# KirillKryukov/naf

Hardware: AMD Instinct MI355X
Metric: unnaf GB/s (uncompressed bases out) on 100 GB synthetic FASTA (higher is better)
Workload: dtype u8; 1 GPU; unnaf decode of a 100.0 GB synthetic-ACGT FASTA archive on one GPU (the size BASELINE.json's metric is quoted on; configs[1] at 10 GB rides along as cfg10_*), 100 records, 80-col lines; archive made in-run by the GPU ennaf; .naf 24739662224 B -> FASTA 99999995684 B, text + archive + decoded text resident in HBM; parallelism=one archive, one GPU, no data-path collective

## Files before the change

### naf_amd/csrc/ctx.h

```cpp
#pragma once
#include "common.h"
#include "../../include/naf_gpu.h"
#include <hip/hip_runtime.h>
#include <stdio.h>
#include <stdarg.h>
#include <string.h>
#include <vector>
#include <functional>
#include <string>

struct ArenaChunk { u8 *base; size_t cap, used; };

struct KTime { const char *name; hipEvent_t a, b; };

#define ZSPLIT_MAX 8
struct ZSplit { int parts; hipEvent_t ev[ZSPLIT_MAX]; u64 out_end[ZSPLIT_MAX]; int done; void *status; };
struct FlatStream { u64 q0, A; };
#define FLAT_DECODED (~0ull)
struct ZFlat { const u8 *src; const FlatStream *si; u64 nslots; const u8 *sym; void *status; bool ready;
               const u8 *tail; u64 tail_q; u32 tail_n;
               const u8 *cls; u32 n_decoded; u32 n_walk;
               struct naf_gpu_ctx *aux; hipEvent_t decoded_ev; void *later; };
struct CtxOpts { std::vector<std::pair<std::string, std::string>> kv; std::string trace; bool tracing = false; };
struct naf_gpu_ctx {
// ... 13 lines not shown
    std::vector<KTime> ktimes;
    std::vector<hipEvent_t> ev_pool;
    size_t ev_used = 0;
    std::vector<std::string> agg_names; std::vector<float> agg_ms; std::vector<int> agg_n;
    float stream_ms[5] = { 0, 0, 0, 0, 0 };
    naf_gpu_ctx *side = nullptr;
    naf_gpu_ctx *side2 = nullptr;
    naf_gpu_ctx *side3 = nullptr;
    naf_gpu_ctx *side4 = nullptr;
    void *sides_thread = nullptr; int sides_rc = 0;
    hipEvent_t fork_ev = nullptr;
    struct ZSplit *zsplit = nullptr;
    hipEvent_t split_ev[ZSPLIT_MAX + 2] = {};
    struct ZFlat *zflat = nullptr;
    void *io_pool = nullptr;
    void *shard_state = nullptr;
    struct HostWorker *worker = nullptr;
};

void ctx_worker_start(naf_gpu_ctx *x, std::function<void()> job);
void ctx_worker_join(naf_gpu_ctx *x);
int  ctx_sides_ready(naf_gpu_ctx *c);

int  ctx_fail(naf_gpu_ctx *c, int code, const char *fmt, ...);
const char *ctx_opt(const naf_gpu_ctx *c, const char *name);
static inline bool ctx_opt_is(const naf_gpu_ctx *c, const char *name, char v) { const char *e = ctx_opt(c, name); return e && e[0] == v; }
bool ctx_tracing(const naf_gpu_ctx *c);
void ctx_trace(naf_gpu_ctx *c, const char *fmt, ...);
#define HIP_TRY(c, call) do { hipError_t e_ = (call); if (e_ != hipSuccess) return ctx_fail((c), NAF_GPU_EHIP, "%s: %s (%s:%d)", #call, hipGetErrorString(e_), __FILE__, __LINE__); } while (0)
static inline void ctx_take_error(naf_gpu_ctx *c, const char (&text)[512]) { memcpy(c->err, text, sizeof c->err); }
static inline void ctx_take_error(naf_gpu_ctx *c, const naf_gpu_ctx *from) { ctx_take_error(c, from->err); }
static inline hipError_t ctx_side_join(naf_gpu_ctx *x) { ctx_worker_join(x); return hipStreamSynchronize(x->stream); }
#define SIDE_SYNC_TRY(c, e, x) do { if ((e) != hipSuccess) return ctx_fail((c), NAF_GPU_EHIP, "%s: %s (%s:%d)", "hipStreamSynchronize(" #x "->stream)", hipGetErrorString(e), __FILE__, __LINE__); } while (0)
struct CtxJoinGuard { naf_gpu_ctx *x; ~CtxJoinGuard() { if (x) ctx_worker_join(x); } };

void  arena_reset(naf_gpu_ctx *c);
void *arena_alloc(naf_gpu_ctx *c, size_t bytes);
void  arena_settle(naf_gpu_ctx *c);
template <typename T> T *arena_new(naf_gpu_ctx *c, size_t n) { return (T *)arena_alloc(c, n * sizeof(T)); }
static inline std::vector<size_t> arena_mark(const naf_gpu_ctx *c) { std::vector<size_t> m; for (auto &ch : c->chunks) m.push_back(ch.used); return m; }
static inline void arena_release(naf_gpu_ctx *c, const std::vector<size_t> &m) { for (size_t k = 0; k < c->chunks.size(); k++) c->chunks[k].used = k < m.size() ? m[k] : 0; }

int ctx_readback(naf_gpu_ctx *c, void *h_dst, const void *d_src, size_t bytes);
int ctx_readback2(naf_gpu_ctx *c, void *h1, const void *d1, size_t n1, void *h2, const void *d2, size_t n2);
int ctx_readbackv(naf_gpu_ctx *c, int n, void *const *h, const void *const *d, const size_t *bytes);

void ktime_begin(naf_gpu_ctx *c, const char *name);
void ktime_end(naf_gpu_ctx *c);

#define LAUNCH(c, name, kern, grid, block, shmem, ...) do { \
    ktime_begin((c), name); \
    hipLaunchKernelGGL(kern, dim3(grid), dim3(block), (shmem), (c)->stream, __VA_ARGS__); \
    ktime_end((c)); } while (0)

static inline u32 cdiv(u64 a, u64 b) { return (u32)((a + b - 1) / b); }

int scan_exclusive_u64(naf_gpu_ctx *c, u64 *d_vals, size_t n, u64 *d_total);
int scan_inclusive_max_i32(naf_gpu_ctx *c, i32 *d_vals, size_t n);
int scan_inclusive_max_i64(naf_gpu_ctx *c, i64 *d_vals, size_t n);
int scan_exclusive_u64_multi(naf_gpu_ctx *c, u64 *const *arrs, int k, size_t n, u64 *const *totals);
int scan_inclusive_max_i64_multi(naf_gpu_ctx *c, i64 *const *arrs, int k, size_t n);

int zstd_decode(naf_gpu_ctx *c, const u8 *d_src, size_t src_len, int has_magic, u8 *d_dst, size_t dst_cap, size_t *out_len, const u8 *head = nullptr);
int zstd_init_tables(naf_gpu_ctx *c);
void ennaf_shard_state_free(naf_gpu_ctx *c);
void io_pool_free(naf_gpu_ctx *c);
struct EmitP;
int zstd_decode_fused_fasta(naf_gpu_ctx *c, const u8 *d_src, size_t src_len, int has_magic, size_t *out_len, const EmitP *P, u8 *text);
struct ZRange { u64 want_lo, want_hi, got_lo, got_hi; bool ranged; u8 *own_buf; };
int zstd_decode_range(naf_gpu_ctx *c, const u8 *d_src, size_t src_len, int has_magic, u8 *d_dst, size_t dst_cap, size_t *out_len, ZRange *rg, const u8 *head = nullptr);
int zstd_split_status(naf_gpu_ctx *c, const ZSplit *sp);
int zstd_flat_later(naf_gpu_ctx *c, ZFlat *zf);
void zstd_flat_drop(ZFlat *zf);
int zstd_small_batch(naf_gpu_ctx *c, int n, const u8 *const *src, const size_t *len, u8 *const *dst, const size_t *cap, bool *ok);
bool zstd_small_fits(size_t len, size_t cap);
int zstd_small_launch(naf_gpu_ctx *c, int n, const u8 *const *src, const size_t *len, u8 *const *dst, const size_t *cap, u32 **d_res_out);
enum { ZENC_PART = 16, ZENC_PART_FIRST = 32, ZENC_PART_LAST = 64, ZENC_PREFER_RAW = 128, ZENC_PREFER_FLAT = 256, ZENC_SHORT_CODES = 512, ZENC_FRAME_TREE = 1024, ZENC_LONG_LAST = 2048 };
int zenc_level_window(int level);
int zenc_repeat_probe(naf_gpu_ctx *c, const u8 *d_src, size_t n, u32 *share_1024);
static inline u32 zenc_probe_every(u64 n) { u32 e = 64; while (((n >> 20) / e) > 128) e <<= 1; return e; }
struct ZencPlace { u8 *(*fn)(void *ud, size_t frame_len); void *ud; };
struct ZencJob;
#define ZENC_LOC_BND 20
struct ZencLoc { const u8 *loc; const i32 *blk_bnd; const u32 *blk_t0; u64 tiles; };
int zstd_encode_begin(naf_gpu_ctx *c, const u8 *d_src, size_t n, int level, int with_magic, int lz, int block_log_hint, int window_log, ZencJob **job, const u8 *direct = nullptr, u32 nd = 0, const ZencLoc *dloc = nullptr);
int zstd_encode_finish(naf_gpu_ctx *c, ZencJob *job, u8 *d_dst, size_t cap, size_t *out_len, const ZencPlace *place);
void zstd_encode_drop(ZencJob *job);
int zstd_encode_size(naf_gpu_ctx *c, ZencJob *job, size_t *frame_len);
const u64 *zstd_encode_total_ptr(const ZencJob *job);
void zstd_encode_set_total(ZencJob *job, u64 total);
int zstd_encode(naf_gpu_ctx *c, const u8 *d_src, size_t n, int level, u8 *d_dst, size_t cap, size_t *out_len, int with_magic, int lz = 0, int block_log_hint = 0, int window_log = 0, const ZencPlace *place = nullptr);
```

### naf_amd/csrc/enc.hip

```cpp
#include "ctx.h"
#include <time.h>
#include "wgscan.h"
#include "enc_swar.h"

#define ET_BYTES 16
#define ET_TILE (256 * ET_BYTES)

struct OpMaxI64 { template <typename T> __device__ static T id() { return (T)(-1); } template <typename T> __device__ static T f(T a, T b) { return (i64)a > (i64)b ? a : b; } };
struct OpMaxU32 { template <typename T> __device__ static T id() { return (T)0; } template <typename T> __device__ static T f(T a, T b) { return a > b ? a : b; } };
struct OpMaxU64 { template <typename T> __device__ static T id() { return (T)0; } template <typename T> __device__ static T f(T a, T b) { return a > b ? a : b; } };

#define REG_ACGT 0x80000000u
#define REG_E(reg) (((reg) >> 24) & 0x7Fu)
struct EncP {
    const u8 *text; u64 n, p0;
    u32 expected[8];
    u8 replacement;
    u8 id_gt_unexpected;
    u8 strict, pad;
    u32 qlo, qhi;
    u32 plo, phi;
    u32 slo, shi;
    u32 nuc32[8];
    u32 *any_case;
// ... 713 lines not shown
    u64 *longest;
    u64 *lead;
    u64 *strict_first;
    const u64 *t_seq, *t_ids, *t_cmt, *t_rec; const u32 *t_tail; const i64 *tile_eol;
    const u32 *irr_list;
    const u32 *t_reg;
    const u8 *direct; u32 nd;
    u32 loc_mode;
    const u32 *sparse_list; const u32 *n_sparse;
};


__device__ __forceinline__ void flush_tile(u8 *dst, const u8 *stage, u32 n)
{
    u32 head = (u32)((8 - ((uintptr_t)dst & 7)) & 7); if (head > n) head = n;
    if (threadIdx.x < head) dst[threadIdx.x] = stage[threadIdx.x];
    u32 words = (n - head) >> 3;
    const u64 *s64 = (const u64 *)stage;
    for (u32 w = threadIdx.x; w < words; w += blockDim.x) {
        u32 off = head + 8 * w, sh = (off & 7) * 8;
        u64 a = s64[off >> 3], b = s64[(off >> 3) + 1];
        *(u64 *)(dst + off) = sh ? (a >> sh) | (b << (64 - sh)) : a;
    }
    u32 done = head + 8 * words;
    if (threadIdx.x < n - done) dst[done + threadIdx.x] = stage[done + threadIdx.x];
}

__device__ __forceinline__ u32 nuc4x4(u32 x, const u32 *t)
{
    const u32 sel = x & 0x07070707u;
    const u32 r0 = swar_perm(t[1], t[0], sel), r1 = swar_perm(t[3], t[2], sel), r2 = swar_perm(t[5], t[4], sel), r3 = swar_perm(t[7], t[6], sel);
    const u32 m3 = ((x >> 3) & 0x01010101u) * 0xFFu, m4 = ((x >> 4) & 0x01010101u) * 0xFFu, m6 = ((x >> 6) & 0x01010101u) * 0xFFu;
    const u32 lo = (r0 & ~m3) | (r1 & m3), hi = (r2 & ~m3) | (r3 & m3);
    const u32 tab = (lo & ~m4) | (hi & m4);
    return (tab & m6) | (m4 & 0x0F0F0F0Fu & ~m6);
}
__device__ __forceinline__ u32 nuc4x4_quick(u32 x) { return swar_perm(0x0F0F0F0Fu, 0x02010408u, (x >> 1) & 0x07070707u); }
__device__ __forceinline__ u32 pack_codes8(u32 c0, u32 c1)
{
    const u32 t0 = c0 | (c0 >> 4), t1 = c1 | (c1 >> 4);
    return swar_perm(t1, t0, 0x06040200u);
}
__device__ __forceinline__ bool all_quick16(const u32 w[4], u32 qlo, u32 qhi)
{
    const u32 L = 0x7F7F7F7Fu; u32 bad = 0;
#pragma unroll
    for (int i = 0; i < 4; i++) { u32 x = w[i], r = swar_perm(qhi, qlo, (x >> 1) & 0x07070707u), d = r ^ (x & 0xDFDFDFDFu); bad |= ((d & L) + L) | d; }
    return (bad & 0x80808080u) == 0;
}
template <bool KNOWN_QUICK>
__device__ __forceinline__ void flush_pack(const EncP &P, u8 *packed, u32 *casebits, u64 tbase, u32 n, const u8 *stage )
{
    if (!n) return;
    const u32 o = (u32)(tbase & 15), span = o + n, ng = (span + 15) >> 4;
    const u64 G0 = tbase >> 4;
    for (u32 j = threadIdx.x; j < ng; j += blockDim.x) {
        const uint4 v = *(const uint4 *)(stage + 16 * j);
        const u32 w[4] = { v.x, v.y, v.z, v.w };
        u32 cd[4];
        if (KNOWN_QUICK || all_quick16(w, P.qlo, P.qhi)) {
#pragma unroll
            for (int i = 0; i < 4; i++) cd[i] = nuc4x4_quick(w[i]);
        } else {
#pragma unroll
            for (int i = 0; i < 4; i++) cd[i] = nuc4x4(w[i], P.nuc32);
        }
        u64 pk = (u64)pack_codes8(cd[0], cd[1]) | ((u64)pack_codes8(cd[2], cd[3]) << 32);
        const u32 H = 0x80808080u;
        u32 cb = swar_movemask16((v.x | ((v.x << 1) & (v.x << 2))) & H, (v.y | ((v.y << 1) & (v.y << 2))) & H,
                                 (v.z | ((v.z << 1) & (v.z << 2))) & H, (v.w | ((v.w << 1) & (v.w << 2))) & H);
        const u32 a = j == 0 ? o : 0u, b = span - 16 * j < 16 ? span - 16 * j : 16u;
        if (a == 0 && b == 16) {
            *(u64 *)(packed + 8 * (G0 + j)) = pk;
            if (casebits) ((u16 *)casebits)[G0 + j] = (u16)cb;
        } else {
            const u64 nm = (b == 16 ? ~0ull : ((1ull << (4 * b)) - 1)) & ~((1ull << (4 * a)) - 1);
            cb &= ((1u << b) - 1) & ~((1u << a) - 1);
            atomicOr((unsigned long long *)(packed + 8 * (G0 + j)), (unsigned long long)(pk & nm));
            if (casebits) atomicOr(casebits + ((G0 + j) >> 1), cb << (16 * (u32)((G0 + j) & 1)));
        }
    }
}
#define DIRECT_PROBE_BLOCKS_LOG 5
__global__ __launch_bounds__(256) void k_direct_blocks(const u8 *text, const u64 *t_seq, const u32 *t_reg, u64 tiles, u32 nd, u32 prefer_flat, int probed, u8 *direct, const u32 *blk_t0 = nullptr, i32 *blk_bnd = nullptr)
{
    __shared__ u32 bins[4][64];
    const u32 wv = threadIdx.x >> 6, lane = threadIdx.x & 63;
    const u32 b = blockIdx.x * 4 + wv;
    bins[wv][lane] = 0;
    __syncthreads();
    bool ok = b < nd;
    if (ok && probed && (((b >> DIRECT_PROBE_BLOCKS_LOG) & (u32)(probed - 1)) == 0)) ok = false;
    u64 t0 = 0, t1 = 0;
    if (ok) {
        const u64 B0 = (u64)b << 16, B1 = B0 + 65536;
        u64 lo = 0, hi = tiles;
        if (blk_t0) { lo = blk_t0[b]; hi = lo + 1; }
        while (hi - lo > 1) {
            const u64 step = (hi - lo + 63) / 64;
            const u64 p = lo + (u64)lane * step;
            const bool le = p < hi && t_seq[p] <= B0;
            const u32 cnt = (u32)__popcll(__ballot(le));
            const u64 nlo = lo + (u64)(cnt - 1) * step, nhi = nlo + step < hi ? nlo + step : hi;
            lo = nlo; hi = nhi;
        }
        t0 = lo;
        const u64 t = t0 + lane;
        const u64 ts = t <= tiles ? t_seq[t] : ~0ull;
        const bool in = t < tiles && ts < B1;
        if (blk_bnd && lane < ZENC_LOC_BND) { const i64 rel = (i64)ts - (i64)B0; blk_bnd[(u64)b * ZENC_LOC_BND + lane] = t <= tiles && rel < (1 << 30) ? (i32)rel : (i32)(1 << 30); }
        const u64 bal = __ballot(in);
        const bool good = !in || ((t_reg[t] & REG_ACGT) != 0);
        ok = __ballot(!good) == 0 && bal != ~0ull;
        t1 = t0 + (u64)__popcll(bal) - 1;
    }
    if (ok) {
        const u64 x0 = t0 * ET_TILE, span = (t1 + 1 - t0) * ET_TILE;
        const u8 *at = text + x0 + (((u64)lane * span) >> 6 & ~63ull);
        uint4 v[4]; __builtin_memcpy(v, at, 64);
        const u32 w[16] = { v[0].x, v[0].y, v[0].z, v[0].w, v[1].x, v[1].y, v[1].z, v[1].w, v[2].x, v[2].y, v[2].z, v[2].w, v[3].x, v[3].y, v[3].z, v[3].w };
        u32 *mybins = &bins[wv][(lane & 3) * 16];
#pragma unroll
        for (int i = 0; i < 16; i++) {
#pragma unroll
            for (int h = 0; h < 2; h++) {
                const u32 pr = (w[i] >> (16 * h)) & 0xFFFFu, c0 = pr & 0xFF, c1 = pr >> 8;
                if ((c0 & 0x40) && (c1 & 0x40)) atomicAdd(&mybins[((c0 >> 1) & 3) | (((c1 >> 1) & 3) << 2)], 1u);
            }
        }
    }
    __syncthreads();
    if (ok) {
        const u32 c = lane < 16 ? bins[wv][lane] + bins[wv][16 + lane] + bins[wv][32 + lane] + bins[wv][48 + lane] : 0u;
        u32 ns = c;
#pragma unroll
        for (u32 d = 1; d < 16; d <<= 1) ns += __shfl_xor((int)ns, d, 64);
        float h = c ? (float)c * __log2f((float)ns / (float)c) : 0.0f;
#pragma unroll
        for (u32 d = 1; d < 16; d <<= 1) h += __shfl_xor(h, d, 64);
        ns = (u32)__shfl((int)ns, 0, 64); h = __shfl(h, 0, 64);
        ok = ns >= 1024 && h * (float)prefer_flat > 4.0f * (float)ns * (float)(prefer_flat - 1);
    }
    if (b < nd && lane == 0) direct[b] = ok ? 1 : 0;
}
__global__ __launch_bounds__(256) void k_direct_verdict(const u64 *t_seq, const u32 *t_reg, const u8 *t_hist, u64 tiles, u32 nd, u32 prefer_flat, int probed, const u32 *blk_t0, u8 *direct, i32 *blk_bnd)
{
    const u32 b = blockIdx.x * 256 + threadIdx.x;
    if (b >= nd) return;
    const u64 B0 = (u64)b << 16, B1 = B0 + 65536, t0 = blk_t0[b];
    bool ok = !(probed && (((b >> DIRECT_PROBE_BLOCKS_LOG) & (u32)(probed - 1)) == 0));
    u64 ts[ZENC_LOC_BND];
#pragma unroll
    for (u32 i = 0; i < ZENC_LOC_BND; i++) ts[i] = t0 + i <= tiles ? t_seq[t0 + i] : ~0ull;
#pragma unroll
    for (u32 i = 0; i < ZENC_LOC_BND; i++) { const i64 rel = (i64)ts[i] - (i64)B0; blk_bnd[(u64)b * ZENC_LOC_BND + i] = ts[i] != ~0ull && rel < (1 << 30) ? (i32)rel : (i32)(1 << 30); }
    u32 acc[8] = { 0, 0, 0, 0, 0, 0, 0, 0 };
    bool end = false;
#pragma unroll
    for (u32 i = 0; i < ZENC_LOC_BND - 1; i++) {
        if (!end && ok) {
            if (t0 + i >= tiles || ts[i] >= B1) end = true;
            else if (!(t_reg[t0 + i] & REG_ACGT)) ok = false;
            else {
                const uint4 h = *(const uint4 *)(t_hist + (t0 + i) * 16);
                acc[0] += h.x & 0x00FF00FFu; acc[1] += (h.x >> 8) & 0x00FF00FFu; acc[2] += h.y & 0x00FF00FFu; acc[3] += (h.y >> 8) & 0x00FF00FFu;
                acc[4] += h.z & 0x00FF00FFu; acc[5] += (h.z >> 8) & 0x00FF00FFu; acc[6] += h.w & 0x00FF00FFu; acc[7] += (h.w >> 8) & 0x00FF00FFu;
            }
        }
    }
    ok = ok && end;
    if (ok) {
        u32 ns = 0;
#pragma unroll
        for (int k = 0; k < 8; k++) ns += (acc[k] & 0xFFFFu) + (acc[k] >> 16);
        float h = 0.0f;
#pragma unroll
        for (int k = 0; k < 8; k++) {
            const u32 c0 = acc[k] & 0xFFFFu, c1 = acc[k] >> 16;
            if (c0) h += (float)c0 * __log2f((float)ns / (float)c0);
            if (c1) h += (float)c1 * __log2f((float)ns / (float)c1);
        }
        ok = ns >= 1024 && h * (float)prefer_flat > 4.0f * (float)ns * (float)(prefer_flat - 1);
    }
    direct[b] = ok ? 1 : 0;
}
__global__ __launch_bounds__(256) void k_case_gather(const u8 *direct, u32 nd, const u32 *blk_t0, const i32 *blk_bnd, const u8 *locc, const u8 *t_lower, u64 *casebits)
{
    __shared__ i32 s_bnd[ZENC_LOC_BND]; __shared__ u8 s_low[ZENC_LOC_BND];
    const u32 b = blockIdx.x;
    if (b >= nd || !direct[b]) return;
    const u64 t0 = blk_t0[b];
    if (threadIdx.x < ZENC_LOC_BND) { s_bnd[threadIdx.x] = blk_bnd[(u64)b * ZENC_LOC_BND + threadIdx.x]; s_low[threadIdx.x] = t_lower[t0 + threadIdx.x]; }
    __syncthreads();
    u32 a[4], c[4], e[4], sh[4], av[4], kk[4]; u64 nx[4];
#pragma unroll
    for (u32 r = 0; r < 4; r++) {
        const u32 W = r * 256u + threadIdx.x;
        const i32 r0 = (i32)(64u * W);
        u32 k = (u32)(r0 - s_bnd[0]) >> 12;
        if (s_bnd[k + 1] <= r0) k++;
        if (s_bnd[k + 1] <= r0) k++;
        const u32 i = (u32)(r0 - s_bnd[k]);
        av[r] = (u32)(s_bnd[k + 1] - r0); kk[r] = k; sh[r] = i & 31u;
        const u32 *p = (const u32 *)(locc + (t0 + k) * (LOC_TILE / 2)) + (i >> 5);
        a[r] = p[0]; c[r] = p[1]; e[r] = p[2];
        nx[r] = av[r] < 64u ? ld64(locc + (t0 + k + 1) * (LOC_TILE / 2)) : 0ull;
    }
#pragma unroll
    for (u32 r = 0; r < 4; r++) {
        u64 w = s_low[kk[r]] ? (u64)__builtin_amdgcn_alignbit(c[r], a[r], sh[r]) | ((u64)__builtin_amdgcn_alignbit(e[r], c[r], sh[r]) << 32) : 0ull;
        if (av[r] < 64u) {
            w &= (1ull << av[r]) - 1;
            if (s_low[kk[r] + 1]) w |= nx[r] << av[r];
        }
        casebits[((u64)b << 10) + r * 256u + threadIdx.x] = w;
    }
}
__global__ void k_irregular_list(const u32 *t_reg, const u64 *pre, u64 tiles, u32 *list, const u64 *t_seq = nullptr, u32 *blk_t0 = nullptr)
{
    const u64 t = (u64)blockIdx.x * blockDim.x + threadIdx.x;
    if (t >= tiles) return;
    if (!t_reg[t]) list[pre[t]] = (u32)t;
    if (blk_t0) {
        const u64 lo = t_seq[t], hi = t_seq[t + 1];
        for (u64 b = (lo + 65535) >> 16; (b << 16) < hi; b++) blk_t0[b] = (u32)t;
    }
}
__global__ void k_pack_edges_zero(const u64 *t_seq, u64 tiles, u64 T, u8 *packed, u32 *casebits, const u8 *direct, u32 nd, u32 loc_mode = 0)
{
    const u64 t = (u64)blockIdx.x * blockDim.x + threadIdx.x;
    if (t >= tiles) return;
    const u64 b0 = t_seq[t], b1 = t + 1 < tiles ? t_seq[t + 1] : T;
    if (b1 <= b0) return;
    const u64 g0 = b0 >> 4, g1 = (b1 - 1) >> 4;
    const bool d0 = direct && (g0 >> 12) < nd && direct[g0 >> 12], d1 = direct && (g1 >> 12) < nd && direct[g1 >> 12];
    if (loc_mode) {
        if (!d0) { *(u64 *)(packed + 8 * g0) = 0; if (casebits) ((u16 *)casebits)[g0] = 0; }
        if (!d1) { *(u64 *)(packed + 8 * g1) = 0; if (casebits) ((u16 *)casebits)[g1] = 0; }
        return;
    }
    if (d0) *((u32 *)(packed + ((g0 >> 12) << 15) + (((g0 >> 10) & 3) << 12)) + (1023u - (u32)(g0 & 1023u))) = 0; else *(u64 *)(packed + 8 * g0) = 0;
    if (d1) *((u32 *)(packed + ((g1 >> 12) << 15) + (((g1 >> 10) & 3) << 12)) + (1023u - (u32)(g1 & 1023u))) = 0; else *(u64 *)(packed + 8 * g1) = 0;
    if (casebits) { ((u16 *)casebits)[g0] = 0; ((u16 *)casebits)[g1] = 0; }
}

__device__ __forceinline__ u64 low_bytes(u32 n) { return n >= 8 ? ~0ull : ((1ull << (8 * n)) - 1); }
__device__ __forceinline__ void lds_store_n(u8 *p, u64 lo, u64 hi, u32 n)
{
    if (n >= 16) { __builtin_memcpy(p, &lo, 8); __builtin_memcpy(p + 8, &hi, 8); return; }
    if (n & 8) { __builtin_memcpy(p, &lo, 8); p += 8; lo = hi; }
    if (n & 4) { u32 v = (u32)lo; __builtin_memcpy(p, &v, 4); p += 4; lo >>= 32; }
    if (n & 2) { u16 v = (u16)lo; __builtin_memcpy(p, &v, 2); p += 2; lo >>= 16; }
    if (n & 1) *p = (u8)lo;
}

__device__ __forceinline__ u32 piece_run_compact(const Piece &pc, u32 a, u32 b, u32 sp, u64 &lo, u64 &hi)
{
    piece_from(pc, a, lo, hi);
    u32 d = (sp >> a) & ((1u << (b - a)) - 1);
    const u32 n = (b - a) - (u32)__popc(d);
    while (d) {
        u32 k = 31 - __clz((int)d); d &= ~(1u << k);
        u64 slo = (lo >> 8) | (hi << 56), shi = hi >> 8;
        if (k < 8) { u64 m = low_bytes(k); lo = (lo & m) | (slo & ~m); hi = shi; }
        else { u64 m = low_bytes(k - 8); hi = (hi & m) | (shi & ~m); }
    }
    return n;
// ... 1721 lines not shown
    if (format == NAF_FMT_FASTA) {
        EncP P; memset(&P, 0, sizeof P);
        P.text = d_text; P.n = n; P.p0 = p0;
        set_expected(P, seq_type, true);
        u64 tiles = n / ET_TILE + 1;
        i64 *t_eol = arena_new<i64>(c, tiles + 1), *t_sp = arena_new<i64>(c, tiles + 1);
        u64 *t_seq = arena_new<u64>(c, tiles + 2), *t_ids = arena_new<u64>(c, tiles + 2), *t_cmt = arena_new<u64>(c, tiles + 2), *t_rec = arena_new<u64>(c, tiles + 2);
        u32 *t_tail = arena_new<u32>(c, tiles + 1), *t_reg = arena_new<u32>(c, tiles + 1), *irr_list = arena_new<u32>(c, tiles + 1);
        u64 *t_irr = arena_new<u64>(c, tiles + 2);
        u64 *tot = arena_new<u64>(c, 8);
        if (!t_eol || !t_sp || !t_seq || !t_ids || !t_cmt || !t_rec || !t_tail || !t_reg || !irr_list || !t_irr || !tot) return NAF_GPU_ENOMEM;
        HIP_TRY(c, hipMemsetAsync(tot + 6, 0, 8, c->stream));
        P.any_case = (u32 *)(tot + 6);
        const char *e_ed = ctx_opt(c, "DIRECT"), *e_epf = ctx_opt(c, "PREFER_FLAT"), *e_ebl = ctx_opt(c, "BLOCK_LOG"), *e_epr = ctx_opt(c, "PROBE"), *e_elz = ctx_opt(c, "LZ"), *e_op = ctx_opt(c, "ONEPASS");
        const u32 e_prefer_flat = e_epf && e_epf[0] ? (u32)atoi(e_epf) : 16u;
        const bool direct_opts = allow_direct && S.fourbit && o->level <= 1 && !o->long_log && !(e_ed && e_ed[0] == '0') && e_prefer_flat >= 2 && !(e_ebl && atoi(e_ebl) != 15) && !(e_epr && e_epr[0] == '1')
                                 && !(e_elz && !strcmp(e_elz, "all")) && n >= 16 * ET_TILE;
        const bool fused = direct_opts && enc_wave_wg(c) && !(e_op && e_op[0] == '0') && (n >> 17) >= ((e_ed && e_ed[0] == '2') || (e_op && e_op[0] == '2') ? 2u : 256u);
        u8 *loc = nullptr, *t_hist = nullptr, *locc = nullptr, *t_lower = nullptr; u32 *t_needf0 = nullptr; u64 *t_need0 = nullptr;
        if (fused) {
            loc = (u8 *)arena_alloc(c, (tiles + 1) * LOC_TILE + 64); t_hist = (u8 *)arena_alloc(c, (tiles + 1) * 16);
            locc = (u8 *)arena_alloc(c, (tiles + 1) * (LOC_TILE / 2) + 64); t_lower = (u8 *)arena_alloc(c, tiles + ZENC_LOC_BND + 2);
            if (!locc || !t_lower) return NAF_GPU_ENOMEM;
            HIP_TRY(c, hipMemsetAsync(t_lower, 0, tiles + ZENC_LOC_BND + 2, c->stream));
            t_needf0 = arena_new<u32>(c, tiles + 1); t_need0 = arena_new<u64>(c, tiles + 2);
            if (!loc || !t_hist || !t_needf0 || !t_need0) return NAF_GPU_ENOMEM;
            LAUNCH(c, "ennaf_split_once", (k_enc_fused<true, 1>), (u32)tiles, 64, 0, P, t_eol, t_sp, t_seq, t_ids, t_cmt, t_rec, t_tail, t_reg, t_irr, t_needf0, t_need0, tiles, loc, t_hist, locc, t_lower);
        } else
        LAUNCH(c, "ennaf_last", k_enc_last_fa, cdiv(tiles, 4 * LAST_TPW), 256, 0, P, t_eol, t_sp, tiles);
        { i64 *const a2[2] = { t_eol, t_sp }; if ((rc = scan_inclusive_max_i64_multi(c, a2, 2, tiles))) return rc; }
        if (S.fourbit && n >= 16 * ET_TILE) {
            u32 *t_needf = fused ? t_needf0 : arena_new<u32>(c, tiles + 1), *need_list = arena_new<u32>(c, tiles + 1); u64 *t_need = fused ? t_need0 : arena_new<u64>(c, tiles + 2);
            if (!t_needf || !need_list || !t_need) return NAF_GPU_ENOMEM;
            if (fused) LAUNCH(c, "ennaf_pure_check", k_pure_check, cdiv(tiles, 256), 256, 0, P, (const i64 *)t_eol, tiles, t_needf, t_need, t_reg, t_irr, (const u32 *)t_tail);
            else if (enc_wave_wg(c)) LAUNCH(c, "ennaf_count_pure", (k_enc_count_pure<1, 1>), (u32)tiles, 64, 0, P, (const i64 *)t_eol, t_seq, t_ids, t_cmt, t_rec, t_tail, t_reg, t_irr, t_needf, t_need, tiles);
            else LAUNCH(c, "ennaf_count_pure", (k_enc_count_pure<4, 1>), cdiv(tiles, 4), 256, 0, P, (const i64 *)t_eol, t_seq, t_ids, t_cmt, t_rec, t_tail, t_reg, t_irr, t_needf, t_need, tiles);
            if ((rc = scan_exclusive_u64(c, t_need, tiles, tot + 5))) return rc;
            LAUNCH(c, "ennaf_need_list", k_need_list, cdiv(tiles, 256), 256, 0, (const u32 *)t_needf, (const u64 *)t_need, tiles, need_list, (const u32 *)nullptr);
            u64 n_need = 0;
            if ((rc = ctx_readback(c, &n_need, tot + 5, 8))) return rc;
            if (ctx_tracing(c)) {
                std::vector<u32> hr(tiles); hipMemcpy(hr.data(), t_reg, tiles * 4, hipMemcpyDeviceToHost);
                u64 nz = 0; for (u64 i = 0; i < tiles; i++) nz += hr[i] != 0;
                ctx_trace(c, "[reg] tiles %llu need %llu regular %llu; reg[1..4] = %08x %08x %08x %08x\n", (unsigned long long)tiles, (unsigned long long)n_need, (unsigned long long)nz, hr[1], hr[2], hr[3], hr[4]);
            }
            if (n_need) LAUNCH(c, "ennaf_count", k_enc_count, n_need, 256, 0, P, (const i64 *)t_eol, (const i64 *)t_sp, t_seq, t_ids, t_cmt, t_rec, t_tail, t_reg, t_irr, (const u32 *)need_list);
        } else
        LAUNCH(c, "ennaf_count", k_enc_count, tiles, 256, 0, P, (const i64 *)t_eol, (const i64 *)t_sp, t_seq, t_ids, t_cmt, t_rec, t_tail, t_reg, t_irr, (const u32 *)nullptr);
        { u64 *const a5[5] = { t_seq, t_ids, t_cmt, t_rec, t_irr }, *const t5[5] = { tot + 0, tot + 1, tot + 2, tot + 3, tot + 4 }; if ((rc = scan_exclusive_u64_multi(c, a5, 5, tiles, t5))) return rc; }
        HIP_TRY(c, hipMemcpyAsync(t_seq + tiles, tot + 0, 8, hipMemcpyDeviceToDevice, c->stream));
        u32 *blk_t0 = fused ? arena_new<u32>(c, (size_t)(n >> 16) + 2) : nullptr;
        if (fused && !blk_t0) return NAF_GPU_ENOMEM;
        LAUNCH(c, "ennaf_irregular_list", k_irregular_list, cdiv(tiles, 256), 256, 0, (const u32 *)t_reg, (const u64 *)t_irr, tiles, irr_list, (const u64 *)t_seq, blk_t0);
        u64 h[7];
        if ((rc = ctx_readback(c, h, tot, 56))) return rc;
        T = h[0]; n_ids = h[1]; n_cmt = h[2]; N = h[3];
        S.no_case = (u32)h[6] == 0 && !(ctx_opt(c, "CASE_CENSUS") && ctx_opt(c, "CASE_CENSUS")[0] == '0');
        P.any_case = nullptr;
        const u64 n_irregular = h[4];
        if ((rc = alloc_bases(c, S, !(allow_direct && S.no_case)))) return rc;
        s_ids = (u8 *)arena_alloc(c, n_ids + 16); s_cmt = (u8 *)arena_alloc(c, n_cmt + 16);
        rec_begin = arena_new<u64>(c, N + 1); rec_end = arena_new<u64>(c, N + 1);
        const size_t NU = 3 * 257 + 3;
        u64 *d_unexp = arena_new<u64>(c, NU);
        if (!s_ids || !s_cmt || !rec_begin || !rec_end || !d_unexp) return NAF_GPU_ENOMEM;
        HIP_TRY(c, hipMemsetAsync(d_unexp, 0, NU * 8, c->stream));
        HIP_TRY(c, hipMemsetAsync(d_unexp + 3 * 257 + 1, 0xFF, 8, c->stream));
        HIP_TRY(c, hipMemsetAsync(rec_begin, 0, (N + 1) * 8, c->stream));
        EncOut O; O.seq = bases; O.packed = S.packed; O.casebits = (u32 *)S.casebits; O.ids = s_ids; O.cmt = s_cmt; O.rec_begin = rec_begin; O.rec_end = rec_end;
        O.unexpected = d_unexp; O.longest = d_unexp + 3 * 257; O.strict_first = o->strict ? d_unexp + 3 * 257 + 1 : nullptr; O.lead = d_unexp + 3 * 257 + 2;
        O.t_seq = t_seq; O.t_ids = t_ids; O.t_cmt = t_cmt; O.t_rec = t_rec; O.t_tail = t_tail; O.tile_eol = t_eol; O.t_reg = t_reg; O.irr_list = S.fourbit ? irr_list : nullptr;
        O.direct = nullptr; O.nd = 0; O.loc_mode = 0; O.sparse_list = nullptr; O.n_sparse = nullptr;
        if (S.fourbit) {
            const u64 n_seqb = (T + 1) / 2;
            const char *ed = e_ed, *epr = e_epr;
            const u32 prefer_flat = e_prefer_flat;
            const u64 nd64 = n_seqb >> 15;
            O.loc_mode = 0; O.sparse_list = nullptr; O.n_sparse = nullptr;
            if (direct_opts && nd64 >= ((ed && ed[0] == '2') || (fused && e_op && e_op[0] == '2') ? 2u : 256u) && nd64 < 0x7FFFFFFFull && !((T & 1) && (n_seqb & 32767) == 0)) {
                S.nd = (u32)nd64; S.direct = (u8 *)arena_alloc(c, S.nd); if (!S.direct) return NAF_GPU_ENOMEM;
                const bool use_loc = fused && !(e_op && e_op[0] == '3' && !S.no_case);
                i32 *blk_bnd = use_loc ? arena_new<i32>(c, (size_t)S.nd * ZENC_LOC_BND + 1) : nullptr;
                if (use_loc && !blk_bnd) return NAF_GPU_ENOMEM;
                if (use_loc) LAUNCH(c, "ennaf_direct_blocks", k_direct_verdict, cdiv(S.nd, 256), 256, 0, (const u64 *)t_seq, (const u32 *)t_reg, (const u8 *)t_hist, tiles, S.nd, prefer_flat, (epr && epr[0] == '0') ? 0 : (int)zenc_probe_every(n_seqb), (const u32 *)blk_t0, S.direct, blk_bnd);
                else LAUNCH(c, "ennaf_direct_blocks", k_direct_blocks, cdiv(S.nd, 4), 256, 0, d_text, (const u64 *)t_seq, (const u32 *)t_reg, tiles, S.nd, prefer_flat, (epr && epr[0] == '0') ? 0 : (int)zenc_probe_every(n_seqb), S.direct, (const u32 *)blk_t0, blk_bnd);
                O.direct = S.direct; O.nd = S.nd;
                if (use_loc) {
                    u32 *sparse_list = arena_new<u32>(c, tiles + 1), *n_sparse = arena_new<u32>(c, 2);
                    if (!sparse_list || !n_sparse) return NAF_GPU_ENOMEM;
                    HIP_TRY(c, hipMemsetAsync(n_sparse, 0, 8, c->stream));
                    O.loc_mode = 1; O.sparse_list = sparse_list; O.n_sparse = n_sparse;
                    LAUNCH(c, "ennaf_sparse_list", k_sparse_list, cdiv(tiles, 256), 256, 0, P, (const i64 *)t_eol, O, tiles, sparse_list, n_sparse);
                    S.dloc.loc = loc; S.dloc.blk_bnd = blk_bnd; S.dloc.blk_t0 = blk_t0; S.dloc.tiles = tiles;
                    if (S.casebits) LAUNCH(c, "ennaf_case_gather", k_case_gather, S.nd, 256, 0, (const u8 *)S.direct, S.nd, (const u32 *)blk_t0, (const i32 *)blk_bnd, (const u8 *)locc, (const u8 *)t_lower, S.casebits);
                }
                if (ctx_tracing(c)) {
                    std::vector<u8> hd(S.nd); hipStreamSynchronize(c->stream); hipMemcpy(hd.data(), S.direct, S.nd, hipMemcpyDeviceToHost);
                    u64 k = 0; for (u8 v : hd) k += v;
                    ctx_trace(c, "[direct] %llu of %u blocks\n", (unsigned long long)k, S.nd);
                }
            }
            S.sc4.P = P; S.sc4.O = O; S.sc4.t_eol = t_eol; S.sc4.t_sp = t_sp; S.sc4.t_seq = t_seq; S.sc4.tiles = tiles; S.sc4.T = T; S.sc4.n = n; S.sc4.n_irregular = n_irregular;
            if ((rc = ennaf_scatter4(c, S.sc4, S.packed, S.casebits))) return rc;
        } else LAUNCH(c, "ennaf_scatter", k_enc_scatter<false>, tiles, 256, 0, P, (const i64 *)t_eol, (const i64 *)t_sp, O);
        std::vector<u64> hu(NU);
        if ((rc = ctx_readback(c, hu.data(), d_unexp, NU * 8))) return rc;
        const u64 sk = hu[3 * 257 + 1];
        if (o->strict && sk != ~0ull) {
            const u64 pos = sk >> 11;
            unsigned long long *d_cnt = arena_new<unsigned long long>(c, 1); if (!d_cnt) return NAF_GPU_ENOMEM;
            HIP_TRY(c, hipMemsetAsync(d_cnt, 0, 8, c->stream));
            LAUNCH(c, "ennaf_count_starts", k_count_starts, (u32)((pos - p0) / 65536 + 1 < 1024 ? (pos - p0) / 65536 + 1 : 1024), 256, 0, d_text, p0, pos, 0, d_cnt);
            u64 cnt = 0; if ((rc = ctx_readback(c, &cnt, d_cnt, 8))) return rc;
            S.err_kind = SE_STRICT; S.err_char = (u32)(sk & 0x1FF); S.err_rec = cnt; S.err_a = (sk >> 9) & 3;
            return 0;
        }
        for (int k = 0; k < 3; k++) for (int i = 0; i < 257; i++) S.unexpected[k][i] = hu[k * 257 + i];
        longest = hu[3 * 257];
        S.lead = N ? hu[3 * 257 + 2] : T;
    }
    return 0;
}

struct EnnafCarry {
    u64 tail_extra;
    u32 skip_first;
    u32 tail_hi;
    int prev_masked;
    int skip_run0;
    u64 run_ext;
};
struct EnnafStreams { const u8 *ptr[6]; u64 len[6], orig[6]; int lz[6], block_log[6], window_log[6]; bool present[6];
                      u32 tail[6]; int flags[6];
                      const u8 *direct; u32 nd, tail_packed; const ZencLoc *dloc; };

static int ennaf_streams(naf_gpu_ctx *c, EnnafSplit &S, const EnnafCarry &K, EnnafStreams &X, int part = 3)
{
    if (part & 1) memset(&X, 0, sizeof X);
    int rc; const u64 T = S.T, N = S.N;
    u32 *s_len = nullptr; u8 *s_seq = nullptr, *s_mask = nullptr;
    u64 n_lenb = 0, n_seqb = 0, n_mask = 0; int mask_block_log = 15; u32 seq_tail = 0;
    if (S.format != 0) {
        if (N && (part & 2)) {
            u64 *lu = arena_new<u64>(c, N + 2); if (!lu) return NAF_GPU_ENOMEM;
            const u64 total = T + K.tail_extra;
            LAUNCH(c, "ennaf_len_count", k_len_unit_count, cdiv(N, 256), 256, 0, (const u64 *)S.rec_begin, (const u64 *)S.rec_end, N, total, lu, S.all_ends);
            if ((rc = scan_exclusive_u64(c, lu, N, lu + N + 1))) return rc;
            u64 nu = 0; if ((rc = ctx_readback(c, &nu, lu + N + 1, 8))) return rc;
            s_len = arena_new<u32>(c, nu + 1); if (!s_len) return NAF_GPU_ENOMEM;
            LAUNCH(c, "ennaf_len_write", k_len_unit_write, cdiv(N, 256), 256, 0, (const u64 *)S.rec_begin, (const u64 *)S.rec_end, N, total, (const u64 *)lu, s_len, S.all_ends);
            n_lenb = nu * 4;
        }
        const u64 mt = (T + MBB_TILE - 1) / MBB_TILE;
        u64 *tc = S.tc;
        if (!(part & 1)) { }
        else if (S.fourbit) {
            const u64 Tp = T > K.skip_first ? T - K.skip_first : 0;
            n_seqb = (Tp + 1) / 2;
            if (K.skip_first && n_seqb) {
                s_seq = (u8 *)arena_alloc(c, n_seqb + 16); if (!s_seq) return NAF_GPU_ENOMEM;
                LAUNCH(c, "ennaf_nibble_shift", k_nibble_shift, cdiv(cdiv(n_seqb, 8), 256), 256, 0, (const u8 *)S.packed, (T + 1) / 2, s_seq, n_seqb);
            } else s_seq = S.packed;
            if ((Tp & 1) && K.tail_hi) LAUNCH(c, "ennaf_tail_nibble", k_set_high_nibble, 1, 64, 0, s_seq + n_seqb - 1, K.tail_hi);
            if ((Tp & 1) && !K.tail_hi && n_seqb >= 2 && !S.store_qual) seq_tail = 1;
        } else {
            if (S.no_mask && T) LAUNCH(c, "ennaf_toupper", k_toupper, cdiv(T, 256), 256, 0, S.bases, T);
            s_seq = S.bases; n_seqb = T;
        }
        if (S.store_mask && T && (part & 2)) {
            u64 nb = 0; i64 *tile_last = S.census ? S.census_last : nullptr;
            const bool one_run = !S.census && S.no_case && !K.skip_run0 && !K.prev_masked;
            if (!one_run) {
            if (!S.census) {
                tc = arena_new<u64>(c, mt + 2); tile_last = arena_new<i64>(c, mt + 1); if (!tc || !tile_last) return NAF_GPU_ENOMEM;
                LAUNCH(c, "ennaf_mask_count", k_maskb_count, mt, 256, 0, (const u64 *)S.casebits, T, tc, 0, tile_last);
                if ((rc = scan_inclusive_max_i64(c, tile_last, mt))) return rc;
            }
            const int b0 = S.census ? ((S.first_base >= 96) != (K.prev_masked != 0)) : 0;
            if (b0) LAUNCH(c, "ennaf_mask_b0", k_add_u64, 1, 64, 0, tc, (u64)1);
            if ((rc = scan_exclusive_u64(c, tc, mt, tc + mt + 1))) return rc;
            if ((rc = ctx_readback(c, &nb, tc + mt + 1, 8))) return rc;
            }
            u64 nu = 0;
            if (nb == 0 && !K.skip_run0) {
                const u64 len = T + K.run_ext;
                nu = len / 255 + 1;
                s_mask = (u8 *)arena_alloc(c, nu + 16); if (!s_mask) return NAF_GPU_ENOMEM;
                HIP_TRY(c, hipMemsetAsync(s_mask, 0xFF, nu, c->stream));
                SmallBytes lb; memset(&lb, 0, sizeof lb); lb.b[0] = (u8)(len % 255); lb.n = 1;
                LAUNCH(c, "ennaf_mask_units", k_put_bytes, 1, 64, 0, s_mask + (nu - 1), lb);
            } else {
            u64 *any_long = arena_new<u64>(c, 1), *bnd = nullptr;
            if (!any_long) return NAF_GPU_ENOMEM;
            u64 longs = 1;
            const char *ms = ctx_opt(c, "MASK_SHORT");
            if (tile_last && nb >= (1u << 16) && nb * 64 >= T && !(ms && (ms[0] == '0' || ms[0] == '1'))) {
                nu = nb + 1 - (K.skip_run0 ? 1 : 0);
                s_mask = (u8 *)arena_alloc(c, nu + 16); if (!s_mask) return NAF_GPU_ENOMEM;
                HIP_TRY(c, hipMemsetAsync(any_long, 0, 8, c->stream));
                LAUNCH(c, "ennaf_mask_units", k_maskb_units_direct, mt, 256, 0, (const u64 *)S.casebits, T, (const u64 *)tc, (const i64 *)tile_last, nb, s_mask, K.run_ext, K.skip_run0, K.prev_masked, any_long);
                if ((rc = ctx_readback(c, &longs, any_long, 8))) return rc;
            }
            if (longs) {
            bnd = arena_new<u64>(c, nb + 1); if (!bnd) return NAF_GPU_ENOMEM;
            if (nb) LAUNCH(c, "ennaf_mask_bscatter", k_maskb_scatter, mt, 256, 0, (const u64 *)S.casebits, T, (const u64 *)tc, nb, bnd, K.prev_masked);
            { 
              if (!(ms && ms[0] == '0') && (nb + 1) * 255 > T + K.run_ext) {
                  nu = nb + 1 - (K.skip_run0 ? 1 : 0);
                  s_mask = (u8 *)arena_alloc(c, nu + 16); if (!s_mask) return NAF_GPU_ENOMEM;
                  HIP_TRY(c, hipMemsetAsync(any_long, 0, 8, c->stream));
                  LAUNCH(c, "ennaf_mask_units", k_mask_units_short, cdiv(nb + 1, 256), 256, 0, (const u64 *)bnd, nb, T, s_mask, K.run_ext, K.skip_run0, any_long);
                  if ((rc = ctx_readback(c, &longs, any_long, 8))) return rc;
              } }
            }
            if (longs) {
                u64 *ru = arena_new<u64>(c, nb + 3); if (!ru) return NAF_GPU_ENOMEM;
                LAUNCH(c, "ennaf_mask_runs", k_mask_run_units, cdiv(nb + 1, 256), 256, 0, (const u64 *)bnd, nb, T, ru, K.run_ext, K.skip_run0);
                if ((rc = scan_exclusive_u64(c, ru, nb + 1, ru + nb + 2))) return rc;
                if ((rc = ctx_readback(c, &nu, ru + nb + 2, 8))) return rc;
                s_mask = (u8 *)arena_alloc(c, nu + 16); if (!s_mask) return NAF_GPU_ENOMEM;
                if (nu) HIP_TRY(c, hipMemsetAsync(s_mask, 0xFF, nu, c->stream));
                LAUNCH(c, "ennaf_mask_units", k_mask_units_write, cdiv(nb + 1, 256), 256, 0, (const u64 *)bnd, nb, T, (const u64 *)ru, s_mask, K.run_ext, K.skip_run0);
            }
            }
            mask_block_log = 13;
            { const char *mb = ctx_opt(c, "MASK_BLOCK_LOG"); if (mb && atoi(mb) >= 10 && atoi(mb) <= 17) mask_block_log = atoi(mb); else if (nu >= (64ull << 20)) mask_block_log = 15; }
            n_mask = nu;
        }
    }
    if (part & 1) {
        X.ptr[0] = S.s_ids; X.len[0] = X.orig[0] = S.n_ids; X.lz[0] = 1; X.present[0] = true;
        X.ptr[1] = S.s_cmt; X.len[1] = X.orig[1] = S.n_cmt; X.lz[1] = 1; X.present[1] = true;
        { const char *sb_ = ctx_opt(c, "NAMES_BLOCK_LOG"); const int v = sb_ ? atoi(sb_) : 0; if (v >= 10 && v <= 15) X.block_log[1] = v; else if (S.n_cmt >= (16u << 20)) X.block_log[1] = 15; }
        X.tail_packed = seq_tail; X.direct = nullptr; X.nd = 0;
        X.dloc = nullptr;
        if (S.direct && (part & 1)) { X.direct = S.direct; X.nd = S.nd; seq_tail = (u32)(n_seqb & 32767); X.dloc = S.dloc.loc ? &S.dloc : nullptr; }
        X.ptr[4] = s_seq; X.len[4] = n_seqb; X.orig[4] = T; X.present[4] = true; X.tail[4] = seq_tail;
        if (S.store_qual) X.flags[4] |= ZENC_LONG_LAST;
        X.ptr[5] = S.s_qual; X.len[5] = X.orig[5] = S.n_qual; X.present[5] = S.store_qual;
    }
    if (part & 2) {
        X.ptr[2] = (const u8 *)s_len; X.len[2] = X.orig[2] = n_lenb; X.lz[2] = 1; X.present[2] = true;
        { const char *sb_ = ctx_opt(c, "SIDE_BLOCK_LOG"); const int v = sb_ ? atoi(sb_) : 0; if (v >= 10 && v <= 15) X.block_log[2] = v; else if (n_lenb >= (16u << 20)) X.block_log[2] = 15; }
        X.ptr[3] = s_mask; X.len[3] = X.orig[3] = n_mask; X.block_log[3] = mask_block_log; X.present[3] = S.store_mask; X.flags[3] = ZENC_PREFER_RAW;
    }
    return 0;
}

static void ennaf_probe_verdict(EnnafStreams &X, u32 share) { if (share >= 32) { X.window_log[4] = 19; X.lz[4] = 1; } }
static int ennaf_windows(naf_gpu_ctx *c, EnnafStreams &X, const naf_gpu_ennaf_opts *o, bool *defer = nullptr)
{
    const int wl = zenc_level_window(o->level);
    for (int i = 0; i < 6; i++) X.window_log[i] = wl;
    if (o->level <= 1) X.flags[4] |= ZENC_PREFER_FLAT;
    if (o->level <= 1) { X.flags[4] |= ZENC_SHORT_CODES; X.flags[5] |= ZENC_SHORT_CODES; }
    if (o->level <= 1) { X.flags[4] |= ZENC_FRAME_TREE; X.flags[5] |= ZENC_FRAME_TREE; }
    if (o->long_log) { X.window_log[4] = o->long_log < 10 ? 10 : o->long_log > 31 ? 31 : o->long_log; X.lz[4] = 1; }
    else if (!wl && X.present[4] && X.len[4]) {
        const char *pe = ctx_opt(c, "PROBE");
        u32 share = 0;
        if (pe && pe[0] == '1') share = 1024;
        else if (!(pe && pe[0] == '0') && defer) { *defer = true; return 0; }
        else if (!(pe && pe[0] == '0')) {
            int rc = zenc_repeat_probe(c, X.ptr[4], X.len[4], &share); if (rc) return rc;
        }
        ennaf_probe_verdict(X, share);
    }
    return 0;
}

static size_t naf_header_bytes(const naf_gpu_ennaf_opts *o, bool store_mask, bool store_qual, u64 longest, u64 N, u8 *hd )
{
    size_t hl = 0;
    hd[hl++] = 0x01; hd[hl++] = 0xF9; hd[hl++] = 0xEC;
    if (o->seq_type == NAF_SEQ_DNA) hd[hl++] = 1; else { hd[hl++] = 2; hd[hl++] = (u8)o->seq_type; }
    hd[hl++] = (u8)(((o->title ? 1 : 0) << 6) | (1 << 5) | (1 << 4) | (1 << 3) | ((store_mask ? 1 : 0) << 2) | (1 << 1) | (store_qual ? 1 : 0));
    hd[hl++] = ' ';
    hl += vle(o->line_length >= 0 ? (u64)o->line_length : longest, hd + hl);
    hl += vle(N, hd + hl);
    if (o->title) hl += vle(strlen(o->title), hd + hl);
    return hl;
}

struct PlaceTail { const ZencPlace *outer; size_t tail_len; u8 *at; };
static u8 *place_before_tail(void *ud, size_t len) { PlaceTail *t = (PlaceTail *)ud; return t->at = t->outer->fn(t->outer->ud, len + t->tail_len); }
struct StreamJob { ZencJob *main; const u8 *d_stream; u64 len; int level, flags; u32 tail; bool sized; u8 *tail_tmp; size_t tail_len; int tail_flags; };
static int encode_stream_begin(naf_gpu_ctx *c, const u8 *d_stream, u64 len, int level, int flags, int lz, int block_log, int window_log, u32 tail, StreamJob *J, const u8 *direct = nullptr, u32 nd = 0, const ZencLoc *dloc = nullptr)
{
    J->main = nullptr; J->d_stream = d_stream; J->len = len; J->level = level; J->flags = flags; J->tail = (tail && len > tail) ? tail : 0;
    J->sized = false; J->tail_tmp = nullptr; J->tail_len = 0; J->tail_flags = 0;
    int f1 = flags;
    if (J->tail) f1 = ZENC_PART | ((!(flags & ZENC_PART) || (flags & ZENC_PART_FIRST)) ? ZENC_PART_FIRST : 0) | (flags & (ZENC_PREFER_RAW | ZENC_PREFER_FLAT | ZENC_SHORT_CODES | ZENC_FRAME_TREE));
    J->tail_flags = flags & ZENC_LONG_LAST;
    if (direct && (lz || len - J->tail != (u64)nd << 15)) return ctx_fail(c, NAF_GPU_EARG, "direct blocks need a stream of whole blocks and no match finder");
    int rc = zstd_encode_begin(c, d_stream, len - J->tail, level, f1, lz, block_log, window_log, &J->main, direct, nd, dloc);
    if (rc) { zstd_encode_drop(J->main); J->main = nullptr; }
    return rc;
}
static int encode_stream_size(naf_gpu_ctx *c, StreamJob *J, size_t *clen)
{
    if (J->tail && !J->sized) {
        const int f2 = ZENC_PART | ((!(J->flags & ZENC_PART) || (J->flags & ZENC_PART_LAST)) ? ZENC_PART_LAST : 0) | J->tail_flags;
        const size_t tb = naf_gpu_zstd_compress_bound(J->tail);
        u8 *tmp = (u8 *)arena_alloc(c, tb); if (!tmp) return NAF_GPU_ENOMEM;
        size_t b = 0;
        int rc = zstd_encode(c, J->d_stream + (J->len - J->tail), J->tail, J->level, tmp, tb, &b, f2, 0, 0, 0); if (rc) return rc;
        J->tail_tmp = tmp; J->tail_len = b;
    }
    size_t a = 0;
    int rc = zstd_encode_size(c, J->main, &a); if (rc) return rc;
    J->sized = true;
    *clen = a + J->tail_len;
    return 0;
}
static int encode_stream_finish(naf_gpu_ctx *c, StreamJob *J, size_t *clen, const ZencPlace *place)
{
    ZencJob *mj = J->main; J->main = nullptr;
    if (!J->tail) return zstd_encode_finish(c, mj, nullptr, 0, clen, place);
    const int f2 = ZENC_PART | ((!(J->flags & ZENC_PART) || (J->flags & ZENC_PART_LAST)) ? ZENC_PART_LAST : 0) | J->tail_flags;
// ... 14 lines not shown
}
static int encode_stream(naf_gpu_ctx *c, const u8 *d_stream, u64 len, int level, u8 *dst, size_t cap, size_t *clen, int flags, int lz, int block_log, int window_log, u32 tail, const ZencPlace *place = nullptr)
{
    if (place) {
        StreamJob J; int rc = encode_stream_begin(c, d_stream, len, level, flags, lz, block_log, window_log, tail, &J); if (rc) return rc;
        return encode_stream_finish(c, &J, clen, place);
    }
    if (!tail || len <= tail) return zstd_encode(c, d_stream, len, level, dst, cap, clen, flags, lz, block_log, window_log);
    const bool part = (flags & ZENC_PART) != 0;
    const int f1 = ZENC_PART | ((!part || (flags & ZENC_PART_FIRST)) ? ZENC_PART_FIRST : 0) | (flags & (ZENC_PREFER_RAW | ZENC_PREFER_FLAT | ZENC_SHORT_CODES | ZENC_FRAME_TREE));
    const int f2 = ZENC_PART | ((!part || (flags & ZENC_PART_LAST)) ? ZENC_PART_LAST : 0) | (flags & ZENC_LONG_LAST) | (tail >= 2048 ? (flags & (ZENC_PREFER_FLAT | ZENC_SHORT_CODES)) : 0);
    size_t a = 0, b = 0;
    int rc = zstd_encode(c, d_stream, len - tail, level, dst, cap, &a, f1, lz, block_log, window_log); if (rc) return rc;
    rc = zstd_encode(c, d_stream + (len - tail), tail, level, dst + a, cap - a, &b, f2, 0, 0, 0); if (rc) return rc;
    *clen = a + b;
    return 0;
}

__global__ void k_collect4(const u64 *a, const u64 *b, const u64 *c4, const u64 *d, u64 *out) { if (threadIdx.x < 4) { const u64 *p = threadIdx.x == 0 ? a : threadIdx.x == 1 ? b : threadIdx.x == 2 ? c4 : d; out[threadIdx.x] = p ? *p : 0; } }
struct SecOut { u64 orig, comp; };

struct SecPlace { naf_gpu_ctx *c; u8 *d_naf; size_t cap, pos; u64 orig; size_t hl; int rc; };
static u8 *place_section(void *ud, size_t clen)
{
    SecPlace *p = (SecPlace *)ud; naf_gpu_ctx *c = p->c;
    SmallBytes h; memset(&h, 0, sizeof h);
    size_t hl = vle(p->orig, h.b); hl += vle(clen, h.b + hl); h.n = (u32)hl;
    if (p->pos + hl + clen > p->cap) { p->rc = ctx_fail(c, NAF_GPU_ECAP, "ennaf output capacity %zu too small", p->cap); return nullptr; }
    hipLaunchKernelGGL(k_put_bytes, dim3(1), dim3(64), 0, c->stream, p->d_naf + p->pos, h);
    if (hipGetLastError() != hipSuccess) { p->rc = ctx_fail(c, NAF_GPU_EHIP, "section header launch failed"); return nullptr; }
    p->hl = hl;
    return p->d_naf + p->pos + hl;
}

static int put_section(naf_gpu_ctx *c, naf_gpu_ctx *report, const u8 *d_stream, u64 stream_len, u64 orig, int level, u8 *d_naf, size_t cap, size_t &pos, SecOut &so, int lz, int block_log, int window_log, u32 tail, StreamJob *early, int flags = 0, const u8 *direct = nullptr, u32 nd = 0, const ZencLoc *dloc = nullptr)
{
    SecPlace sp = { c, d_naf, cap, pos, orig, 0, 0 }; ZencPlace P = { place_section, &sp };
    size_t clen = 0;
    StreamJob J;
    int rc = 0;
    if (!early) { rc = encode_stream_begin(c, d_stream, stream_len, level, flags, lz, block_log, window_log, tail, &J, direct, nd, dloc); early = &J; }
    if (!rc) rc = encode_stream_finish(c, early, &clen, &P);
    if (rc) { if (report != c) ctx_fail(report, sp.rc ? sp.rc : rc, "%s", c->err); return sp.rc ? sp.rc : rc; }
    pos += sp.hl + clen;
    so.orig = orig; so.comp = clen;
    return 0;
}

static int ennaf_whole(naf_gpu_ctx *c, const void *d_text_, size_t n, const naf_gpu_ennaf_opts *o,
                       void *d_naf_, size_t cap, size_t *naf_len, naf_gpu_ennaf_report *rep);
extern "C" int naf_gpu_ennaf(naf_gpu_ctx *c, const void *d_text_, size_t n, const naf_gpu_ennaf_opts *o,
                             void *d_naf_, size_t cap, size_t *naf_len, naf_gpu_ennaf_report *rep)
{
    if (!c || !o || !d_naf_ || !naf_len || (!d_text_ && n)) return NAF_GPU_EARG;
    int rc = ennaf_whole(c, d_text_, n, o, d_naf_, cap, naf_len, rep);
    arena_settle(c);
    return rc;
}
static int ennaf_whole(naf_gpu_ctx *c, const void *d_text_, size_t n, const naf_gpu_ennaf_opts *o,
                       void *d_naf_, size_t cap, size_t *naf_len, naf_gpu_ennaf_report *rep)
{
    arena_reset(c);
    { int rs = ctx_sides_ready(c); if (rs) return rs; }
    const u8 *d_text = (const u8 *)d_text_; u8 *d_naf = (u8 *)d_naf_;
    naf_gpu_ennaf_report R; memset(&R, 0, sizeof R);
    if (o->seq_type < 0 || o->seq_type > 3) return ctx_fail(c, NAF_GPU_EARG, "bad seq_type");
    int format = 0, rc; u64 p0 = 0;
    if ((rc = ennaf_sniff(c, d_text, n, o->format, &format, &p0))) return rc;
    R.format = format;
    EnnafSplit S;
    if ((rc = ennaf_split(c, d_text, n, o, format, p0, true, S, true))) return rc;
    if (S.err_kind) return split_error_text(c, o->seq_type, S.err_kind, S.err_char, S.err_rec, S.err_a, S.err_b, 0);
    EnnafCarry K; memset(&K, 0, sizeof K);
    naf_gpu_ctx *sc = c->side;
    const char *eo = ctx_opt(c, "ENC_OVERLAP");
    const bool force_overlap = eo && !strcmp(eo, "2");
    const bool overlap = sc && !(eo && !strcmp(eo, "0")) && (force_overlap || S.T >= (32u << 20) || S.n_qual >= (16u << 20));
    EnnafStreams X;
    if ((rc = ennaf_streams(c, S, K, X, overlap ? 1 : 3))) return rc;
    bool probe_later = false;
    if ((rc = ennaf_windows(c, X, o, overlap ? &probe_later : nullptr))) return rc;
    auto undirect = [&]() -> int {
        if (!X.direct) return 0;
        X.direct = nullptr; X.nd = 0; X.tail[4] = X.tail_packed; S.direct = nullptr; S.nd = 0; X.dloc = nullptr; S.dloc.loc = nullptr;
        S.sc4.O.direct = nullptr; S.sc4.O.nd = 0; S.sc4.O.loc_mode = 0;
        return ennaf_scatter4(c, S.sc4, S.packed, S.casebits);
    };
    if (X.lz[4] && (rc = undirect())) return rc;
    u8 hd[64]; size_t hl = naf_header_bytes(o, S.store_mask, S.store_qual, S.longest, S.N, hd);
    size_t tl = o->title ? strlen(o->title) : 0;
    size_t pos = 0;
    if (hl + tl > cap) return ctx_fail(c, NAF_GPU_ECAP, "ennaf output capacity %zu too small", cap);
    { SmallBytes hb; memset(&hb, 0, sizeof hb); memcpy(hb.b, hd, hl); hb.n = (u32)hl; LAUNCH(c, "ennaf_header", k_put_bytes, 1, 64, 0, d_naf, hb); pos += hl; }
    if (tl) { HIP_TRY(c, hipMemcpyAsync(d_naf + pos, o->title, tl, hipMemcpyHostToDevice, c->stream)); pos += tl; HIP_TRY(c, hipStreamSynchronize(c->stream)); }
    StreamJob big[6]; bool early[6] = { false, false, false, false, false, false };
    naf_gpu_ctx *sb = nullptr; int rcB = 0;
    naf_gpu_ctx *pc = nullptr; int rcP = 0; u32 probe_share = 0; bool probe_out = false;
    auto bail = [&](int r, naf_gpu_ctx *from) -> int {
        if (sb) ctx_worker_join(sb);
        if (probe_out) { ctx_worker_join(pc); probe_out = false; hipStreamSynchronize(pc->stream); }
        for (int k = 0; k < 6; k++) if (early[k]) { zstd_encode_drop(big[k].main); early[k] = false; }
        hipStreamSynchronize(sc->stream); if (sb) hipStreamSynchronize(sb->stream);
        return from && from != c ? ctx_fail(c, r, "%s", from->err) : r;
    };
    if (overlap) {
        arena_reset(sc);
        HIP_TRY(c, hipEventRecord(c->fork_ev, c->stream));
        HIP_TRY(c, hipStreamWaitEvent(sc->stream, c->fork_ev, 0));
        sb = (S.N >= 65536 || force_overlap || (S.store_mask && S.T >= (256u << 20))) ? c->side2 : nullptr;
        if (sb) {
            arena_reset(sb);
            HIP_TRY(c, hipStreamWaitEvent(sb->stream, c->fork_ev, 0));
            ctx_worker_start(sb, [&] {
                rcB = ennaf_streams(sb, S, K, X, 2);
                for (int i = 2; i < 4 && !rcB; i++)
                    if (X.present[i]) { rcB = encode_stream_begin(sb, X.ptr[i], X.len[i], o->level, X.flags[i], X.lz[i], X.block_log[i], X.window_log[i], X.tail[i], &big[i]); early[i] = !rcB; }
            });
        } else if ((rc = ennaf_streams(sc, S, K, X, 2))) return bail(rc, sc);
        if (probe_later && c->side3) {
            pc = c->side3;
            arena_reset(pc);
            if (hipStreamWaitEvent(pc->stream, c->fork_ev, 0) != hipSuccess) return bail(ctx_fail(c, NAF_GPU_EHIP, "ennaf: the look's stream"), c);
            probe_out = true;
            ctx_worker_start(pc, [&] { rcP = zenc_repeat_probe(pc, X.ptr[4], X.len[4], &probe_share); });
        }
        for (int i = 4; i < 6; i++)
            if (X.present[i]) {
                if ((rc = encode_stream_begin(c, X.ptr[i], X.len[i], o->level, X.flags[i], X.lz[i], X.block_log[i], X.window_log[i], X.tail[i], &big[i], i == 4 ? X.direct : nullptr, i == 4 ? X.nd : 0u, i == 4 ? X.dloc : nullptr))) return bail(rc, c);
                early[i] = true;
            }
        for (int i = 0; i < 2; i++)
            if (X.present[i]) {
                if ((rc = encode_stream_begin(sc, X.ptr[i], X.len[i], o->level, X.flags[i], X.lz[i], X.block_log[i], X.window_log[i], X.tail[i], &big[i]))) return bail(rc, sc);
                early[i] = true;
            }
        if (probe_later) {
            if (probe_out) { ctx_worker_join(pc); probe_out = false; if (rcP) return bail(rcP, pc); }
            else if ((rc = zenc_repeat_probe(sc, X.ptr[4], X.len[4], &probe_share))) return bail(rc, sc);
            ennaf_probe_verdict(X, probe_share);
            if (X.lz[4]) {
                zstd_encode_drop(big[4].main); early[4] = false;
                if ((rc = undirect())) return bail(rc, c);
                if ((rc = encode_stream_begin(c, X.ptr[4], X.len[4], o->level, X.flags[4], X.lz[4], X.block_log[4], X.window_log[4], X.tail[4], &big[4]))) return bail(rc, c);
                early[4] = true;
            }
        }
    }
    for (int i = 0; i < 257; i++) { R.unexpected_id[i] = S.unexpected[0][i]; R.unexpected_comment[i] = S.unexpected[1][i]; R.unexpected_seq[i] = S.unexpected[2][i]; R.unexpected_qual[i] = S.unexpected[3][i]; }
    R.n_sequences = S.N; R.n_bases = S.T; R.longest_line = S.longest;

    SecOut so[6]; memset(so, 0, sizeof so);
    bool joined = !overlap, joinedB = sb == nullptr;
    auto join = [&]() -> int {
        if (joined) return 0;
        joined = true;
        if (hipEventRecord(c->split_ev[0], sc->stream) != hipSuccess || hipStreamWaitEvent(c->stream, c->split_ev[0], 0) != hipSuccess) return ctx_fail(c, NAF_GPU_EHIP, "ennaf: joining the side stream failed");
        if (sb && (hipEventRecord(c->split_ev[1], sb->stream) != hipSuccess || hipStreamWaitEvent(c->stream, c->split_ev[1], 0) != hipSuccess)) return ctx_fail(c, NAF_GPU_EHIP, "ennaf: joining the side stream failed");
        return 0;
    };
    auto joinB = [&]() -> int {
        if (joinedB) return 0;
        joinedB = true;
        ctx_worker_join(sb);
        return rcB ? ctx_fail(c, rcB, "%s", sb->err) : 0;
    };
    const char *sf = ctx_opt(c, "SIZES_FIRST");
    if (overlap && !(sf && sf[0] == '0')) {
// ... 378 lines not shown
```

### naf_amd/csrc/zstd_enc.hip

```cpp
#include "ctx.h"
#include <vector>
#include "zstd_enc_core.h"

#define ZENC_TREE_SLOT 192
#include "wgscan.h"
#include "enc_swar.h"
struct OpMaxU64 { template <typename T> __device__ static T id() { return (T)0; } template <typename T> __device__ static T f(T a, T b) { return a > b ? a : b; } };
#define ZENC_HCOPIES 4
#define ZENC_CACHE_ENTRIES 256
struct ZTreeEntry { u64 key; u32 tb, pad; u8 wt[256]; u8 tree[ZENC_TREE_SLOT]; };
struct ZTreeCache { ZTreeEntry e[ZENC_CACHE_ENTRIES]; };
static_assert(ZENC_CACHE_ENTRIES == 256, "one entry per thread of the plan kernel");
struct ZPlanWS {
    u32 tot[256]; u32 w[512]; u16 order[256]; u16 parent[512]; u8 depth[512];
    u8 len[256], wt[256], tree[ZENC_TREE_SLOT], tmp[160];
    FseWS fse; u32 log, tb;
};

struct ZFlat16 { u32 tb; u8 tree[ZENC_TREE_SLOT]; };
static const ZFlat16 &zenc_flat16()
{
    static const ZFlat16 T = [] {
        ZFlat16 t; memset(&t, 0, sizeof t);
        u8 wt[256]; memset(wt, 0, sizeof wt);
        for (u32 s = 0; s < 256; s++) if (__builtin_popcount(s & 15u) == 1 && __builtin_popcount(s >> 4) == 1) wt[s] = 1;
        static FseWS ws; u8 tmp[160];
        t.tb = huf_write_tree_w(t.tree, wt, 0x88u, tmp, ws, true);
        return t;
    }();
    return T;
}
__host__ __device__ static inline u64 zenc_block_lo(u64 n, u32 nblk, u32 b) { u64 q = n / nblk, r = n % nblk; return (u64)b * q + (b < r ? b : r); }

#define ZENC_FLATSCAN_WAVES 4
__global__ __launch_bounds__(64 * ZENC_FLATSCAN_WAVES) void k_zenc_flat_scan(const u8 *src, u64 n, u32 nblk, ZEncPlan *plan, u16 *codes, u8 *trees, u64 *csize, u8 *done, u32 min_gain, u32 prefer_flat, ZFlat16 f16, const u8 *planned, const u8 *direct)
{
    __shared__ u32 bins[ZENC_FLATSCAN_WAVES][64];
    const u32 wv = threadIdx.x >> 6, lane = threadIdx.x & 63;
    for (u32 bq = blockIdx.x; bq * ZENC_FLATSCAN_WAVES < nblk; bq += gridDim.x) {
    const u32 b = bq * ZENC_FLATSCAN_WAVES + wv;
    if (planned && bq * ZENC_FLATSCAN_WAVES + ZENC_FLATSCAN_WAVES <= nblk && *(const u32 *)(planned + bq * ZENC_FLATSCAN_WAVES) == 0x01010101u) continue;
    bins[wv][lane] = 0;
    __syncthreads();
    bool ok = b < nblk;
    u32 bn = 0; const u8 *s = src;
    if (ok) {
        const u64 lo = zenc_block_lo(n, nblk, b), hi = zenc_block_lo(n, nblk, b + 1);
        bn = (u32)(hi - lo); s = src + lo;
        ok = bn >= 2048;
    }
    const bool dir = ok && direct && direct[b];
    if (ok && !dir) {
        u64 bad = 0;
        const bool sampler = (lane & 3) == 0;
        u32 *mybins = &bins[wv][((lane >> 2) & 3) * 16];
        const u64 M5 = 0x5555555555555555ull, M3 = 0x3333333333333333ull, ONE = 0x1111111111111111ull;
#pragma unroll 8
        for (u32 i = lane * 16; i + 16 <= bn; i += 1024) {
            const u64 w0 = ld64(s + i), w1 = ld64(s + i + 8);
            u64 c0 = w0 - ((w0 >> 1) & M5), c1 = w1 - ((w1 >> 1) & M5);
            c0 = (c0 & M3) + ((c0 >> 2) & M3); c1 = (c1 & M3) + ((c1 >> 2) & M3);
            bad |= (c0 ^ ONE) | (c1 ^ ONE);
            if (sampler) {
                const u64 lg = ((w0 >> 1) & 0x7777777777777777ull) - ((w0 >> 3) & 0x1111111111111111ull);
                const u64 rk = ((lg >> 2) & 0x0C0C0C0C0C0C0C0Cull) | (lg & 0x0303030303030303ull);
#pragma unroll
                for (u32 k = 0; k < 8; k++) atomicAdd(&mybins[(u32)(rk >> (8 * k)) & 15u], 1u);
            }
        }
        if (lane == 0) for (u32 k = bn & ~15u; k < bn; k++) { const u32 v = s[k]; if (__popc(v & 15u) != 1 || __popc(v >> 4) != 1) bad = 1; }
        ok = __ballot(bad != 0) == 0;
    }
    __syncthreads();
    bool fast = dir;
    if (ok && !dir) {
        const u32 c = lane < 16 ? bins[wv][lane] + bins[wv][16 + lane] + bins[wv][32 + lane] + bins[wv][48 + lane] : 0u;
        u32 ns = c;
#pragma unroll
        for (u32 d = 1; d < 16; d <<= 1) ns += __shfl_xor((int)ns, d, 64);
        float h = c ? (float)c * __log2f((float)ns / (float)c) : 0.0f;
#pragma unroll
        for (u32 d = 1; d < 16; d <<= 1) h += __shfl_xor(h, d, 64);
        ns = (u32)__shfl((int)ns, 0, 64); h = __shfl(h, 0, 64);
        fast = ns > 0 && h * (float)prefer_flat > 4.0f * (float)ns * (float)(prefer_flat - 1);
    }
    if (fast) {
        const u32 perq = (bn + 3) / 4;
        ZEncPlan p; p.n = bn; p.kind = ZK_RAW; p.csize = 3 + bn; p.log = 0; p.tree_bytes = 0; p.lhdr = 0; p.pad = 0; p.frame = 0; p.pad2 = 0;
        for (u32 k = 0; k < 4; k++) p.ssz[k] = ((k < 3 ? perq : bn - 3 * perq) * 4 + 8) >> 3;
        zenc_plan_finish(p, bn, 4, f16.tb, min_gain);
        fast = p.kind == ZK_HUF;
        if (fast) {
            p.pad = dir ? 2 : 1;
            if (lane == 0) { plan[b] = p; if (csize) csize[b] = p.csize; }
            if (!dir)
            for (u32 sym = lane; sym < 256; sym += 64) {
                const bool is16 = __popc(sym & 15u) == 1 && __popc(sym >> 4) == 1;
                const u32 hn = sym >> 4, ln = sym & 15u, rank = 4 * ((hn >> 1) - (hn >> 3)) + ((ln >> 1) - (ln >> 3));
                codes[(u64)b * 256 + sym] = is16 ? (u16)(rank | (4u << 12)) : (u16)0;
            }
            for (u32 k = lane; k < p.tree_bytes; k += 64) trees[(u64)b * ZENC_TREE_SLOT + k] = f16.tree[k];
        }
    }
    if (b < nblk && lane == 0) done[b] = fast ? 1 : 0;
    }
}

__global__ void k_zenc_direct_plans(const u8 *direct, u32 nblk, ZEncPlan pd, ZFlat16 f16, ZEncPlan *plan, u8 *trees, u64 *csize, u8 *done)
{
    const u32 b = blockIdx.x * blockDim.x + threadIdx.x;
    if (b >= nblk || !direct[b]) return;
    plan[b] = pd; if (csize) csize[b] = pd.csize; done[b] = 1;
    for (u32 k = 0; k < pd.tree_bytes; k++) trees[(u64)b * ZENC_TREE_SLOT + k] = f16.tree[k];
}

__global__ __launch_bounds__(256) void k_zenc_plan(const u8 *src, u64 n, u32 nblk, ZEncPlan *plan, u16 *codes, u8 *trees, u64 *csize, const u32 *blk_len, u64 slot, ZTreeCache *cache, u32 sample_stride, u32 try_fse, u32 min_gain, u32 maxbits, u32 prefer_flat, const u8 *done, u8 *wt_defer,
                                                    u32 *fhist = nullptr, const ZEncPlan *fplan = nullptr, const u16 *fcodes = nullptr, const u32 *fratio = nullptr, u32 long_last = 0)
{
    __shared__ u32 hist[ZENC_HCOPIES * 1024];
    u32 b = sample_stride ? blockIdx.x * sample_stride : blockIdx.x;
    if (done && done[b]) return;
    u64 lo = zenc_block_lo(n, nblk, b), hi = zenc_block_lo(n, nblk, b + 1);
    if (blk_len) { lo = (u64)b * slot; hi = lo + blk_len[b]; }
    u32 bn = (u32)(hi - lo);
    for (u32 i = threadIdx.x; i < ZENC_HCOPIES * 1024; i += 256) hist[i] = 0;
    __syncthreads();
    u32 per = (bn + 3) / 4; if (!per) per = 1;
    const u8 *s = src + lo;
    const u32 cpy = threadIdx.x & (ZENC_HCOPIES - 1), rot = 8 * cpy;
    u32 *my = hist + cpy * 1024;
    const u64 rot8 = 0x0101010101010101ull * rot;
#ifdef ZPLAN_NOHIST
    if (threadIdx.x < 16) for (u32 q = 0; q < 4; q++) hist[q * 256 + threadIdx.x * 17] = bn / 64;
    if (0)
#endif
    for (u32 i0 = threadIdx.x * 8; i0 < bn; i0 += 8 * 2048) {
        u64 wv[8];
#pragma unroll
        for (u32 j = 0; j < 8; j++) { const u32 i = i0 + j * 2048; wv[j] = i + 8 <= bn ? ld64(s + i) : 0; }
#pragma unroll
        for (u32 j = 0; j < 8; j++) {
            const u32 i = i0 + j * 2048;
            if (i >= bn) break;
            if (i + 8 <= bn) {
                const u64 w = wv[j];
                const u32 q0 = (i >= per) + (i >= 2 * per) + (i >= 3 * per), q7 = (i + 7 >= per) + (i + 7 >= 2 * per) + (i + 7 >= 3 * per);
                if (q0 == q7) {
                    const u64 H = 0x8080808080808080ull;
                    const u64 wr = ((w & ~H) + rot8) ^ (w & H);
                    u32 *hq = my + q0 * 256;
                    const u32 lo = (u32)wr, hi = (u32)(wr >> 32);
#pragma unroll
                    for (u32 k = 0; k < 4; k++) { atomicAdd(&hq[(lo >> (8 * k)) & 0xFF], 1u); atomicAdd(&hq[(hi >> (8 * k)) & 0xFF], 1u); }
                } else {
#pragma unroll
                    for (u32 k = 0; k < 8; k++) { u32 pos = i + k, q = (pos >= per) + (pos >= 2 * per) + (pos >= 3 * per); atomicAdd(&my[q * 256 + (((u32)(w >> (8 * k)) + rot) & 0xFF)], 1u); }
                }
            } else {
                for (u32 k = 0; i + k < bn; k++) { u32 pos = i + k, q = (pos >= per) + (pos >= 2 * per) + (pos >= 3 * per); atomicAdd(&my[q * 256 + ((s[pos] + rot) & 0xFF)], 1u); }
            }
        }
    }
    __syncthreads();
    u32 red4[4];
    for (u32 q = 0; q < 4; q++) { u32 v = 0; for (u32 k = 0; k < ZENC_HCOPIES; k++) v += hist[k * 1024 + q * 256 + ((threadIdx.x + 8 * k) & 0xFF)]; red4[q] = v; }
    __syncthreads();
    for (u32 q = 0; q < 4; q++) hist[q * 256 + threadIdx.x] = red4[q];
    __syncthreads();
    static_assert(sizeof(ZPlanWS) <= (ZENC_HCOPIES - 1) * 4096, "plan workspace must fit the dead histogram copies");
    ZPlanWS &ws = *(ZPlanWS *)(hist + 1024);
    __shared__ u64 red[4];
    const u32 sym = threadIdx.x;
    u32 mine = hist[sym] + hist[256 + sym] + hist[512 + sym] + hist[768 + sym];
    ws.tot[sym] = mine; ws.len[sym] = 0;
    u32 distinct = (u32)__syncthreads_count(mine != 0);
    __shared__ u16 plist[256]; __shared__ u32 wave_n[4];
    u64 bal = __ballot(mine != 0);
    u32 myidx = (u32)__popcll(bal & ((1ull << (threadIdx.x & 63)) - 1));
    if ((threadIdx.x & 63) == 0) wave_n[threadIdx.x >> 6] = (u32)__popcll(bal);
    __syncthreads();
    for (u32 w = 0; w < (threadIdx.x >> 6); w++) myidx += wave_n[w];
    if (mine) plist[myidx] = (u16)sym;
    __syncthreads();
    ZEncPlan p; p.n = bn; p.kind = ZK_RAW; p.csize = 3 + bn; p.log = 0; p.tree_bytes = 0; p.lhdr = 0; p.pad = 0; p.frame = 0; p.pad2 = 0;
    p.ssz[0] = p.ssz[1] = p.ssz[2] = p.ssz[3] = 0;
    if (fhist && sample_stride && mine) atomicAdd(&fhist[sym], mine);
    if (fcodes && !sample_stride && fplan->kind == ZK_HUF && bn >= 64 && distinct >= 2) {
        __shared__ u64 fred[4];
        const u32 fl = (u32)fcodes[sym] >> 12;
        if (__syncthreads_and(mine == 0 || fl != 0)) {
            const float ent = mine ? (float)mine * __log2f((float)bn / (float)mine) : 0.f;
            u64 both; wg_scan_inclusive<u64, OpAdd>(((u64)(mine * fl) << 32) | (u64)(u32)(ent + 0.5f), &both, fred);
            const u64 fbits = both >> 32, ebits = both & 0xFFFFFFFFull;
            if (fbits * 1024 * 100 <= ebits * fratio[0] * 103 + 6400ull * 1024) {
                for (u32 k = 0; k < 4; k++) { u64 bits; wg_scan_inclusive<u64, OpAdd>((u64)hist[256 * k + sym] * fl, &bits, fred); p.ssz[k] = (u32)((bits + 1 + 7) / 8); }
                zenc_plan_finish(p, bn, fplan->log, 0, min_gain);
                if (p.kind == ZK_HUF && p.csize + fplan->tree_bytes <= 3 + bn) {
                    p.frame = 1; codes[(u64)b * 256 + sym] = fcodes[sym];
                    if (threadIdx.x == 0) { plan[b] = p; if (csize) csize[b] = p.csize; }
                    return;
                }
                if (p.kind != ZK_HUF) {
                    if (threadIdx.x == 0) { plan[b] = p; if (csize) csize[b] = p.csize; }
// ... 100 lines not shown
        __syncthreads();
        u32 log = ws.log;
        if (prefer_flat && log && !flat_log && (distinct & (distinct - 1)) == 0) {
            const u32 k = (u32)(31 - __clz((int)distinct));
            u64 hb; wg_scan_inclusive<u64, OpAdd>((u64)mine * ws.len[sym], &hb, red);
            const u64 fb = (u64)bn * k;
            if (fb >= hb && (fb - hb) * prefer_flat < fb) {
                ws.len[sym] = mine ? (u8)k : (u8)0;
                if (threadIdx.x == 0) ws.log = k;
                flat_log = k;
            }
            __syncthreads();
            log = ws.log;
        }
        if (log) {
            u32 l = ws.len[sym];
            ws.wt[sym] = l ? (u8)(log + 1 - l) : 0;
            u64 lastw; wg_scan_inclusive<u64, OpMaxU64>(l ? (u64)sym : 0, &lastw, red);
            u64 hk; wg_scan_inclusive<u64, OpAdd>(l ? (u64)(sym * 16 + (log + 1 - l) + 1) * 0x9E3779B97F4A7C15ull ^ ((u64)sym << 40) : 0, &hk, red);
            hk |= 1;
            bool hit = false;
            if (cache && !sample_stride) {
                __shared__ u32 s_slot;
                if (threadIdx.x == 0) s_slot = ~0u;
                __syncthreads();
                if (cache->e[sym].key == hk) atomicMin(&s_slot, sym);
                __syncthreads();
                u32 slot_i = s_slot;
                if (slot_i != ~0u) {
                    const ZTreeEntry *ce = &cache->e[slot_i];
                    hit = __syncthreads_and(ce->wt[sym] == ws.wt[sym]) != 0;
                    if (hit) { if (sym < ZENC_TREE_SLOT) ws.tree[sym] = ce->tree[sym]; if (sym == 0) ws.tb = ce->tb; }
                }
            }
            const bool direct_w = !try_fse && (u32)lastw >= 1 && (u32)lastw <= 128;
            defer = wt_defer && !sample_stride && !hit && !direct_w && (u32)lastw >= 1;
            if (!hit && direct_w) {
                const u32 nw = (u32)lastw;
                if (sym == 0) { ws.tree[0] = (u8)(127 + nw); ws.tb = 1 + (nw + 1) / 2; }
                if (2 * sym < nw) ws.tree[1 + sym] = (u8)((ws.wt[2 * sym] << 4) | (2 * sym + 1 < nw ? ws.wt[2 * sym + 1] : 0));
            }
            else if (!hit && defer) wt_defer[(u64)b * 256 + sym] = ws.wt[sym];
            else if (!hit && threadIdx.x == 0) ws.tb = huf_write_tree_w(ws.tree, ws.wt, (u32)lastw, ws.tmp, ws.fse, try_fse != 0);
            if (cache && sample_stride) {
                __syncthreads();
                ZTreeEntry *ce = &cache->e[blockIdx.x];
                ce->wt[sym] = ws.wt[sym]; if (sym < ZENC_TREE_SLOT) ce->tree[sym] = ws.tree[sym];
                if (sym == 0) { ce->tb = ws.tb; ce->key = ws.tb ? hk : 0; }
            }
            u64 bits;
            if (flat_log) {
                const u32 perq = (bn + 3) / 4;
                for (u32 k = 0; k < 4; k++) p.ssz[k] = ((k < 3 ? perq : bn - 3 * perq) * flat_log + 8) >> 3;
            } else
            for (u32 k = 0; k < 4; k++) { wg_scan_inclusive<u64, OpAdd>((u64)hist[256 * k + sym] * l, &bits, red); p.ssz[k] = (u32)((bits + 1 + 7) / 8); }
            __syncthreads();
            u32 tb = ws.tb;
            if (defer) {
                huf = true; p.log = (u8)log; p.tree_bytes = (u16)lastw; p.lhdr = (u8)(try_fse != 0);
                p.pad = (u8)(0x80u | ((log == 4 && distinct == 16) ? 1u : 0u));
            } else
            if (tb) { zenc_plan_finish(p, bn, log, tb, min_gain); huf = p.kind == ZK_HUF; if (huf && log == 4 && distinct == 16) p.pad = 1; }
        }
    }
    if (threadIdx.x == 0) { plan[b] = p; if (csize) csize[b] = p.csize; }
    if (huf && p.log && ws.len[plist[0]] == p.log && distinct == (1u << p.log)) {
        const u32 l = ws.len[sym];
        codes[(u64)b * 256 + sym] = l ? (u16)(myidx | (l << 12)) : (u16)0;
        if (!defer && sym < p.tree_bytes) trees[(u64)b * ZENC_TREE_SLOT + sym] = ws.tree[sym];
    } else
    if (huf) {
        __shared__ u32 wcnt[16], wstart[16];
        if (sym < 16) wcnt[sym] = 0;
        __syncthreads();
        u32 l = ws.len[sym], wgt = l ? p.log + 1 - l : 0, rank = 0;
        if (l) { atomicAdd(&wcnt[wgt], 1u); for (u32 j = 0; j < myidx; j++) rank += ws.len[plist[j]] == l; }
        __syncthreads();
        if (sym == 0) { u32 pos = 0; for (u32 w = 1; w <= p.log; w++) { wstart[w] = pos; pos += wcnt[w] << (w - 1); } }
        __syncthreads();
        codes[(u64)b * 256 + sym] = l ? (u16)(((wstart[wgt] >> (wgt - 1)) + rank) | (l << 12)) : (u16)0;
        if (!defer && sym < p.tree_bytes) trees[(u64)b * ZENC_TREE_SLOT + sym] = ws.tree[sym];
    }
}

#define ZENC_FRAME_BLOCK 32768u
__global__ __launch_bounds__(256) void k_zenc_frame_block(const u32 *fhist, u8 *blockbuf, u32 *blen)
{
    __shared__ u64 red[4];
    const u32 sym = threadIdx.x, h = fhist[sym];
    u64 tot; wg_scan_inclusive<u64, OpAdd>((u64)h, &tot, red);
    u32 cnt = 0;
    if (h && tot) { cnt = (u32)(((u64)h * (ZENC_FRAME_BLOCK - 256)) / tot); if (!cnt) cnt = 1; }
    u64 all; const u64 inc = wg_scan_inclusive<u64, OpAdd>((u64)cnt, &all, red);
    u8 *o = blockbuf + (inc - cnt);
    for (u32 k = 0; k < cnt; k++) o[k] = (u8)sym;
    if (sym == 0) *blen = (u32)all;
}
__global__ __launch_bounds__(256) void k_zenc_frame_ratio(u32 *fhist, const u16 *fcodes)
{
    __shared__ u64 red[4];
    const u32 h = fhist[threadIdx.x], l = (u32)fcodes[threadIdx.x] >> 12;
    u64 tot = wg_reduce1<u64, OpAdd>((u64)h, red);
    __syncthreads();
    const float ent = (h && tot) ? (float)h * __log2f((float)tot / (float)h) : 0.f;
    const u64 both = wg_reduce1<u64, OpAdd>(((u64)h * l) << 0 | 0ull, red);
    __syncthreads();
    const u64 e = wg_reduce1<u64, OpAdd>((u64)(ent + 0.5f), red);
    if (threadIdx.x == 0) { u64 r = e ? both * 1024 / e : 1024; fhist[257] = (u32)(r < 1024 ? 1024 : r > 1229 ? 1229 : r); }
}
#define ZQ_MISSING 0x80u
__device__ __forceinline__ u32 zq_hash4(u32 x) { return (x ^ (x >> 4)) & 0x0F0F0F0Fu; }
__global__ __launch_bounds__(256) void k_zenc_frame_stats(const u32 *fhist, const u16 *fcodes, float *fstat)
{
    __shared__ u64 red[4];
    const u32 sym = threadIdx.x, h = fhist[sym], l = (u32)fcodes[sym] >> 12, x[3] = { l, l * l, (sym ^ (sym >> 4)) & 15u };
    const u64 N = wg_reduce1<u64, OpAdd>((u64)h, red);
    __syncthreads();
    for (u32 k = 0; k < 3; k++) {
        const u64 a = wg_reduce1<u64, OpAdd>((u64)h * x[k], red);
        __syncthreads();
        const u64 b2 = wg_reduce1<u64, OpAdd>((u64)h * x[k] * x[k], red);
        __syncthreads();
        if (sym == 0) {
            const double mu = N ? (double)a / (double)N : 0.0, var = N ? (double)b2 / (double)N - mu * mu : 0.0;
            fstat[2 * k] = (float)mu; fstat[2 * k + 1] = var > 0.0 ? (float)sqrt(var) : 0.f;
        }
    }
}
__global__ __launch_bounds__(256) void k_zenc_frame_quick(const u8 *src, u64 n, u32 nblk, ZEncPlan *plan, u16 *codes, u64 *csize, u8 *done,
                                                           const ZEncPlan *fplan, const u16 *fcodes, const float *fstat, u32 min_gain, u32 stride, u32 *tally, const u32 *gate)
{
    __shared__ __attribute__((aligned(16))) u8 tab[256 * 64];
    __shared__ u32 s_q[4][4], s_accept;
    const u32 b = stride ? blockIdx.x * stride : blockIdx.x, tid = threadIdx.x, lane = tid & 63, q = tid >> 6;
    if (!stride && gate && gate[0] * 2 < gate[1]) return;
    if (b >= nblk || done[b] || fplan->kind != ZK_HUF) return;
    const u64 lo = zenc_block_lo(n, nblk, b), hi = zenc_block_lo(n, nblk, b + 1);
    const u32 bn = (u32)(hi - lo);
    if (bn < 64) return;
    const u16 fc = fcodes[tid];
    {
        const u32 l = (u32)fc >> 12, v = (l ? l : ZQ_MISSING) * 0x01010101u;
        uint4 r; r.x = r.y = r.z = r.w = v;
        uint4 *row = (uint4 *)(tab + 64 * tid);
        row[0] = r; row[1] = r; row[2] = r; row[3] = r;
    }
    __syncthreads();
    const u32 per = (bn + 3) / 4;
    const u32 qlo = q * per < bn ? q * per : bn, qhi = q == 3 ? bn : (qlo + per < bn ? qlo + per : bn);
    const u8 *s = src + lo, *my = tab + lane;
    u32 s1 = 0, s2 = 0, orr = 0, sh = 0;
    for (u32 i0 = qlo + lane * 8; i0 < qhi; i0 += 8 * 512) {
        u64 wv[8];
#pragma unroll
        for (u32 j = 0; j < 8; j++) { const u32 i = i0 + j * 512; wv[j] = i + 8 <= qhi ? ld64(s + i) : 0; }
#pragma unroll
        for (u32 j = 0; j < 8; j++) {
            const u32 i = i0 + j * 512;
            if (i >= qhi) break;
            if (i + 8 <= qhi) {
                const u32 x0 = (u32)wv[j], x1 = (u32)(wv[j] >> 32);
#pragma unroll
                for (u32 k = 0; k < 4; k++) {
                    const u32 t0 = my[((x0 >> (8 * k)) & 0xFF) << 6], t1 = my[((x1 >> (8 * k)) & 0xFF) << 6];
                    s1 += t0 + t1; s2 += t0 * t0; s2 += t1 * t1; orr |= t0 | t1;
                }
                sh = swar_dot4(zq_hash4(x0), 0x01010101u, sh); sh = swar_dot4(zq_hash4(x1), 0x01010101u, sh);
            } else for (u32 k = 0; i + k < qhi; k++) {
                const u32 c = s[i + k], t = my[c << 6];
                s1 += t; s2 += t * t; orr |= t; sh += (c ^ (c >> 4)) & 15u;
            }
        }
    }
#pragma unroll
    for (int d = 32; d; d >>= 1) { s1 += (u32)__shfl_xor((int)s1, d, 64); s2 += (u32)__shfl_xor((int)s2, d, 64); sh += (u32)__shfl_xor((int)sh, d, 64); orr |= (u32)__shfl_xor((int)orr, d, 64); }
    if (lane == 0) { s_q[q][0] = s1; s_q[q][1] = s2; s_q[q][2] = sh; s_q[q][3] = orr; }
    __syncthreads();
    ZEncPlan p;
    if (tid == 0) {
        u32 accept = 0;
        const u32 S[3] = { s_q[0][0] + s_q[1][0] + s_q[2][0] + s_q[3][0], s_q[0][1] + s_q[1][1] + s_q[2][1] + s_q[3][1], s_q[0][2] + s_q[1][2] + s_q[2][2] + s_q[3][2] };
        bool like = !((s_q[0][3] | s_q[1][3] | s_q[2][3] | s_q[3][3]) & ZQ_MISSING);
        const float fb = (float)bn, rt = sqrtf(fb);
        for (u32 k = 0; k < 3 && like; k++) {
            const float want = fb * fstat[2 * k], d = fabsf((float)S[k] - want);
            if (d > 6.f * rt * fstat[2 * k + 1] + 0.005f * want) like = false;
        }
        if (like) {
            p.n = bn; p.kind = ZK_RAW; p.csize = 3 + bn; p.log = 0; p.tree_bytes = 0; p.lhdr = 0; p.pad = 0; p.frame = 0; p.pad2 = 0;
            for (u32 k = 0; k < 4; k++) p.ssz[k] = (s_q[k][0] + 1 + 7) / 8;
            zenc_plan_finish(p, bn, fplan->log, 0, min_gain);
            if (p.kind == ZK_HUF && p.csize + fplan->tree_bytes <= 3 + bn) { p.frame = 1; accept = 1; }
            else if (p.kind != ZK_HUF) accept = 2;
        }
        if (stride) { atomicAdd(&tally[1], 1u); if (accept) atomicAdd(&tally[0], 1u); accept = 0; }
        if (accept) { plan[b] = p; if (csize) csize[b] = p.csize; done[b] = 1; }
        s_accept = accept;
    }
    __syncthreads();
    if (s_accept == 1) codes[(u64)b * 256 + tid] = fc;
}

__global__ void k_zenc_frame_class(const ZEncPlan *plan, u32 nblk, i32 *v)
{
    const u32 b = blockIdx.x * blockDim.x + threadIdx.x;
    if (b < nblk) v[b] = plan[b].kind == ZK_HUF ? (i32)(2 * b + (plan[b].frame ? 0u : 1u)) : -1;
}
__global__ void k_zenc_frame_fix(ZEncPlan *plan, u32 nblk, const i32 *v, const ZEncPlan *fplan, const u8 *ftree, u8 *trees, u64 *csize)
{
    const u32 b = blockIdx.x * blockDim.x + threadIdx.x;
    if (b >= nblk || plan[b].kind != ZK_HUF || !plan[b].frame) return;
    const i32 prev = b ? v[b - 1] : -1;
    if (prev >= 0 && !(prev & 1)) return;
    ZEncPlan p = plan[b];
    const u32 tb = fplan->tree_bytes;
    zenc_plan_force(p, tb);
    for (u32 k = 0; k < tb; k++) trees[(u64)b * ZENC_TREE_SLOT + k] = ftree[k];
    plan[b] = p; if (csize) csize[b] = p.csize;
}

struct ZTreeLane { FseWS fse; u8 tmp[160]; u8 w[256]; u32 odd; };
static_assert((sizeof(ZTreeLane) / 4) % 2 == 1, "odd word stride: the lanes' workspaces start in different LDS banks");
__global__ __launch_bounds__(64) void k_zenc_tree(u32 nblk, ZEncPlan *plan, u8 *trees, u64 *csize, const u8 *wt_defer, u32 min_gain)
{
    __builtin_amdgcn_s_setprio(3);
    extern __shared__ __attribute__((aligned(16))) u8 tree_lds[];
    const u32 b = blockIdx.x * 64 + threadIdx.x;
    const bool pending = b < nblk && (plan[b].pad & 0x80u);
    if (!__ballot(pending)) return;
    if (!pending) return;
    ZTreeLane &L = ((ZTreeLane *)tree_lds)[threadIdx.x];
    ZEncPlan p = plan[b];
    const u32 lastw = p.tree_bytes, log = p.log, try_fse = p.lhdr, flat16 = p.pad & 1u;
    for (u32 k = 0; k < 256; k += 4) *(u32 *)(L.w + k) = *(const u32 *)(wt_defer + (u64)b * 256 + k);
    u8 *tree = trees + (u64)b * ZENC_TREE_SLOT;
    const u32 tb = huf_write_tree_w(tree, L.w, lastw, L.tmp, L.fse, try_fse != 0);
    p.kind = ZK_RAW; p.csize = 3 + p.n; p.log = 0; p.tree_bytes = 0; p.lhdr = 0; p.pad = 0; p.frame = 0; p.pad2 = 0;
    if (tb) { zenc_plan_finish(p, p.n, log, tb, min_gain); if (p.kind == ZK_HUF && flat16) p.pad = 1; }
    plan[b] = p;
    if (csize) csize[b] = p.csize;
}

#define LZ_MINMATCH 5
__device__ __forceinline__ u32 rdlane(u32 v, u32 l) { return (u32)__builtin_amdgcn_readlane((int)v, (int)l); }
#define LZ_HASH_LOG 12
#define LZ_BLOCK_MAX 32768
#define LZ_LANE_EXT 32
struct LzBufs {
    u8 *lits; u64 slot;
    u16 *ll, *ml, *of; u64 seq_slot;
    u32 *ofv;
    u32 *nseq, *nlit;
    u8 *seqbuf; u32 *seq_bytes;
};
__global__ __launch_bounds__(64) void k_lz_parse(const u8 *src, u64 n, u32 nblk, LzBufs B, u32 buf_bytes, u32 hash_log, const u8 *fallback = nullptr)
{
    if (fallback && !fallback[blockIdx.x]) return;

    __builtin_amdgcn_s_setprio(3);
    extern __shared__ __attribute__((aligned(16))) u8 lz_lds[];
    u8 *buf = lz_lds;
    u16 *tab = (u16 *)(lz_lds + buf_bytes);
    const u32 b = blockIdx.x, lane = threadIdx.x;
    const u64 lo = zenc_block_lo(n, nblk, b);
    const u32 bn = (u32)(zenc_block_lo(n, nblk, b + 1) - lo);
    for (u32 i = lane * 16; i < bn; i += 64 * 16) {
        if (i + 16 <= bn) { uint4 v; __builtin_memcpy(&v, src + lo + i, 16); *(uint4 *)(buf + i) = v; }
        else for (u32 k = i; k < bn; k++) buf[k] = src[lo + k];
    }
    for (u32 i = lane; i < (1u << hash_log); i += 64) tab[i] = 0;
    for (u32 i = bn + lane; i < bn + 320 && i < buf_bytes; i += 64) buf[i] = 0;
    __syncthreads();
    u8 *lits = B.lits + (u64)b * B.slot;
    u16 *sll = B.ll + (u64)b * B.seq_slot, *sml = B.ml + (u64)b * B.seq_slot, *sof = B.of + (u64)b * B.seq_slot;
    u32 cur = 0, anchor = 0, ns = 0, nl = 0;
    while (cur + LZ_MINMATCH <= bn) {
        u32 p = cur + lane; bool valid = p + LZ_MINMATCH <= bn;
        u32 v = 0, h = 0, c = 0, m = 0;
        if (valid) {
            __builtin_memcpy(&v, buf + p, 4);
            h = (v * 2654435761u) >> (32 - hash_log);
            c = tab[h];
            if (c) {
                u32 q = c - 1, cv; __builtin_memcpy(&cv, buf + q, 4);
                if (cv == v) {
                    m = 4;
                    for (;;) {
                        u64 x, y; __builtin_memcpy(&x, buf + q + m, 8); __builtin_memcpy(&y, buf + p + m, 8);
                        const u64 d = x ^ y;
                        if (d) { m += (u32)(__ffsll((long long)d) - 1) >> 3; break; }
                        m += 8;
                        if (p + m >= bn || m >= LZ_LANE_EXT) break;
                    }
                    if (p + m > bn) m = bn - p;
                }
            }
        }
        u64 win = __ballot(m >= LZ_MINMATCH);
        if (valid) tab[h] = (u16)(p + 1);
        u32 next = cur < anchor ? anchor : cur;
        while (next < cur + 64) {
            u64 w2 = win & ~((1ull << (next - cur)) - 1);
            if (!w2) break;
            u32 f = (u32)__ffsll((long long)w2) - 1;
            u32 pf = cur + f, mf = rdlane(m, f), cf = rdlane(c, f) - 1;
            while (mf >= LZ_LANE_EXT && pf + mf < bn) {
                u32 x, y; __builtin_memcpy(&x, buf + cf + mf + 4 * lane, 4); __builtin_memcpy(&y, buf + pf + mf + 4 * lane, 4);
                u32 d = x ^ y;
                u64 ne = __ballot(d != 0);
                if (!ne) { mf += 256; continue; }
                u32 l0 = (u32)__ffsll((long long)ne) - 1;
                u32 d0 = rdlane(d, l0);
                mf += 4 * l0 + (((u32)__ffs((int)d0) - 1) >> 3);
                break;
            }
            if (pf + mf > bn) mf = bn - pf;
            u32 ll = pf - anchor;
            for (u32 k = lane; k < ll; k += 64) lits[nl + k] = buf[anchor + k];
            if (lane == 0) { sll[ns] = (u16)ll; sml[ns] = (u16)mf; sof[ns] = (u16)(pf - cf); }
            nl += ll; ns++;
            anchor = next = pf + mf;
        }
        cur += 64;
// ... 337 lines not shown
    mode[b] = lz ? 1 : 0; csize[b] = lz ? s1 : s0;
}

#define ZENC_BLOCKS_PER_WG 16
#define ZENC_OROW 80
template <int GROUP>
__device__ __forceinline__ void huf_encode_stream_staged(u8 *out, const u8 *src, u32 n, const u16 *codes, u8 *orow)
{
    u64 acc = 0; u32 nb = 0;
    u32 lo = (u32)((uintptr_t)out & 63), fill = lo;
    u8 *seg = out - lo;
    auto flush_group = [&]() {
        __builtin_memcpy(orow + fill, &acc, 8);
        fill += nb >> 3; acc >>= (nb & ~7u); nb &= 7;
        if (fill >= 64) {
            if (lo == 0) { const uint4 *r = (const uint4 *)orow; uint4 *g = (uint4 *)seg; g[0] = r[0]; g[1] = r[1]; g[2] = r[2]; g[3] = r[3]; }
            else { for (u32 k = lo; k < 64; k++) seg[k] = orow[k]; lo = 0; }
            u64 t0, t1; __builtin_memcpy(&t0, orow + 64, 8); __builtin_memcpy(&t1, orow + 72, 8);
            __builtin_memcpy(orow, &t0, 8); __builtin_memcpy(orow + 8, &t1, 8);
            seg += 64; fill -= 64;
        }
    };
    auto put_e = [&](u32 e) { acc |= (u64)(e & 0xFFF) << nb; nb += e >> 12; };
    u32 i = n;
    while (i >= 64) {
        i -= 64;
        uint4 q[4]; __builtin_memcpy(q, src + i, 64);
#pragma unroll
        for (int wdx = 7; wdx >= 0; wdx--) {
            const uint4 &qq = q[wdx >> 1];
            u64 w = (wdx & 1) ? ((u64)qq.z | ((u64)qq.w << 32)) : ((u64)qq.x | ((u64)qq.y << 32));
            u32 e[8];
#pragma unroll
            for (int k = 0; k < 8; k++) e[k] = codes[(u32)(w >> (8 * k)) & 0xFF];
            if (GROUP == 8) {
#pragma unroll
                for (int k = 7; k >= 0; k--) put_e(e[k]);
                flush_group();
            } else {
                put_e(e[7]); put_e(e[6]); put_e(e[5]); put_e(e[4]); flush_group();
                put_e(e[3]); put_e(e[2]); put_e(e[1]); put_e(e[0]); flush_group();
            }
        }
    }
    while (i > 0) {
        u32 g = i < 4 ? i : 4;
        for (u32 k = 0; k < g; k++) put_e(codes[src[--i]]);
        flush_group();
    }
    acc |= 1ull << nb; nb++;
    __builtin_memcpy(orow + fill, &acc, 8); fill += (nb + 7) >> 3;
    for (u32 k = lo; k < fill; k++) seg[k] = orow[k];
}

__device__ __forceinline__ void zenc_flat4_stream(u8 *out, const u8 *s, u32 n, const u16 *codes, u32 lane)
{
    const u32 B = (4 * n + 8) >> 3;
    for (u32 t0 = lane * 16; t0 < B; t0 += 64 * 16) {
        const u32 q0 = 2 * t0;
        if (q0 + 32 <= n) {
            uint4 v0, v1; __builtin_memcpy(&v0, s + (n - 32 - q0), 16); __builtin_memcpy(&v1, s + (n - 16 - q0), 16);
            const u32 wd[8] = { v0.x, v0.y, v0.z, v0.w, v1.x, v1.y, v1.z, v1.w };
            u64 lo = 0, hi = 0;
#pragma unroll
            for (int i = 0; i < 16; i++) {
                const u32 a = (wd[(31 - i) >> 2] >> (8 * ((31 - i) & 3))) & 0xFFu, b2 = (wd[(15 - i) >> 2] >> (8 * ((15 - i) & 3))) & 0xFFu;
                lo |= (u64)(codes[a] & 0xFu) << (4 * i);
                hi |= (u64)(codes[b2] & 0xFu) << (4 * i);
            }
            const uint4 o4 = make_uint4((u32)lo, (u32)(lo >> 32), (u32)hi, (u32)(hi >> 32));
            __builtin_memcpy(out + t0, &o4, 16);
        } else {
            const u32 t1 = t0 + 16 < B ? t0 + 16 : B;
            for (u32 t = t0; t < t1; t++) {
                const u32 qa = 2 * t, qb = qa + 1;
                const u32 na = qa < n ? (codes[s[n - 1 - qa]] & 0xFu) : (qa == n ? 1u : 0u), nbv = qb < n ? (codes[s[n - 1 - qb]] & 0xFu) : (qb == n ? 1u : 0u);
                out[t] = (u8)(na | (nbv << 4));
            }
        }
    }
}

struct ZWriteLz { const u8 *mode; const ZEncPlan *plan1; const u16 *codes1; const u8 *trees1; LzBufs B; u32 not_last; u32 wave_general; u32 frame_split; };
struct ZencJob { const u8 *src; size_t n; u32 nblk, frame_wlog; ZEncPlan *plan; u16 *codes; u8 *trees; u64 *offs; u64 hdr; int with_magic, empty; ZWriteLz L; bool direct; u32 block_bytes; ZencLoc dloc; u64 known_total; int have_total; };
template <bool FRAME>
__global__ __launch_bounds__(64) void k_zenc_write(const u8 *src, u64 n, u32 nblk, const ZEncPlan *plan, const u16 *codes_g, const u8 *trees,
                                                    const u64 *offs, u8 *dst, u64 frame_hdr, ZWriteLz L)
{
    __shared__ __attribute__((aligned(16))) u16 codes[FRAME ? 1 : ZENC_BLOCKS_PER_WG][256];
    __shared__ __attribute__((aligned(16))) u8 orows[64 * ZENC_OROW];
    int lane = threadIdx.x;
    u32 b0 = blockIdx.x * ZENC_BLOCKS_PER_WG;
    auto framed = [&](u32 bb) { return plan[bb].kind == ZK_HUF && plan[bb].frame != 0 && !plan[bb].pad; };
    if (FRAME) {
        const u32 bb = b0 + (u32)lane;
        const u64 fr = __ballot(lane < ZENC_BLOCKS_PER_WG && bb < nblk && framed(bb));
        if (!fr) return;
        const uint4 *g = (const uint4 *)(codes_g + (u64)(b0 + (u32)__ffsll((long long)fr) - 1) * 256);
        if (lane < 32) ((uint4 *)codes[0])[lane] = g[lane];
    } else {
    {
        const u32 bb = b0 + (u32)lane;
        const bool other = lane < ZENC_BLOCKS_PER_WG && bb < nblk && !(plan[bb].kind == ZK_HUF && (plan[bb].pad == 2 || L.wave_general) && !(L.mode && L.mode[bb])) && !(L.frame_split && framed(bb));
        if (__ballot(other) == 0) return;
    }
    for (u32 jj = 0; jj < ZENC_BLOCKS_PER_WG; jj++) {
        u32 bb = b0 + jj;
        if (bb >= nblk) break;
        const bool lzb = L.mode && L.mode[bb];
        if ((lzb ? L.plan1[bb].kind : plan[bb].kind) != ZK_HUF || (!lzb && plan[bb].pad == 2)) continue;
        if (L.frame_split && framed(bb)) continue;
        const uint4 *g = (const uint4 *)((lzb ? L.codes1 : codes_g) + (u64)bb * 256);
        if (lane < 32) ((uint4 *)codes[FRAME ? 0 : jj])[lane] = g[lane];
    }
    }
    __syncthreads();
    if (!FRAME) for (u32 jj = 0; jj < ZENC_BLOCKS_PER_WG; jj++) {
        const u32 bb = b0 + jj;
        if (bb >= nblk) break;
        if (L.mode && L.mode[bb]) continue;
        const ZEncPlan p = plan[bb];
        if (p.kind != ZK_HUF || !p.pad || L.wave_general) continue;
        if (p.pad == 2) continue;
        u8 *out = dst + frame_hdr + offs[bb];
        const u64 lo = zenc_block_lo(n, nblk, bb);
        if (lane == 0) { zenc_write_block_prefix(out, p, trees + (u64)bb * ZENC_TREE_SLOT, bb + 1 == nblk && !L.not_last, src[lo]); out[p.csize - 1] = 0; }
        const u32 per = (p.n + 3) / 4;
        u32 o = 3 + p.lhdr + p.tree_bytes + 6;
        for (u32 q = 0; q < 4; q++) { zenc_flat4_stream(out + o, src + lo + (u64)q * per, q < 3 ? per : p.n - 3 * per, codes[FRAME ? 0 : jj], (u32)lane); o += p.ssz[q]; }
    }
    u32 j = lane >> 2, k = lane & 3, b = b0 + j;
    if (b < nblk && (FRAME ? framed(b) : !(L.frame_split && framed(b)))) {
        const bool lzb = L.mode && L.mode[b];
        const u16 *ct = codes[FRAME ? 0 : j];
        u8 *out = dst + frame_hdr + offs[b];
        if (!lzb && plan[b].kind == ZK_HUF && (plan[b].pad || L.wave_general)) { }
        else if (!lzb) {
            const ZEncPlan p = plan[b];
            u64 lo = zenc_block_lo(n, nblk, b);
            if (k == 0) zenc_write_block_prefix(out, p, trees + (u64)b * ZENC_TREE_SLOT, b + 1 == nblk && !L.not_last, p.n ? src[lo] : 0);
            if (p.kind == ZK_HUF) {
                u32 per = (p.n + 3) / 4;
                u32 cnt = k < 3 ? per : p.n - 3 * per;
                const u32 o = 3 + p.lhdr + p.tree_bytes + 6 + (k > 0 ? p.ssz[0] : 0u) + (k > 1 ? p.ssz[1] : 0u) + (k > 2 ? p.ssz[2] : 0u);
                if (p.log <= 7) huf_encode_stream_staged<8>(out + o, src + lo + (u64)k * per, cnt, ct, orows + lane * ZENC_OROW);
                else huf_encode_stream_staged<4>(out + o, src + lo + (u64)k * per, cnt, ct, orows + lane * ZENC_OROW);
                if (k == 3) out[p.csize - 1] = 0;
            }
        } else {
            const ZEncPlan p = L.plan1[b];
            const u8 *lits = L.B.lits + (u64)b * L.B.slot;
            const u32 lsec = lz_lit_section_bytes(p), sbytes = L.B.seq_bytes[b];
            if (k == 0) zenc_write_block_header(out, 2, lsec + sbytes, b + 1 == nblk && !L.not_last);
            if (p.kind == ZK_HUF) {
                if (k == 0) zenc_write_huf_lit_prefix(out + 3, p, L.trees1 + (u64)b * ZENC_TREE_SLOT);
                u32 per = (p.n + 3) / 4;
                u32 cnt = k < 3 ? per : p.n - 3 * per;
                const u32 o = 3 + p.lhdr + p.tree_bytes + 6 + (k > 0 ? p.ssz[0] : 0u) + (k > 1 ? p.ssz[1] : 0u) + (k > 2 ? p.ssz[2] : 0u);
                if (p.log <= 7) huf_encode_stream_staged<8>(out + o, lits + (u64)k * per, cnt, ct, orows + lane * ZENC_OROW);
                else huf_encode_stream_staged<4>(out + o, lits + (u64)k * per, cnt, ct, orows + lane * ZENC_OROW);
            } else if (k == 0) {
                u32 h = zenc_lit_header_raw(out + 3, p.kind == ZK_RLE ? 1u : 0u, p.n);
                if (p.kind == ZK_RLE) out[3 + h] = lits[0];
                else for (u32 i = 0; i < p.n; i++) out[3 + h + i] = lits[i];
            }
            const u8 *sq = L.B.seqbuf + (u64)b * L.B.slot;
            for (u32 i = k; i < sbytes; i += 4) out[3 + lsec + i] = sq[i];
        }
    }
    if (!FRAME) for (u32 jj = 0; jj < ZENC_BLOCKS_PER_WG; jj++) {
        u32 bb = b0 + jj;
        if (bb >= nblk) break;
        if ((L.mode && L.mode[bb]) || plan[bb].kind != ZK_RAW) continue;
        u64 lo = zenc_block_lo(n, nblk, bb);
        u32 bn = plan[bb].n;
        const u8 *s = src + lo; u8 *o = dst + frame_hdr + offs[bb] + 3;
        for (u32 i = lane * 8; i + 8 <= bn; i += 64 * 8) st64(o + i, ld64(s + i));
        for (u32 i = (bn & ~7u) + lane; i < bn; i += 64) o[i] = s[i];
    }
}

#define ZWW_OBUF 12288u
#define ZWW_BLOCKS 64u
__global__ __launch_bounds__(256) void k_zenc_write_wave(const u8 *src, u64 n, u32 nblk, const ZEncPlan *plan, const u16 *codes_g, const u8 *trees,
                                                         const u64 *offs, u8 *dst, u64 frame_hdr, u32 not_last)
{
    extern __shared__ __attribute__((aligned(16))) u8 zww[];
    __shared__ u64 s_general;
    if (threadIdx.x < 64) {
        const u64 bb = (u64)blockIdx.x + (u64)threadIdx.x * gridDim.x;
        const u64 m = __ballot(bb < nblk && plan[bb].kind == ZK_HUF && plan[bb].pad != 2);
        if (threadIdx.x == 0) s_general = m;
    }
    __syncthreads();
    for (u64 todo = s_general; todo; todo &= todo - 1) {
    const u32 b = blockIdx.x + (u32)(__ffsll((long long)todo) - 1) * gridDim.x;
    const ZEncPlan p = plan[b];
    __syncthreads();
    u16 *codes = (u16 *)zww;
    if (threadIdx.x < 32) ((uint4 *)codes)[threadIdx.x] = ((const uint4 *)(codes_g + (u64)b * 256))[threadIdx.x];
    const u32 k = threadIdx.x >> 6, lane = threadIdx.x & 63;
    u32 *ob = (u32 *)(zww + 512 + k * ZWW_OBUF);
    const u32 per = (p.n + 3) / 4, cnt = k < 3 ? per : p.n - 3 * per, sbytes = k == 0 ? p.ssz[0] : k == 1 ? p.ssz[1] : k == 2 ? p.ssz[2] : p.ssz[3];
    for (u32 i = lane; i < (sbytes + 11) / 4; i += 64) ob[i] = 0;
    __syncthreads();
    const u64 lo_b = zenc_block_lo(n, nblk, b);
    const u8 *s = src + lo_b + (u64)k * per;
    u8 *out = dst + frame_hdr + offs[b];
    const u32 o = 3 + p.lhdr + p.tree_bytes + 6 + (k > 0 ? p.ssz[0] : 0u) + (k > 1 ? p.ssz[1] : 0u) + (k > 2 ? p.ssz[2] : 0u);
    if (p.pad == 1) {
        zenc_flat4_stream(out + o, s, cnt, codes, lane);
        if (threadIdx.x == 0) zenc_write_block_prefix(out, p, trees + (u64)b * ZENC_TREE_SLOT, b + 1 == nblk && !not_last, 0);
        if (threadIdx.x == 255) out[p.csize - 1] = 0;
        continue;
    }
    const u32 chunk = (cnt + 63) / 64, lo = lane * chunk < cnt ? lane * chunk : cnt, hi = lo + chunk < cnt ? lo + chunk : cnt;
    u32 bits = 0;
    {
        u32 i = lo;
        for (; i + 8 <= hi; i += 8) { const u64 v = ld64(s + i);
#pragma unroll
            for (u32 q = 0; q < 8; q++) bits += codes[(u32)(v >> (8 * q)) & 0xFFu] >> 12; }
        for (; i < hi; i++) bits += codes[s[i]] >> 12;
    }
    const u32 incl = wave_scan_inclusive<u32, OpAdd>(bits);
    const u32 total = (u32)__builtin_amdgcn_readlane((int)incl, 63);
    u32 pos = total - incl;
    u64 acc = 0; u32 nb = pos & 31, w = pos >> 5;
    {
        u32 i = hi;
        for (; i >= lo + 8; i -= 8) { const u64 v = ld64(s + i - 8);
#pragma unroll
            for (int q = 7; q >= 0; q--) {
                const u32 e = codes[(u32)(v >> (8 * q)) & 0xFFu];
                acc |= (u64)(e & 0xFFFu) << nb; nb += e >> 12;
                if (nb >= 32) { atomicOr(&ob[w], (u32)acc); w++; acc >>= 32; nb -= 32; }
            } }
        for (; i-- > lo;) {
            const u32 e = codes[s[i]];
            acc |= (u64)(e & 0xFFFu) << nb; nb += e >> 12;
            if (nb >= 32) { atomicOr(&ob[w], (u32)acc); w++; acc >>= 32; nb -= 32; }
        }
    }
    if (nb) atomicOr(&ob[w], (u32)acc);
    if (lane == 0) atomicOr(&ob[total >> 5], 1u << (total & 31));
    __syncthreads();
    const u8 *img = (const u8 *)ob;
    for (u32 i = lane * 8; i + 8 <= sbytes; i += 64 * 8) st64(out + o + i, ld64(img + i));
    for (u32 i = (sbytes & ~7u) + lane; i < sbytes; i += 64) out[o + i] = img[i];
    if (threadIdx.x == 0) zenc_write_block_prefix(out, p, trees + (u64)b * ZENC_TREE_SLOT, b + 1 == nblk && !not_last, 0);
    if (threadIdx.x == 255) out[p.csize - 1] = 0;
    }
}

__global__ __launch_bounds__(256) void k_zenc_write_direct(const u8 *src, u32 nblk, const ZEncPlan *plan, const u8 *trees, const u64 *offs, u8 *dst, u64 frame_hdr, u32 not_last)
{
    const u32 b = blockIdx.x, q = threadIdx.x >> 6, lane = threadIdx.x & 63;
    const ZEncPlan p = plan[b];
    if (p.kind != ZK_HUF || p.pad != 2) return;
    const u32 o = 3 + p.lhdr + p.tree_bytes + 6 + (q > 0 ? p.ssz[0] : 0u) + (q > 1 ? p.ssz[1] : 0u) + (q > 2 ? p.ssz[2] : 0u);
    const uint4 *in = (const uint4 *)(src + ((u64)b << 15) + 4096u * q);
    u8 *out = dst + frame_hdr + offs[b], *so = out + o;
    if (threadIdx.x == 255) { zenc_write_block_prefix(out, p, trees + (u64)b * ZENC_TREE_SLOT, b + 1 == nblk && !not_last, 0); out[p.csize - 1] = 0; }
    uint4 v[4];
#pragma unroll
    for (u32 r = 0; r < 4; r++) v[r] = in[r * 64 + lane];
#pragma unroll
    for (u32 r = 0; r < 4; r++) __builtin_memcpy(so + 16u * (r * 64 + lane), &v[r], 16);
    if (lane == 0) so[4096] = 1;
}

__device__ __forceinline__ u32 nibble_rev32(u32 x) { const u32 r = __builtin_bswap32(x); return ((r & 0x0F0F0F0Fu) << 4) | ((r >> 4) & 0x0F0F0F0Fu); }
__global__ __launch_bounds__(256) void k_zenc_write_direct_loc(ZencLoc D, u32 nblk, const ZEncPlan *plan, const u8 *trees, const u64 *offs, u8 *dst, u64 frame_hdr, u32 not_last)
{
    __shared__ i32 s_bnd[4][ZENC_LOC_BND];
    const u32 b = blockIdx.x, q = threadIdx.x >> 6, lane = threadIdx.x & 63;
    const u64 t0 = D.blk_t0[b];
    const i32 mine = lane < ZENC_LOC_BND ? D.blk_bnd[(u64)b * ZENC_LOC_BND + lane] : 0;
    const ZEncPlan p = plan[b];
    if (p.kind != ZK_HUF || p.pad != 2) return;
    if (lane < ZENC_LOC_BND) s_bnd[q][lane] = mine;
    __builtin_amdgcn_fence(__ATOMIC_RELEASE, "wavefront"); __builtin_amdgcn_wave_barrier(); __builtin_amdgcn_fence(__ATOMIC_ACQUIRE, "wavefront");
    const i32 *bnd = s_bnd[q];
    const i32 b0rel = bnd[0];
    uint4 A[4]; u32 E[4], sh[4], avail[4]; u64 N0[4], N1[4];
#pragma unroll
    for (u32 r = 0; r < 4; r++) {
        const u32 cidx = r * 64 + lane, Q = 255u - cidx;
        const i32 r0 = (i32)(16384u * q + 64u * Q);
        u32 k = (u32)(r0 - b0rel) >> 12;
        if (bnd[k + 1] <= r0) k++;
        if (bnd[k + 1] <= r0) k++;
        const u32 i = (u32)(r0 - bnd[k]);
        const u32 *pw = (const u32 *)(D.loc + (t0 + k) * 1024) + (i >> 4);
        __builtin_memcpy(&A[r], pw, 16); E[r] = pw[4];
        sh[r] = 2u * (i & 15u);
        const u32 av = (u32)(bnd[k + 1] - r0);
        avail[r] = av < 64u ? av : 64u;
        N0[r] = N1[r] = 0;
        if (av < 64u) { const u8 *nx = D.loc + (t0 + k + 1) * 1024; N0[r] = ld64(nx); N1[r] = ld64(nx + 8); }
    }
    const u32 o = 3 + p.lhdr + p.tree_bytes + 6 + (q > 0 ? p.ssz[0] : 0u) + (q > 1 ? p.ssz[1] : 0u) + (q > 2 ? p.ssz[2] : 0u);
    u8 *out = dst + frame_hdr + offs[b], *so = out + o;
    if (threadIdx.x == 255) { zenc_write_block_prefix(out, p, trees + (u64)b * ZENC_TREE_SLOT, b + 1 == nblk && !not_last, 0); out[p.csize - 1] = 0; }
    uint4 v[4];
#pragma unroll
    for (u32 r = 0; r < 4; r++) {
        const u32 w0 = __builtin_amdgcn_alignbit(A[r].y, A[r].x, sh[r]), w1 = __builtin_amdgcn_alignbit(A[r].z, A[r].y, sh[r]),
                  w2 = __builtin_amdgcn_alignbit(A[r].w, A[r].z, sh[r]), w3 = __builtin_amdgcn_alignbit(E[r], A[r].w, sh[r]);
        u64 a = (u64)w0 | ((u64)w1 << 32), c = (u64)w2 | ((u64)w3 << 32);
        if (avail[r] < 64u) {
            const u64 n0 = N0[r], n1 = N1[r];
            const u32 s = 2u * avail[r];
            if (s < 64) { const u64 m = (1ull << s) - 1; a = (a & m) | (n0 << s); c = (n1 << s) | (n0 >> (64 - s)); }
            else if (s == 64) { c = n0; }
            else { const u64 m = (1ull << (s - 64)) - 1; c = (c & m) | (n0 << (s - 64)); }
        }
        v[r] = make_uint4(nibble_rev32((u32)(c >> 32)), nibble_rev32((u32)c), nibble_rev32((u32)(a >> 32)), nibble_rev32((u32)a));
    }
#pragma unroll
    for (u32 r = 0; r < 4; r++) __builtin_memcpy(so + 16u * (r * 64 + lane), &v[r], 16);
    if (lane == 0) so[4096] = 1;
}

__global__ void k_zenc_frame_header(u8 *dst, int with_magic, u32 wlog)
{
    if (threadIdx.x || blockIdx.x) return;
    u32 p = 0;
    if (with_magic) { dst[p++] = 0x28; dst[p++] = 0xB5; dst[p++] = 0x2F; dst[p++] = 0xFD; }
    dst[p++] = 0x00;
    dst[p++] = (u8)((wlog - 10) << 3);
}

#define PROBE_REGION_LOG 20
#define PROBE_TLOG 16
__global__ __launch_bounds__(256) void k_ldm_probe(const u8 *src, u64 n, u32 *tab, u32 *counts , int pass, u32 every)
{
    const u64 region = (u64)(blockIdx.x >> 9) * every, rbase = region << PROBE_REGION_LOG;
    const u64 p0 = rbase + ((u64)(blockIdx.x & 511) * 256 + threadIdx.x) * 8;
    u32 anchors = 0, hits = 0;
    if (p0 + 24 <= n) {
        const u64 w0 = ld64(src + p0), w1 = ld64(src + p0 + 8), w2 = ld64(src + p0 + 16);
        u32 *t = tab + ((u64)(blockIdx.x >> 9) << PROBE_TLOG);
#pragma unroll
        for (u32 k = 0; k < 8; k++) {
            const u64 a = k ? (w0 >> (8 * k)) | (w1 << (64 - 8 * k)) : w0, b = k ? (w1 >> (8 * k)) | (w2 << (64 - 8 * k)) : w1;
            u32 idx;
            if (!ldm_key(a, b, PROBE_TLOG, idx) || (ldm_mix(a) >> 58) != 0) continue;
            const u32 rel = (u32)(p0 + k - rbase);
            if (pass == 0) atomicMin(&t[idx], rel);
            else {
                anchors++;
                const u32 q = t[idx];
                if (q < rel && rel - q < (1u << 19) && ld64(src + rbase + q) == a && ld64(src + rbase + q + 8) == b) hits++;
            }
        }
    }
    if (pass) {
        __shared__ u32 s_c[4];
        const u32 tot = wg_reduce1<u32, OpAdd>(anchors | (hits << 16), s_c);
        if (threadIdx.x == 0) counts[blockIdx.x] = tot;
    }
}
int zenc_repeat_probe(naf_gpu_ctx *c, const u8 *d_src, size_t n, u32 *share_1024)
{
    *share_1024 = 0;
    if (n < 65536) return 0;
    if (n < (4u << PROBE_REGION_LOG)) { *share_1024 = 1024; return 0; }
    const u32 every = zenc_probe_every(n);
    const u64 regions = ((n >> PROBE_REGION_LOG) + every - 1) / every;
    const u32 nwg = (u32)(regions * 512);
    u32 *tab = arena_new<u32>(c, regions << PROBE_TLOG), *cnt = arena_new<u32>(c, nwg);
    if (!tab || !cnt) return NAF_GPU_ENOMEM;
    HIP_TRY(c, hipMemsetAsync(tab, 0xFF, (regions << PROBE_TLOG) * 4, c->stream));
    LAUNCH(c, "zenc_probe_insert", k_ldm_probe, nwg, 256, 0, d_src, (u64)n, tab, cnt, 0, every);
    LAUNCH(c, "zenc_probe_count", k_ldm_probe, nwg, 256, 0, d_src, (u64)n, tab, cnt, 1, every);
    std::vector<u32> hc(nwg);
    int rc = ctx_readback(c, hc.data(), cnt, (size_t)nwg * 4); if (rc) return rc;
    u64 h[2] = { 0, 0 };
    for (u32 v : hc) { h[0] += v & 0xFFFF; h[1] += v >> 16; }
    if (h[0]) *share_1024 = (u32)(h[1] * 1024 / h[0]);
    return 0;
}

int zenc_level_window(int level)
{
    static const unsigned char w[23] = { 0, 0, 20, 21, 21, 21, 21, 21, 21, 21, 22, 22, 22, 22, 22, 22, 22, 23, 23, 23, 25, 26, 27 };
    if (level < 2) return 0;
    return w[level > 22 ? 22 : level];
}

extern "C" size_t naf_gpu_zstd_compress_bound(size_t n)
{
    return n + 3 * (n / 1024 + 2) + 64;
}

int zstd_encode_begin(naf_gpu_ctx *c, const u8 *d_src, size_t n, int level, int with_magic, int lz, int block_log_hint, int window_log, ZencJob **job, const u8 *direct, u32 nd, const ZencLoc *dloc)
{
    ZencJob *J = new ZencJob; *job = J;
    memset(J, 0, sizeof *J);
    J->src = d_src; J->n = n;
    const bool part = (with_magic & ZENC_PART) != 0, part_first = (with_magic & ZENC_PART_FIRST) != 0, part_last = (with_magic & ZENC_PART_LAST) != 0;
    const u32 min_gain = (with_magic & ZENC_PREFER_RAW) ? 32u : 0u;
    const bool frame_tree_ok = level <= 1 && (with_magic & ZENC_FRAME_TREE) != 0;
    u32 maxbits = (with_magic & ZENC_PREFER_RAW) ? 9u : (with_magic & ZENC_SHORT_CODES) ? 7u : (u32)ZENC_HUF_MAXBITS;
    u32 prefer_flat = (with_magic & ZENC_PREFER_FLAT) ? 16u : 0u;
    if (prefer_flat) { const char *pf = ctx_opt(c, "PREFER_FLAT"); if (pf && pf[0]) prefer_flat = (u32)atoi(pf); }
    const u32 long_last = ((with_magic & ZENC_LONG_LAST) && (!part || part_last)) ? 1u : 0u;
    with_magic &= ~(ZENC_PREFER_RAW | ZENC_PREFER_FLAT | ZENC_SHORT_CODES | ZENC_FRAME_TREE | ZENC_LONG_LAST);
    if (part) with_magic = 0;
    if (part && n == 0 && !part_last) {
        J->empty = 1; J->hdr = part_first ? 2 : 0; J->frame_wlog = (u32)(window_log >= 10 ? window_log : 19);
        return 0;
    }
    u32 block_log = 15;
    if (block_log_hint >= 10 && block_log_hint <= 17) block_log = (u32)block_log_hint;
    const char *e = ctx_opt(c, "BLOCK_LOG");
    if (e) { int v = atoi(e); if (v >= 10 && v <= 17) block_log = (u32)v; }
    const char *el = ctx_opt(c, "LZ");
    bool use_lz = lz || level >= 2;
    if (el && !strcmp(el, "0")) use_lz = false;
    if (el && !strcmp(el, "all")) use_lz = true;
    if (use_lz && !e) block_log = (lz && block_log_hint >= 10 && block_log_hint <= 15) ? (u32)block_log_hint : 13u;
    if (use_lz && block_log > 15) block_log = 15;
    const bool lzx = use_lz && window_log >= 10 && n >= 64;
    if (window_log > 31) window_log = 31;
    if (lzx) {
        block_log = 16;
        if (block_log > (u32)window_log) block_log = (u32)window_log;
    }
    const u32 frame_wlog = (use_lz && window_log >= 10) ? (u32)window_log : 19u;
    u64 bs = 1ull << block_log;
    u64 nblk64 = n ? (n + bs - 1) / bs : 1;
    if (nblk64 > 0x7FFFFFFFull) return ctx_fail(c, NAF_GPU_EARG, "stream too large");
    u32 nblk = (u32)nblk64;
    u64 hdr = with_magic ? 6 : (part && !part_first) ? 0 : 2;
    ZEncPlan *plan = arena_new<ZEncPlan>(c, nblk);
    u16 *codes = arena_new<u16>(c, (size_t)nblk * 256); u8 *trees = (u8 *)arena_alloc(c, (size_t)nblk * ZENC_TREE_SLOT);
    u64 *offs = arena_new<u64>(c, (size_t)nblk + 2);
    const u32 try_fse = level >= 2;
    const u32 sample_stride = nblk >= 16 * ZENC_CACHE_ENTRIES ? nblk / ZENC_CACHE_ENTRIES : 0;
    ZTreeCache *cache = sample_stride ? arena_new<ZTreeCache>(c, 1) : nullptr;
    if (!plan || !codes || !trees || !offs || (sample_stride && !cache)) return NAF_GPU_ENOMEM;
    if (cache) HIP_TRY(c, hipMemsetAsync(cache, 0, sizeof(ZTreeCache), c->stream));
    u8 *done = nullptr;
    if (direct && (use_lz || block_log != 15 || nblk != nd || n != (size_t)nd << 15 || prefer_flat < 2 || !zenc_flat16().tb))
        return ctx_fail(c, NAF_GPU_EARG, "direct blocks: the stream must be %u blocks of 32 KiB coded without the match finder", nd);
    if (prefer_flat >= 2 && n >= 2048 && zenc_flat16().tb) {
        done = (u8 *)arena_alloc(c, nblk); if (!done) return NAF_GPU_ENOMEM;
        bool dplans = false;
        if (direct) {
            ZEncPlan pd; memset(&pd, 0, sizeof pd);
            const u32 bn = 32768, perq = bn / 4;
            pd.n = bn; pd.kind = ZK_RAW; pd.csize = 3 + bn;
            for (u32 k = 0; k < 4; k++) pd.ssz[k] = (perq * 4 + 8) >> 3;
            zenc_plan_finish(pd, bn, 4, zenc_flat16().tb, min_gain);
            if (pd.kind == ZK_HUF) {
                pd.pad = 2; dplans = true;
                LAUNCH(c, "zenc_direct_plans", k_zenc_direct_plans, cdiv(nblk, 256), 256, 0, direct, nblk, pd, zenc_flat16(), plan, trees, offs, done);
            }
        }
        LAUNCH(c, "zenc_flat_scan", k_zenc_flat_scan, (dplans && cdiv(nblk, ZENC_FLATSCAN_WAVES) > 16384u) ? 16384u : cdiv(nblk, ZENC_FLATSCAN_WAVES), 64 * ZENC_FLATSCAN_WAVES, 0, d_src, (u64)n, nblk, plan, codes, trees, offs, done, min_gain, prefer_flat, zenc_flat16(), dplans ? direct : (const u8 *)nullptr, direct);
    }
    const char *eft = ctx_opt(c, "FRAME_TREE");
    const bool frame_tree = frame_tree_ok && cache && !use_lz && !direct && !(eft && eft[0] == '0');
    u32 *fhist = nullptr; ZEncPlan *fplan = nullptr; u16 *fcodes = nullptr; u8 *ftree = nullptr;
    if (frame_tree) {
        fhist = arena_new<u32>(c, 256 + 2); fplan = arena_new<ZEncPlan>(c, 1); fcodes = arena_new<u16>(c, 256); ftree = (u8 *)arena_alloc(c, ZENC_TREE_SLOT);
        if (!fhist || !fplan || !fcodes || !ftree) return NAF_GPU_ENOMEM;
        HIP_TRY(c, hipMemsetAsync(fhist, 0, 258 * 4, c->stream));
        HIP_TRY(c, hipMemsetAsync(fplan, 0, sizeof(ZEncPlan), c->stream));
        HIP_TRY(c, hipMemsetAsync(fcodes, 0, 512, c->stream));
    }
    if (cache) LAUNCH(c, "zenc_plan_sample", k_zenc_plan, ZENC_CACHE_ENTRIES, 256, 0, d_src, (u64)n, nblk, plan, codes, trees, offs, (const u32 *)nullptr, (u64)0, cache, sample_stride, try_fse, min_gain, maxbits, prefer_flat, (const u8 *)done, (u8 *)nullptr, fhist, (const ZEncPlan *)nullptr, (const u16 *)nullptr);
    if (frame_tree) {
        u8 *fblock = (u8 *)arena_alloc(c, ZENC_FRAME_BLOCK + 64); if (!fblock) return NAF_GPU_ENOMEM;
        LAUNCH(c, "zenc_frame_block", k_zenc_frame_block, 1, 256, 0, (const u32 *)fhist, fblock, fhist + 256);
        u8 *fwt = (u8 *)arena_alloc(c, 256); if (!fwt) return NAF_GPU_ENOMEM;
        LAUNCH(c, "zenc_plan_frame", k_zenc_plan, 1, 256, 0, (const u8 *)fblock, (u64)0, 1u, fplan, fcodes, ftree, (u64 *)nullptr, (const u32 *)(fhist + 256), (u64)0, (ZTreeCache *)nullptr, 0u, try_fse, 0u, maxbits, 0u, (const u8 *)nullptr, fwt, (u32 *)nullptr, (const ZEncPlan *)nullptr, (const u16 *)nullptr);
        LAUNCH(c, "zenc_tree", k_zenc_tree, 1, 64, 64 * sizeof(ZTreeLane), 1u, fplan, ftree, (u64 *)nullptr, (const u8 *)fwt, 0u);
        LAUNCH(c, "zenc_frame_ratio", k_zenc_frame_ratio, 1, 256, 0, fhist, (const u16 *)fcodes);
        const char *fq = ctx_opt(c, "FRAME_QUICK");
        if (!(fq && fq[0] == '0')) {
            float *fstat = arena_new<float>(c, 8); if (!fstat) return NAF_GPU_ENOMEM;
            if (!done) { done = (u8 *)arena_alloc(c, nblk); if (!done) return NAF_GPU_ENOMEM; HIP_TRY(c, hipMemsetAsync(done, 0, nblk, c->stream)); }
            LAUNCH(c, "zenc_frame_stats", k_zenc_frame_stats, 1, 256, 0, (const u32 *)fhist, (const u16 *)fcodes, fstat);
            u32 *tally = arena_new<u32>(c, 2); if (!tally) return NAF_GPU_ENOMEM;
            HIP_TRY(c, hipMemsetAsync(tally, 0, 8, c->stream));
            const u32 qs = nblk / 512 ? nblk / 512 : 1u;
            LAUNCH(c, "zenc_frame_quick", k_zenc_frame_quick, cdiv(nblk, qs), 256, 0, d_src, (u64)n, nblk, plan, codes, offs, done, (const ZEncPlan *)fplan, (const u16 *)fcodes, (const float *)fstat, min_gain, qs, tally, (const u32 *)nullptr);
            LAUNCH(c, "zenc_frame_quick", k_zenc_frame_quick, nblk, 256, 0, d_src, (u64)n, nblk, plan, codes, offs, done, (const ZEncPlan *)fplan, (const u16 *)fcodes, (const float *)fstat, min_gain, 0u, (u32 *)nullptr, (const u32 *)tally);
        }
    }
    LzBufs B; memset(&B, 0, sizeof B);
    u8 *lz_fallback = nullptr;
    const u32 lz_buf = (u32)((bs + 1 + 320 + 15) & ~15ull);
    if (use_lz && n >= 64) {
        B.slot = bs; B.seq_slot = bs / 4 + 2; B.of = nullptr; B.ofv = nullptr;
        B.lits = (u8 *)arena_alloc(c, (size_t)nblk * B.slot + 64); B.seqbuf = (u8 *)arena_alloc(c, (size_t)nblk * B.slot + 64);
        B.ll = arena_new<u16>(c, (size_t)nblk * B.seq_slot + 8); B.ml = arena_new<u16>(c, (size_t)nblk * B.seq_slot + 8);
        if (lzx) B.ofv = arena_new<u32>(c, (size_t)nblk * B.seq_slot + 8); else B.of = arena_new<u16>(c, (size_t)nblk * B.seq_slot + 8);
        B.nseq = arena_new<u32>(c, nblk); B.nlit = arena_new<u32>(c, nblk); B.seq_bytes = arena_new<u32>(c, nblk);
        if (!B.lits || !B.seqbuf || !B.ll || !B.ml || (!B.of && !B.ofv) || !B.nseq || !B.nlit || !B.seq_bytes) return NAF_GPU_ENOMEM;
        const char *ll_ = ctx_opt(c, "LZ_LINES");
        if (!lzx && !(ll_ && ll_[0] == '0') && bs <= 32768 && nblk >= 64) {
            lz_fallback = (u8 *)arena_alloc(c, nblk); if (!lz_fallback) return NAF_GPU_ENOMEM;
            if (!done) { done = (u8 *)arena_alloc(c, nblk); if (!done) return NAF_GPU_ENOMEM; HIP_TRY(c, hipMemsetAsync(done, 0, nblk, c->stream)); }
            const u32 line_div = bs > 16384 ? 16u : 8u, ml_slots = 2 * (u32)(bs / line_div) + 4;
            const u32 lines_lds = lz_buf + 4 * ml_slots + 2 * (u32)(bs / line_div + 2);
            LAUNCH(c, "zenc_lz_lines", k_lz_parse_lines, nblk, 64, lines_lds, d_src, (u64)n, nblk, B, lz_buf, lz_fallback, plan, offs, done, line_div, ml_slots);
        }
    }
    const char *td = ctx_opt(c, "TREE_DEFER");
    u8 *wt_defer = (nblk >= 256 && !(td && td[0] == '0')) ? (u8 *)arena_alloc(c, (size_t)nblk * 256) : nullptr;
    LAUNCH(c, "zenc_plan", k_zenc_plan, nblk, 256, 0, d_src, (u64)n, nblk, plan, codes, trees, offs, (const u32 *)nullptr, (u64)0, cache, 0u, try_fse, min_gain, maxbits, prefer_flat, (const u8 *)done, wt_defer, (u32 *)nullptr, (const ZEncPlan *)fplan, (const u16 *)fcodes, (const u32 *)(fhist ? fhist + 257 : nullptr), long_last);
    if (wt_defer) LAUNCH(c, "zenc_tree", k_zenc_tree, cdiv(nblk, 64), 64, 64 * sizeof(ZTreeLane), nblk, plan, trees, offs, (const u8 *)wt_defer, min_gain);
    if (frame_tree) {
        i32 *fv = arena_new<i32>(c, (size_t)nblk + 1); if (!fv) return NAF_GPU_ENOMEM;
        LAUNCH(c, "zenc_frame_class", k_zenc_frame_class, cdiv(nblk, 256), 256, 0, (const ZEncPlan *)plan, nblk, fv);
        int rcs = scan_inclusive_max_i32(c, fv, nblk); if (rcs) return rcs;
        LAUNCH(c, "zenc_frame_fix", k_zenc_frame_fix, cdiv(nblk, 256), 256, 0, plan, nblk, (const i32 *)fv, (const ZEncPlan *)fplan, (const u8 *)ftree, trees, offs);
    }
    ZWriteLz &L = J->L;
    L.not_last = part && !part_last;
    { const char *fs = ctx_opt(c, "FRAME_WRITE"); L.frame_split = (frame_tree && !(fs && fs[0] == '0')) ? 1u : 0u; }
    if (use_lz && n >= 64) {
        if (!c->d_seqctab) {
            SeqCTabs T; zenc_build_predefined(T);
            HIP_TRY(c, hipMalloc(&c->d_seqctab, sizeof T));
            HIP_TRY(c, hipMemcpy(c->d_seqctab, &T, sizeof T, hipMemcpyHostToDevice));
        }
        ZEncPlan *plan1 = arena_new<ZEncPlan>(c, nblk);
        u16 *codes1 = arena_new<u16>(c, (size_t)nblk * 256); u8 *trees1 = (u8 *)arena_alloc(c, (size_t)nblk * ZENC_TREE_SLOT);
        u8 *mode = (u8 *)arena_alloc(c, nblk);
        if (!plan1 || !codes1 || !trees1 || !mode) return NAF_GPU_ENOMEM;
        if (lzx) {
            LdmTab T; T.wlog = (u32)window_log; T.elog = T.wlog - 1; T.pad = 0;
            const u64 E = 1ull << T.elog, span = n < E ? n : E;
            u32 tl = 4; while ((1ull << tl) < span / 4 + 16) tl++;
            T.tlog = tl;
            const u64 n_ep = (n >> T.elog) + 1, entries = n_ep << T.tlog;
            T.tab = arena_new<u32>(c, entries); if (!T.tab) return NAF_GPU_ENOMEM;
            HIP_TRY(c, hipMemsetAsync(T.tab, 0xFF, entries * 4, c->stream));
            LAUNCH(c, "zenc_ldm_insert", k_ldm_insert, cdiv(cdiv(n, 8), 256), 256, 0, d_src, (u64)n, T);
            HIP_TRY(c, hipFuncSetAttribute((const void *)k_lzx_parse, hipFuncAttributeMaxDynamicSharedMemorySize, (int)(lz_buf + (2u << LZ_HASH_LOG))));
            LAUNCH(c, "zenc_lz_parse", k_lzx_parse, nblk, 64, lz_buf + (2u << LZ_HASH_LOG), d_src, (u64)n, nblk, B, lz_buf, T);
            LAUNCH(c, "zenc_lz_seqenc", k_lzx_seqenc, nblk, 64, 0, nblk, B, (const SeqCTabs *)c->d_seqctab);
        } else {
            const u32 hash_log = LZ_HASH_LOG;
            LAUNCH(c, "zenc_lz_parse", k_lz_parse, nblk, 64, lz_buf + (2u << hash_log), d_src, (u64)n, nblk, B, lz_buf, hash_log, (const u8 *)lz_fallback);
            LAUNCH(c, "zenc_lz_seqenc", k_lz_seqenc, cdiv(nblk, 64), 64, 0, nblk, B, (const SeqCTabs *)c->d_seqctab);
        }
        LAUNCH(c, "zenc_plan", k_zenc_plan, nblk, 256, 0, (const u8 *)B.lits, (u64)n, nblk, plan1, codes1, trees1, (u64 *)nullptr, (const u32 *)B.nlit, B.slot, (ZTreeCache *)nullptr, 0u, try_fse, min_gain, maxbits, 0u, (const u8 *)nullptr, wt_defer);
        if (wt_defer) LAUNCH(c, "zenc_tree", k_zenc_tree, cdiv(nblk, 64), 64, 64 * sizeof(ZTreeLane), nblk, plan1, trees1, (u64 *)nullptr, (const u8 *)wt_defer, min_gain);
        LAUNCH(c, "zenc_lz_choose", k_lz_choose, cdiv(nblk, 256), 256, 0, nblk, (const ZEncPlan *)plan, (const ZEncPlan *)plan1, (const u32 *)B.nseq, (const u32 *)B.seq_bytes, mode, offs);
        L.mode = mode; L.plan1 = plan1; L.codes1 = codes1; L.trees1 = trees1; L.B = B;
    }
    int rc = scan_exclusive_u64(c, offs, nblk, offs + nblk + 1); if (rc) return rc;
    J->direct = direct != nullptr;
    if (direct && dloc) J->dloc = *dloc;
    J->block_bytes = (u32)bs; J->nblk = nblk; J->plan = plan; J->codes = codes; J->trees = trees; J->offs = offs; J->hdr = hdr; J->with_magic = with_magic; J->frame_wlog = frame_wlog;
    return 0;
}

static int zenc_finish(naf_gpu_ctx *c, ZencJob *J, u8 *d_dst, size_t cap, size_t *out_len, const ZencPlace *place);
void zstd_encode_drop(ZencJob *J) { delete J; }
int zstd_encode_finish(naf_gpu_ctx *c, ZencJob *J, u8 *d_dst, size_t cap, size_t *out_len, const ZencPlace *place)
{
    if (!J) return NAF_GPU_EARG;
    int rc = zenc_finish(c, J, d_dst, cap, out_len, place);
    delete J;
    return rc;
}
static int zenc_finish(naf_gpu_ctx *c, ZencJob *J, u8 *d_dst, size_t cap, size_t *out_len, const ZencPlace *place)
{
    const u64 hdr = J->hdr; const u32 nblk = J->nblk;
    if (J->empty) {
        if (place && !(d_dst = place->fn(place->ud, hdr))) return NAF_GPU_ECAP;
        if (!place && cap < hdr) return ctx_fail(c, NAF_GPU_ECAP, "zstd_compress capacity %zu too small", cap);
        if (hdr) LAUNCH(c, "zenc_frame_header", k_zenc_frame_header, 1, 64, 0, d_dst, 0, J->frame_wlog);
        *out_len = hdr;
        return 0;
    }
    if (!place && cap < hdr + J->n + 3ull * nblk) return ctx_fail(c, NAF_GPU_ECAP, "zstd_compress capacity %zu too small (bound %llu)", cap, (unsigned long long)(hdr + J->n + 3ull * nblk));
    int rc;
    u64 total = 0;
    if (place) {
        if (J->have_total) total = J->known_total;
        else if ((rc = ctx_readback(c, &total, J->offs + nblk + 1, 8))) return rc;
        if (!(d_dst = place->fn(place->ud, hdr + total))) return NAF_GPU_ECAP;
    }
    if (hdr) LAUNCH(c, "zenc_frame_header", k_zenc_frame_header, 1, 64, 0, d_dst, J->with_magic, J->frame_wlog);
    {
        J->L.wave_general = (!J->L.mode && J->block_bytes <= 32768u && (J->direct || nblk <= 2048u)) ? 1u : 0u;
    }
    if (J->L.frame_split) LAUNCH(c, "zenc_write", k_zenc_write<true>, cdiv(nblk, ZENC_BLOCKS_PER_WG), 64, 0, J->src, (u64)J->n, nblk, (const ZEncPlan *)J->plan, (const u16 *)J->codes, (const u8 *)J->trees,
           (const u64 *)J->offs, d_dst, hdr, J->L);
    LAUNCH(c, "zenc_write", k_zenc_write<false>, cdiv(nblk, ZENC_BLOCKS_PER_WG), 64, 0, J->src, (u64)J->n, nblk, (const ZEncPlan *)J->plan, (const u16 *)J->codes, (const u8 *)J->trees,
           (const u64 *)J->offs, d_dst, hdr, J->L);
    naf_gpu_ctx *aux = (J->L.wave_general && J->direct && J->have_total && c->side3 && c->split_ev[ZSPLIT_MAX - 1]) ? c->side3 : nullptr;
    if (aux && hipStreamWaitEvent(aux->stream, c->fork_ev, 0) != hipSuccess) aux = nullptr;
    if (aux) {
        hipLaunchKernelGGL(k_zenc_write_wave, dim3(cdiv(nblk, ZWW_BLOCKS)), dim3(256), 512u + 4u * ZWW_OBUF, aux->stream, J->src, (u64)J->n, nblk, (const ZEncPlan *)J->plan, (const u16 *)J->codes, (const u8 *)J->trees,
                           (const u64 *)J->offs, d_dst, hdr, J->L.not_last);
        if (hipGetLastError() != hipSuccess || hipEventRecord(c->split_ev[ZSPLIT_MAX - 1], aux->stream) != hipSuccess) return ctx_fail(c, NAF_GPU_EHIP, "zenc_write_wave beside the gather: launch failed");
    } else
    if (J->L.wave_general) LAUNCH(c, "zenc_write_wave", k_zenc_write_wave, cdiv(nblk, ZWW_BLOCKS), 256, 512u + 4u * ZWW_OBUF, J->src, (u64)J->n, nblk, (const ZEncPlan *)J->plan, (const u16 *)J->codes, (const u8 *)J->trees,
           (const u64 *)J->offs, d_dst, hdr, J->L.not_last);
    if (J->direct && J->dloc.loc) LAUNCH(c, "zenc_write_direct", k_zenc_write_direct_loc, nblk, 256, 0, J->dloc, nblk, (const ZEncPlan *)J->plan, (const u8 *)J->trees, (const u64 *)J->offs, d_dst, hdr, J->L.not_last);
    else if (J->direct) LAUNCH(c, "zenc_write_direct", k_zenc_write_direct, nblk, 256, 0, J->src, nblk, (const ZEncPlan *)J->plan, (const u8 *)J->trees, (const u64 *)J->offs, d_dst, hdr, J->L.not_last);
    if (aux && hipStreamWaitEvent(c->stream, c->split_ev[ZSPLIT_MAX - 1], 0) != hipSuccess) return ctx_fail(c, NAF_GPU_EHIP, "zenc_write_wave beside the gather: join failed");
    if (!place) { if (J->have_total) total = J->known_total; else if ((rc = ctx_readback(c, &total, J->offs + nblk + 1, 8))) return rc; }
    *out_len = hdr + total;
    return 0;
}
const u64 *zstd_encode_total_ptr(const ZencJob *J) { return (!J || J->empty || J->have_total) ? nullptr : J->offs + J->nblk + 1; }
void zstd_encode_set_total(ZencJob *J, u64 total) { if (J && !J->empty) { J->known_total = total; J->have_total = 1; } }
int zstd_encode_size(naf_gpu_ctx *c, ZencJob *J, size_t *frame_len)
{
    if (!J || !frame_len) return NAF_GPU_EARG;
    if (J->empty) { *frame_len = J->hdr; return 0; }
    if (!J->have_total) {
        u64 t = 0; int rc = ctx_readback(c, &t, J->offs + J->nblk + 1, 8); if (rc) return rc;
        J->known_total = t; J->have_total = 1;
    }
    *frame_len = J->hdr + J->known_total;
    return 0;
}

int zstd_encode(naf_gpu_ctx *c, const u8 *d_src, size_t n, int level, u8 *d_dst, size_t cap, size_t *out_len, int with_magic, int lz, int block_log_hint, int window_log, const ZencPlace *place)
{
    ZencJob *J = nullptr;
    int rc = zstd_encode_begin(c, d_src, n, level, with_magic, lz, block_log_hint, window_log, &J);
    if (rc) { delete J; return rc; }
    return zstd_encode_finish(c, J, d_dst, cap, out_len, place);
}

extern "C" int naf_gpu_zstd_compress(naf_gpu_ctx *c, const void *d_src, size_t n, int level, void *d_dst, size_t cap, size_t *out_len)
{
    if (!c || !d_dst || !out_len || (!d_src && n)) return NAF_GPU_EARG;
    if (cap < naf_gpu_zstd_compress_bound(n)) return ctx_fail(c, NAF_GPU_ECAP, "zstd_compress capacity %zu is less than the bound %zu", cap, naf_gpu_zstd_compress_bound(n));
    arena_reset(c);
    return zstd_encode(c, (const u8 *)d_src, n, level, (u8 *)d_dst, cap, out_len, 1, 0, 0, zenc_level_window(level));
}
```

Measured before the change: 4251 GB/s.

## Plan and write only non-direct zstd blocks via a compacted block list

The direct-block verdict kernels now also build a compacted list of non-direct blocks and pre-fill fixed compressed sizes for direct ones. The zstd encoder's flat-scan, plan, tree and write kernels then run grid-stride over that list instead of launching one workgroup per block, and direct-block writers take a shared plan instead of per-block plans. The changed code is all on the encode side (ennaf), while the metric times unnaf decode, so the measured path is probably untouched. Risks include atomics for list building and correctness coupling between the list and the frame's block size.

```diff
diff --git a/naf_amd/csrc/ctx.h b/naf_amd/csrc/ctx.h
--- a/naf_amd/csrc/ctx.h
+++ b/naf_amd/csrc/ctx.h
@@ -119,7 +119,8 @@
 struct ZencPlace { u8 *(*fn)(void *ud, size_t frame_len); void *ud; };
 struct ZencJob;
 #define ZENC_LOC_BND 20
-struct ZencLoc { const u8 *loc; const i32 *blk_bnd; const u32 *blk_t0; u64 tiles; };
+struct ZencLoc { const u8 *loc; const i32 *blk_bnd; const u32 *blk_t0; u64 tiles; const u32 *list; const u32 *list_n; u64 *offs; u32 csize; };
+u32 zenc_direct_csize();
 int zstd_encode_begin(naf_gpu_ctx *c, const u8 *d_src, size_t n, int level, int with_magic, int lz, int block_log_hint, int window_log, ZencJob **job, const u8 *direct = nullptr, u32 nd = 0, const ZencLoc *dloc = nullptr);
 int zstd_encode_finish(naf_gpu_ctx *c, ZencJob *job, u8 *d_dst, size_t cap, size_t *out_len, const ZencPlace *place);
 void zstd_encode_drop(ZencJob *job);
diff --git a/naf_amd/csrc/enc.hip b/naf_amd/csrc/enc.hip
--- a/naf_amd/csrc/enc.hip
+++ b/naf_amd/csrc/enc.hip
@@ -819,7 +819,8 @@
     }
 }
 #define DIRECT_PROBE_BLOCKS_LOG 5
-__global__ __launch_bounds__(256) void k_direct_blocks(const u8 *text, const u64 *t_seq, const u32 *t_reg, u64 tiles, u32 nd, u32 prefer_flat, int probed, u8 *direct, const u32 *blk_t0 = nullptr, i32 *blk_bnd = nullptr)
+__global__ __launch_bounds__(256) void k_direct_blocks(const u8 *text, const u64 *t_seq, const u32 *t_reg, u64 tiles, u32 nd, u32 prefer_flat, int probed, u8 *direct, const u32 *blk_t0 = nullptr, i32 *blk_bnd = nullptr,
+                                                       u32 *list = nullptr, u32 *list_n = nullptr, u64 *offs = nullptr, u32 csize = 0)
 {
     __shared__ u32 bins[4][64];
     const u32 wv = threadIdx.x >> 6, lane = threadIdx.x & 63;
@@ -878,9 +879,13 @@
         ns = (u32)__shfl((int)ns, 0, 64); h = __shfl(h, 0, 64);
         ok = ns >= 1024 && h * (float)prefer_flat > 4.0f * (float)ns * (float)(prefer_flat - 1);
     }
-    if (b < nd && lane == 0) direct[b] = ok ? 1 : 0;
-}
-__global__ __launch_bounds__(256) void k_direct_verdict(const u64 *t_seq, const u32 *t_reg, const u8 *t_hist, u64 tiles, u32 nd, u32 prefer_flat, int probed, const u32 *blk_t0, u8 *direct, i32 *blk_bnd)
+    if (b < nd && lane == 0) {
+        direct[b] = ok ? 1 : 0;
+        if (list) { if (ok) offs[b] = csize; else list[atomicAdd(list_n, 1u)] = b; }
+    }
+}
+__global__ __launch_bounds__(256) void k_direct_verdict(const u64 *t_seq, const u32 *t_reg, const u8 *t_hist, u64 tiles, u32 nd, u32 prefer_flat, int probed, const u32 *blk_t0, u8 *direct, i32 *blk_bnd,
+                                                        u32 *list = nullptr, u32 *list_n = nullptr, u64 *offs = nullptr, u32 csize = 0)
 {
     const u32 b = blockIdx.x * 256 + threadIdx.x;
     if (b >= nd) return;
@@ -920,6 +925,17 @@
         ok = ns >= 1024 && h * (float)prefer_flat > 4.0f * (float)ns * (float)(prefer_flat - 1);
     }
     direct[b] = ok ? 1 : 0;
+    if (list) {
+        if (ok) offs[b] = csize;
+        const u64 m = __ballot(!ok);
+        if (m) {
+            const u32 lane = threadIdx.x & 63, lead = (u32)__ffsll((long long)m) - 1;
+            u32 base = 0;
+            if (lane == lead) base = atomicAdd(list_n, (u32)__popcll(m));
+            base = (u32)__shfl((int)base, (int)lead, 64);
+            if (!ok) list[base + (u32)__popcll(m & ((1ull << lane) - 1))] = b;
+        }
+    }
 }
 __global__ __launch_bounds__(256) void k_case_gather(const u8 *direct, u32 nd, const u32 *blk_t0, const i32 *blk_bnd, const u8 *locc, const u8 *t_lower, u64 *casebits)
 {
@@ -2807,8 +2823,16 @@
                 const bool use_loc = fused && !(e_op && e_op[0] == '3' && !S.no_case);
                 i32 *blk_bnd = use_loc ? arena_new<i32>(c, (size_t)S.nd * ZENC_LOC_BND + 1) : nullptr;
                 if (use_loc && !blk_bnd) return NAF_GPU_ENOMEM;
-                if (use_loc) LAUNCH(c, "ennaf_direct_blocks", k_direct_verdict, cdiv(S.nd, 256), 256, 0, (const u64 *)t_seq, (const u32 *)t_reg, (const u8 *)t_hist, tiles, S.nd, prefer_flat, (epr && epr[0] == '0') ? 0 : (int)zenc_probe_every(n_seqb), (const u32 *)blk_t0, S.direct, blk_bnd);
-                else LAUNCH(c, "ennaf_direct_blocks", k_direct_blocks, cdiv(S.nd, 4), 256, 0, d_text, (const u64 *)t_seq, (const u32 *)t_reg, tiles, S.nd, prefer_flat, (epr && epr[0] == '0') ? 0 : (int)zenc_probe_every(n_seqb), S.direct, (const u32 *)blk_t0, blk_bnd);
+                const char *e_pl = ctx_opt(c, "PLAN_LIST");
+                u32 *nd_list = nullptr, *nd_list_n = nullptr; u64 *nd_offs = nullptr; const u32 d_csize = zenc_direct_csize();
+                if (d_csize && !(e_pl && e_pl[0] == '0')) {
+                    nd_list = arena_new<u32>(c, S.nd); nd_list_n = arena_new<u32>(c, 2); nd_offs = arena_new<u64>(c, (size_t)S.nd + 2);
+                    if (!nd_list || !nd_list_n || !nd_offs) return NAF_GPU_ENOMEM;
+                    HIP_TRY(c, hipMemsetAsync(nd_list_n, 0, 8, c->stream));
+                }
+                if (use_loc) LAUNCH(c, "ennaf_direct_blocks", k_direct_verdict, cdiv(S.nd, 256), 256, 0, (const u64 *)t_seq, (const u32 *)t_reg, (const u8 *)t_hist, tiles, S.nd, prefer_flat, (epr && epr[0] == '0') ? 0 : (int)zenc_probe_every(n_seqb), (const u32 *)blk_t0, S.direct, blk_bnd, nd_list, nd_list_n, nd_offs, d_csize);
+                else LAUNCH(c, "ennaf_direct_blocks", k_direct_blocks, cdiv(S.nd, 4), 256, 0, d_text, (const u64 *)t_seq, (const u32 *)t_reg, tiles, S.nd, prefer_flat, (epr && epr[0] == '0') ? 0 : (int)zenc_probe_every(n_seqb), S.direct, (const u32 *)blk_t0, blk_bnd, nd_list, nd_list_n, nd_offs, d_csize);
+                S.dloc.list = nd_list; S.dloc.list_n = nd_list_n; S.dloc.offs = nd_offs; S.dloc.csize = d_csize;
                 O.direct = S.direct; O.nd = S.nd;
                 if (use_loc) {
                     u32 *sparse_list = arena_new<u32>(c, tiles + 1), *n_sparse = arena_new<u32>(c, 2);
@@ -2959,7 +2983,7 @@
         { const char *sb_ = ctx_opt(c, "NAMES_BLOCK_LOG"); const int v = sb_ ? atoi(sb_) : 0; if (v >= 10 && v <= 15) X.block_log[1] = v; else if (S.n_cmt >= (16u << 20)) X.block_log[1] = 15; }
         X.tail_packed = seq_tail; X.direct = nullptr; X.nd = 0;
         X.dloc = nullptr;
-        if (S.direct && (part & 1)) { X.direct = S.direct; X.nd = S.nd; seq_tail = (u32)(n_seqb & 32767); X.dloc = S.dloc.loc ? &S.dloc : nullptr; }
+        if (S.direct && (part & 1)) { X.direct = S.direct; X.nd = S.nd; seq_tail = (u32)(n_seqb & 32767); X.dloc = (S.dloc.loc || S.dloc.list) ? &S.dloc : nullptr; }
         X.ptr[4] = s_seq; X.len[4] = n_seqb; X.orig[4] = T; X.present[4] = true; X.tail[4] = seq_tail;
         if (S.store_qual) X.flags[4] |= ZENC_LONG_LAST;
         X.ptr[5] = S.s_qual; X.len[5] = X.orig[5] = S.n_qual; X.present[5] = S.store_qual;
@@ -3140,7 +3164,7 @@
     if ((rc = ennaf_windows(c, X, o, overlap ? &probe_later : nullptr))) return rc;
     auto undirect = [&]() -> int {
         if (!X.direct) return 0;
-        X.direct = nullptr; X.nd = 0; X.tail[4] = X.tail_packed; S.direct = nullptr; S.nd = 0; X.dloc = nullptr; S.dloc.loc = nullptr;
+        X.direct = nullptr; X.nd = 0; X.tail[4] = X.tail_packed; S.direct = nullptr; S.nd = 0; X.dloc = nullptr; S.dloc.loc = nullptr; S.dloc.list = nullptr;
         S.sc4.O.direct = nullptr; S.sc4.O.nd = 0; S.sc4.O.loc_mode = 0;
         return ennaf_scatter4(c, S.sc4, S.packed, S.casebits);
     };
diff --git a/naf_amd/csrc/zstd_enc.hip b/naf_amd/csrc/zstd_enc.hip
--- a/naf_amd/csrc/zstd_enc.hip
+++ b/naf_amd/csrc/zstd_enc.hip
@@ -31,6 +31,17 @@
     return T;
 }
 __host__ __device__ static inline u64 zenc_block_lo(u64 n, u32 nblk, u32 b) { u64 q = n / nblk, r = n % nblk; return (u64)b * q + (b < r ? b : r); }
+static ZEncPlan zenc_direct_plan(u32 min_gain)
+{
+    ZEncPlan pd; memset(&pd, 0, sizeof pd);
+    const u32 bn = 32768, perq = bn / 4;
+    pd.n = bn; pd.kind = ZK_RAW; pd.csize = 3 + bn;
+    for (u32 k = 0; k < 4; k++) pd.ssz[k] = (perq * 4 + 8) >> 3;
+    if (zenc_flat16().tb) zenc_plan_finish(pd, bn, 4, zenc_flat16().tb, min_gain);
+    if (pd.kind == ZK_HUF) pd.pad = 2;
+    return pd;
+}
+u32 zenc_direct_csize() { const ZEncPlan pd = zenc_direct_plan(0); return pd.kind == ZK_HUF ? pd.csize : 0u; }
 
 #define ZENC_FLATSCAN_WAVES 4
 __global__ __launch_bounds__(64 * ZENC_FLATSCAN_WAVES) void k_zenc_flat_scan(const u8 *src, u64 n, u32 nblk, ZEncPlan *plan, u16 *codes, u8 *trees, u64 *csize, u8 *done, u32 min_gain, u32 prefer_flat, ZFlat16 f16, const u8 *planned, const u8 *direct)
@@ -106,6 +117,74 @@
     }
 }
 
+#define ZENC_LIST_GRID 1024u
+__global__ __launch_bounds__(256) void k_zenc_flat_scan_list(const u8 *src, u64 n, u32 nblk, ZEncPlan *plan, u16 *codes, u8 *trees, u64 *csize, u8 *done, u32 min_gain, u32 prefer_flat, ZFlat16 f16, const u32 *list, const u32 *list_n)
+{
+    __shared__ u32 bins[64];
+    const u32 lane = threadIdx.x & 63, cnt = *list_n;
+    for (u32 li = blockIdx.x; li < cnt; li += gridDim.x) {
+        const u32 b = list[li];
+        if (threadIdx.x < 64) bins[threadIdx.x] = 0;
+        __syncthreads();
+        const u64 lo = zenc_block_lo(n, nblk, b), hi = zenc_block_lo(n, nblk, b + 1);
+        const u32 bn = (u32)(hi - lo); const u8 *s = src + lo;
+        bool ok = bn >= 2048;
+        u64 bad = 0;
+        if (ok) {
+            const bool sampler = (threadIdx.x & 3) == 0;
+            u32 *mybins = &bins[((threadIdx.x >> 2) & 3) * 16];
+            const u64 M5 = 0x5555555555555555ull, M3 = 0x3333333333333333ull, ONE = 0x1111111111111111ull;
+#pragma unroll 8
+            for (u32 i = threadIdx.x * 16; i + 16 <= bn; i += 4096) {
+                const u64 w0 = ld64(s + i), w1 = ld64(s + i + 8);
+                u64 c0 = w0 - ((w0 >> 1) & M5), c1 = w1 - ((w1 >> 1) & M5);
+                c0 = (c0 & M3) + ((c0 >> 2) & M3); c1 = (c1 & M3) + ((c1 >> 2) & M3);
+                bad |= (c0 ^ ONE) | (c1 ^ ONE);
+                if (sampler) {
+                    const u64 lg = ((w0 >> 1) & 0x7777777777777777ull) - ((w0 >> 3) & 0x1111111111111111ull);
+                    const u64 rk = ((lg >> 2) & 0x0C0C0C0C0C0C0C0Cull) | (lg & 0x0303030303030303ull);
+#pragma unroll
+                    for (u32 k = 0; k < 8; k++) atomicAdd(&mybins[(u32)(rk >> (8 * k)) & 15u], 1u);
+                }
+            }
+            if (threadIdx.x == 0) for (u32 k = bn & ~15u; k < bn; k++) { const u32 v = s[k]; if (__popc(v & 15u) != 1 || __popc(v >> 4) != 1) bad = 1; }
+        }
+        ok = !__syncthreads_or(bad != 0) && ok;
+        bool fast = false;
+        if (ok) {
+            const u32 c = lane < 16 ? bins[lane] + bins[16 + lane] + bins[32 + lane] + bins[48 + lane] : 0u;
+            u32 ns = c;
+#pragma unroll
+            for (u32 d = 1; d < 16; d <<= 1) ns += __shfl_xor((int)ns, d, 64);
+            float h = c ? (float)c * __log2f((float)ns / (float)c) : 0.0f;
+#pragma unroll
+            for (u32 d = 1; d < 16; d <<= 1) h += __shfl_xor(h, d, 64);
+            ns = (u32)__shfl((int)ns, 0, 64); h = __shfl(h, 0, 64);
+            fast = ns > 0 && h * (float)prefer_flat > 4.0f * (float)ns * (float)(prefer_flat - 1);
+        }
+        if (fast) {
+            const u32 perq = (bn + 3) / 4;
+            ZEncPlan p; p.n = bn; p.kind = ZK_RAW; p.csize = 3 + bn; p.log = 0; p.tree_bytes = 0; p.lhdr = 0; p.pad = 0; p.frame = 0; p.pad2 = 0;
+            for (u32 k = 0; k < 4; k++) p.ssz[k] = ((k < 3 ? perq : bn - 3 * perq) * 4 + 8) >> 3;
+            zenc_plan_finish(p, bn, 4, f16.tb, min_gain);
+            fast = p.kind == ZK_HUF;
+            if (fast) {
+                p.pad = 1;
+                if (threadIdx.x == 0) { plan[b] = p; if (csize) csize[b] = p.csize; }
+                {
+                    const u32 sym = threadIdx.x;
+                    const bool is16 = __popc(sym & 15u) == 1 && __popc(sym >> 4) == 1;
+                    const u32 hn = sym >> 4, ln = sym & 15u, rank = 4 * ((hn >> 1) - (hn >> 3)) + ((ln >> 1) - (ln >> 3));
+                    codes[(u64)b * 256 + sym] = is16 ? (u16)(rank | (4u << 12)) : (u16)0;
+                }
+                if (threadIdx.x < p.tree_bytes) trees[(u64)b * ZENC_TREE_SLOT + threadIdx.x] = f16.tree[threadIdx.x];
+            }
+        }
+        if (threadIdx.x == 0) done[b] = fast ? 1 : 0;
+        __syncthreads();
+    }
+}
+
 __global__ void k_zenc_direct_plans(const u8 *direct, u32 nblk, ZEncPlan pd, ZFlat16 f16, ZEncPlan *plan, u8 *trees, u64 *csize, u8 *done)
 {
     const u32 b = blockIdx.x * blockDim.x + threadIdx.x;
@@ -114,11 +193,10 @@
     for (u32 k = 0; k < pd.tree_bytes; k++) trees[(u64)b * ZENC_TREE_SLOT + k] = f16.tree[k];
 }
 
-__global__ __launch_bounds__(256) void k_zenc_plan(const u8 *src, u64 n, u32 nblk, ZEncPlan *plan, u16 *codes, u8 *trees, u64 *csize, const u32 *blk_len, u64 slot, ZTreeCache *cache, u32 sample_stride, u32 try_fse, u32 min_gain, u32 maxbits, u32 prefer_flat, const u8 *done, u8 *wt_defer,
-                                                    u32 *fhist = nullptr, const ZEncPlan *fplan = nullptr, const u16 *fcodes = nullptr, const u32 *fratio = nullptr, u32 long_last = 0)
+__device__ __forceinline__ void zenc_plan_wg(const u32 b, const u8 *src, u64 n, u32 nblk, ZEncPlan *plan, u16 *codes, u8 *trees, u64 *csize, const u32 *blk_len, u64 slot, ZTreeCache *cache, u32 sample_stride, u32 try_fse, u32 min_gain, u32 maxbits, u32 prefer_flat, const u8 *done, u8 *wt_defer,
+                                             u32 *fhist, const ZEncPlan *fplan, const u16 *fcodes, const u32 *fratio, u32 long_last)
 {
     __shared__ u32 hist[ZENC_HCOPIES * 1024];
-    u32 b = sample_stride ? blockIdx.x * sample_stride : blockIdx.x;
     if (done && done[b]) return;
     u64 lo = zenc_block_lo(n, nblk, b), hi = zenc_block_lo(n, nblk, b + 1);
     if (blk_len) { lo = (u64)b * slot; hi = lo + blk_len[b]; }
@@ -385,6 +463,20 @@
         if (!defer && sym < p.tree_bytes) trees[(u64)b * ZENC_TREE_SLOT + sym] = ws.tree[sym];
     }
 }
+__global__ __launch_bounds__(256) void k_zenc_plan(const u8 *src, u64 n, u32 nblk, ZEncPlan *plan, u16 *codes, u8 *trees, u64 *csize, const u32 *blk_len, u64 slot, ZTreeCache *cache, u32 sample_stride, u32 try_fse, u32 min_gain, u32 maxbits, u32 prefer_flat, const u8 *done, u8 *wt_defer,
+                                                    u32 *fhist = nullptr, const ZEncPlan *fplan = nullptr, const u16 *fcodes = nullptr, const u32 *fratio = nullptr, u32 long_last = 0)
+{
+    zenc_plan_wg(sample_stride ? blockIdx.x * sample_stride : blockIdx.x, src, n, nblk, plan, codes, trees, csize, blk_len, slot, cache, sample_stride, try_fse, min_gain, maxbits, prefer_flat, done, wt_defer, fhist, fplan, fcodes, fratio, long_last);
+}
+__global__ __launch_bounds__(256) void k_zenc_plan_list(const u8 *src, u64 n, u32 nblk, ZEncPlan *plan, u16 *codes, u8 *trees, u64 *csize, ZTreeCache *cache, u32 try_fse, u32 min_gain, u32 maxbits, u32 prefer_flat, const u8 *done, u8 *wt_defer, u32 long_last,
+                                                         const u32 *list, const u32 *list_n)
+{
+    const u32 cnt = *list_n;
+    for (u32 li = blockIdx.x; li < cnt; li += gridDim.x) {
+        zenc_plan_wg(list[li], src, n, nblk, plan, codes, trees, csize, (const u32 *)nullptr, (u64)0, cache, 0u, try_fse, min_gain, maxbits, prefer_flat, done, wt_defer, (u32 *)nullptr, (const ZEncPlan *)nullptr, (const u16 *)nullptr, (const u32 *)nullptr, long_last);
+        __syncthreads();
+    }
+}
 
 #define ZENC_FRAME_BLOCK 32768u
 __global__ __launch_bounds__(256) void k_zenc_frame_block(const u32 *fhist, u8 *blockbuf, u32 *blen)
@@ -524,15 +616,8 @@
 
 struct ZTreeLane { FseWS fse; u8 tmp[160]; u8 w[256]; u32 odd; };
 static_assert((sizeof(ZTreeLane) / 4) % 2 == 1, "odd word stride: the lanes' workspaces start in different LDS banks");
-__global__ __launch_bounds__(64) void k_zenc_tree(u32 nblk, ZEncPlan *plan, u8 *trees, u64 *csize, const u8 *wt_defer, u32 min_gain)
-{
-    __builtin_amdgcn_s_setprio(3);
-    extern __shared__ __attribute__((aligned(16))) u8 tree_lds[];
-    const u32 b = blockIdx.x * 64 + threadIdx.x;
-    const bool pending = b < nblk && (plan[b].pad & 0x80u);
-    if (!__ballot(pending)) return;
-    if (!pending) return;
-    ZTreeLane &L = ((ZTreeLane *)tree_lds)[threadIdx.x];
+__device__ __forceinline__ void zenc_tree_lane(const u32 b, ZTreeLane &L, ZEncPlan *plan, u8 *trees, u64 *csize, const u8 *wt_defer, u32 min_gain)
+{
     ZEncPlan p = plan[b];
     const u32 lastw = p.tree_bytes, log = p.log, try_fse = p.lhdr, flat16 = p.pad & 1u;
     for (u32 k = 0; k < 256; k += 4) *(u32 *)(L.w + k) = *(const u32 *)(wt_defer + (u64)b * 256 + k);
@@ -542,6 +627,28 @@
     if (tb) { zenc_plan_finish(p, p.n, log, tb, min_gain); if (p.kind == ZK_HUF && flat16) p.pad = 1; }
     plan[b] = p;
     if (csize) csize[b] = p.csize;
+}
+__global__ __launch_bounds__(64) void k_zenc_tree(u32 nblk, ZEncPlan *plan, u8 *trees, u64 *csize, const u8 *wt_defer, u32 min_gain)
+{
+    __builtin_amdgcn_s_setprio(3);
+    extern __shared__ __attribute__((aligned(16))) u8 tree_lds[];
+    const u32 b = blockIdx.x * 64 + threadIdx.x;
+    const bool pending = b < nblk && (plan[b].pad & 0x80u);
+    if (!__ballot(pending)) return;
+    if (!pending) return;
+    zenc_tree_lane(b, ((ZTreeLane *)tree_lds)[threadIdx.x], plan, trees, csize, wt_defer, min_gain);
+}
+__global__ __launch_bounds__(64) void k_zenc_tree_list(ZEncPlan *plan, u8 *trees, u64 *csize, const u8 *wt_defer, u32 min_gain, const u32 *list, const u32 *list_n)
+{
+    __builtin_amdgcn_s_setprio(3);
+    extern __shared__ __attribute__((aligned(16))) u8 tree_lds[];
+    const u32 cnt = *list_n;
+    for (u32 l0 = blockIdx.x * 64; l0 < cnt; l0 += gridDim.x * 64) {
+        const u32 li = l0 + threadIdx.x;
+        if (li >= cnt) continue;
+        const u32 b = list[li];
+        if (plan[b].pad & 0x80u) zenc_tree_lane(b, ((ZTreeLane *)tree_lds)[threadIdx.x], plan, trees, csize, wt_defer, min_gain);
+    }
 }
 
 #define LZ_MINMATCH 5
@@ -1045,17 +1152,18 @@
 }
 
 struct ZWriteLz { const u8 *mode; const ZEncPlan *plan1; const u16 *codes1; const u8 *trees1; LzBufs B; u32 not_last; u32 wave_general; u32 frame_split; };
-struct ZencJob { const u8 *src; size_t n; u32 nblk, frame_wlog; ZEncPlan *plan; u16 *codes; u8 *trees; u64 *offs; u64 hdr; int with_magic, empty; ZWriteLz L; bool direct; u32 block_bytes; ZencLoc dloc; u64 known_total; int have_total; };
+struct ZencJob { const u8 *src; size_t n; u32 nblk, frame_wlog; ZEncPlan *plan; u16 *codes; u8 *trees; u64 *offs; u64 hdr; int with_magic, empty; ZWriteLz L; bool direct; u32 block_bytes; ZencLoc dloc; u64 known_total; int have_total; const u8 *dflags; ZEncPlan pd; bool dplans; const u32 *list, *list_n; u32 list_grid; hipEvent_t planned_ev; };
 template <bool FRAME>
-__global__ __launch_bounds__(64) void k_zenc_write(const u8 *src, u64 n, u32 nblk, const ZEncPlan *plan, const u16 *codes_g, const u8 *trees,
-                                                    const u64 *offs, u8 *dst, u64 frame_hdr, ZWriteLz L)
+__device__ __forceinline__ void zenc_write_wg(const u32 grp, const u32 *list, const u32 cnt, const u8 *src, u64 n, u32 nblk, const ZEncPlan *plan, const u16 *codes_g, const u8 *trees,
+                                              const u64 *offs, u8 *dst, u64 frame_hdr, const ZWriteLz &L)
 {
     __shared__ __attribute__((aligned(16))) u16 codes[FRAME ? 1 : ZENC_BLOCKS_PER_WG][256];
     __shared__ __attribute__((aligned(16))) u8 orows[64 * ZENC_OROW];
     int lane = threadIdx.x;
-    u32 b0 = blockIdx.x * ZENC_BLOCKS_PER_WG;
+    auto blk = [&](u32 jj) -> u32 { const u32 e = grp * ZENC_BLOCKS_PER_WG + jj; return !list ? e : e < cnt ? list[e] : nblk; };
     auto framed = [&](u32 bb) { return plan[bb].kind == ZK_HUF && plan[bb].frame != 0 && !plan[bb].pad; };
     if (FRAME) {
+        const u32 b0 = grp * ZENC_BLOCKS_PER_WG;
         const u32 bb = b0 + (u32)lane;
         const u64 fr = __ballot(lane < ZENC_BLOCKS_PER_WG && bb < nblk && framed(bb));
         if (!fr) return;
@@ -1063,12 +1171,12 @@
         if (lane < 32) ((uint4 *)codes[0])[lane] = g[lane];
     } else {
     {
-        const u32 bb = b0 + (u32)lane;
-        const bool other = lane < ZENC_BLOCKS_PER_WG && bb < nblk && !(plan[bb].kind == ZK_HUF && (plan[bb].pad == 2 || L.wave_general) && !(L.mode && L.mode[bb])) && !(L.frame_split && framed(bb));
+        const u32 bb = lane < ZENC_BLOCKS_PER_WG ? blk((u32)lane) : nblk;
+        const bool other = bb < nblk && !(plan[bb].kind == ZK_HUF && (plan[bb].pad == 2 || L.wave_general) && !(L.mode && L.mode[bb])) && !(L.frame_split && framed(bb));
         if (__ballot(other) == 0) return;
     }
     for (u32 jj = 0; jj < ZENC_BLOCKS_PER_WG; jj++) {
-        u32 bb = b0 + jj;
+        u32 bb = blk(jj);
         if (bb >= nblk) break;
         const bool lzb = L.mode && L.mode[bb];
         if ((lzb ? L.plan1[bb].kind : plan[bb].kind) != ZK_HUF || (!lzb && plan[bb].pad == 2)) continue;
@@ -1079,7 +1187,7 @@
     }
     __syncthreads();
     if (!FRAME) for (u32 jj = 0; jj < ZENC_BLOCKS_PER_WG; jj++) {
-        const u32 bb = b0 + jj;
+        const u32 bb = blk(jj);
         if (bb >= nblk) break;
         if (L.mode && L.mode[bb]) continue;
         const ZEncPlan p = plan[bb];
@@ -1092,7 +1200,7 @@
         u32 o = 3 + p.lhdr + p.tree_bytes + 6;
         for (u32 q = 0; q < 4; q++) { zenc_flat4_stream(out + o, src + lo + (u64)q * per, q < 3 ? per : p.n - 3 * per, codes[FRAME ? 0 : jj], (u32)lane); o += p.ssz[q]; }
     }
-    u32 j = lane >> 2, k = lane & 3, b = b0 + j;
+    u32 j = lane >> 2, k = lane & 3, b = blk(j);
     if (b < nblk && (FRAME ? framed(b) : !(L.frame_split && framed(b)))) {
         const bool lzb = L.mode && L.mode[b];
         const u16 *ct = codes[FRAME ? 0 : j];
@@ -1132,7 +1240,7 @@
         }
     }
     if (!FRAME) for (u32 jj = 0; jj < ZENC_BLOCKS_PER_WG; jj++) {
-        u32 bb = b0 + jj;
+        u32 bb = blk(jj);
         if (bb >= nblk) break;
         if ((L.mode && L.mode[bb]) || plan[bb].kind != ZK_RAW) continue;
         u64 lo = zenc_block_lo(n, nblk, bb);
@@ -1142,22 +1250,43 @@
         for (u32 i = (bn & ~7u) + lane; i < bn; i += 64) o[i] = s[i];
     }
 }
+template <bool FRAME>
+__global__ __launch_bounds__(64) void k_zenc_write(const u8 *src, u64 n, u32 nblk, const ZEncPlan *plan, const u16 *codes_g, const u8 *trees,
+                                                    const u64 *offs, u8 *dst, u64 frame_hdr, ZWriteLz L)
+{
+    zenc_write_wg<FRAME>(blockIdx.x, (const u32 *)nullptr, 0u, src, n, nblk, plan, codes_g, trees, offs, dst, frame_hdr, L);
+}
+__global__ __launch_bounds__(64) void k_zenc_write_list(const u8 *src, u64 n, u32 nblk, const ZEncPlan *plan, const u16 *codes_g, const u8 *trees,
+                                                         const u64 *offs, u8 *dst, u64 frame_hdr, ZWriteLz L, const u32 *list, const u32 *list_n)
+{
+    const u32 cnt = *list_n;
+    for (u32 g = blockIdx.x; g * ZENC_BLOCKS_PER_WG < cnt; g += gridDim.x) {
+        zenc_write_wg<false>(g, list, cnt, src, n, nblk, plan, codes_g, trees, offs, dst, frame_hdr, L);
+        __syncthreads();
+    }
+}
 
 #define ZWW_OBUF 12288u
 #define ZWW_BLOCKS 64u
 __global__ __launch_bounds__(256) void k_zenc_write_wave(const u8 *src, u64 n, u32 nblk, const ZEncPlan *plan, const u16 *codes_g, const u8 *trees,
-                                                         const u64 *offs, u8 *dst, u64 frame_hdr, u32 not_last)
+                                                         const u64 *offs, u8 *dst, u64 frame_hdr, u32 not_last, const u32 *list = nullptr, const u32 *list_n = nullptr)
 {
     extern __shared__ __attribute__((aligned(16))) u8 zww[];
     __shared__ u64 s_general;
+    const u64 total = list ? *list_n : nblk;
+    for (u64 e0 = blockIdx.x; e0 < total; e0 += (u64)ZWW_BLOCKS * gridDim.x) {
     if (threadIdx.x < 64) {
-        const u64 bb = (u64)blockIdx.x + (u64)threadIdx.x * gridDim.x;
+        const u64 e = e0 + (u64)threadIdx.x * gridDim.x;
+        const u64 bb = e >= total ? nblk : list ? list[e] : e;
         const u64 m = __ballot(bb < nblk && plan[bb].kind == ZK_HUF && plan[bb].pad != 2);
         if (threadIdx.x == 0) s_general = m;
     }
     __syncthreads();
-    for (u64 todo = s_general; todo; todo &= todo - 1) {
-    const u32 b = blockIdx.x + (u32)(__ffsll((long long)todo) - 1) * gridDim.x;
+    const u64 general = s_general;
+    __syncthreads();
+    for (u64 todo = general; todo; todo &= todo - 1) {
+    const u64 e = e0 + (u64)(__ffsll((long long)todo) - 1) * gridDim.x;
+    const u32 b = list ? list[e] : (u32)e;
     const ZEncPlan p = plan[b];
     __syncthreads();
     u16 *codes = (u16 *)zww;
@@ -1214,17 +1343,17 @@
     if (threadIdx.x == 0) zenc_write_block_prefix(out, p, trees + (u64)b * ZENC_TREE_SLOT, b + 1 == nblk && !not_last, 0);
     if (threadIdx.x == 255) out[p.csize - 1] = 0;
     }
-}
-
-__global__ __launch_bounds__(256) void k_zenc_write_direct(const u8 *src, u32 nblk, const ZEncPlan *plan, const u8 *trees, const u64 *offs, u8 *dst, u64 frame_hdr, u32 not_last)
+    }
+}
+
+__global__ __launch_bounds__(256) void k_zenc_write_direct(const u8 *src, u32 nblk, const u8 *direct, const ZEncPlan p, const ZFlat16 f16, const u64 *offs, u8 *dst, u64 frame_hdr, u32 not_last)
 {
     const u32 b = blockIdx.x, q = threadIdx.x >> 6, lane = threadIdx.x & 63;
-    const ZEncPlan p = plan[b];
-    if (p.kind != ZK_HUF || p.pad != 2) return;
+    if (!direct[b]) return;
     const u32 o = 3 + p.lhdr + p.tree_bytes + 6 + (q > 0 ? p.ssz[0] : 0u) + (q > 1 ? p.ssz[1] : 0u) + (q > 2 ? p.ssz[2] : 0u);
     const uint4 *in = (const uint4 *)(src + ((u64)b << 15) + 4096u * q);
     u8 *out = dst + frame_hdr + offs[b], *so = out + o;
-    if (threadIdx.x == 255) { zenc_write_block_prefix(out, p, trees + (u64)b * ZENC_TREE_SLOT, b + 1 == nblk && !not_last, 0); out[p.csize - 1] = 0; }
+    if (threadIdx.x == 255) { zenc_write_block_prefix(out, p, f16.tree, b + 1 == nblk && !not_last, 0); out[p.csize - 1] = 0; }
     uint4 v[4];
 #pragma unroll
     for (u32 r = 0; r < 4; r++) v[r] = in[r * 64 + lane];
@@ -1234,14 +1363,13 @@
 }
 
 __device__ __forceinline__ u32 nibble_rev32(u32 x) { const u32 r = __builtin_bswap32(x); return ((r & 0x0F0F0F0Fu) << 4) | ((r >> 4) & 0x0F0F0F0Fu); }
-__global__ __launch_bounds__(256) void k_zenc_write_direct_loc(ZencLoc D, u32 nblk, const ZEncPlan *plan, const u8 *trees, const u64 *offs, u8 *dst, u64 frame_hdr, u32 not_last)
+__global__ __launch_bounds__(256) void k_zenc_write_direct_loc(ZencLoc D, u32 nblk, const u8 *direct, const ZEncPlan p, const ZFlat16 f16, const u64 *offs, u8 *dst, u64 frame_hdr, u32 not_last)
 {
     __shared__ i32 s_bnd[4][ZENC_LOC_BND];
     const u32 b = blockIdx.x, q = threadIdx.x >> 6, lane = threadIdx.x & 63;
     const u64 t0 = D.blk_t0[b];
     const i32 mine = lane < ZENC_LOC_BND ? D.blk_bnd[(u64)b * ZENC_LOC_BND + lane] : 0;
-    const ZEncPlan p = plan[b];
-    if (p.kind != ZK_HUF || p.pad != 2) return;
+    if (!direct[b]) return;
     if (lane < ZENC_LOC_BND) s_bnd[q][lane] = mine;
     __builtin_amdgcn_fence(__ATOMIC_RELEASE, "wavefront"); __builtin_amdgcn_wave_barrier(); __builtin_amdgcn_fence(__ATOMIC_ACQUIRE, "wavefront");
     const i32 *bnd = s_bnd[q];
@@ -1265,7 +1393,7 @@
     }
     const u32 o = 3 + p.lhdr + p.tree_bytes + 6 + (q > 0 ? p.ssz[0] : 0u) + (q > 1 ? p.ssz[1] : 0u) + (q > 2 ? p.ssz[2] : 0u);
     u8 *out = dst + frame_hdr + offs[b], *so = out + o;
-    if (threadIdx.x == 255) { zenc_write_block_prefix(out, p, trees + (u64)b * ZENC_TREE_SLOT, b + 1 == nblk && !not_last, 0); out[p.csize - 1] = 0; }
+    if (threadIdx.x == 255) { zenc_write_block_prefix(out, p, f16.tree, b + 1 == nblk && !not_last, 0); out[p.csize - 1] = 0; }
     uint4 v[4];
 #pragma unroll
     for (u32 r = 0; r < 4; r++) {
@@ -1400,7 +1528,8 @@
     u64 hdr = with_magic ? 6 : (part && !part_first) ? 0 : 2;
     ZEncPlan *plan = arena_new<ZEncPlan>(c, nblk);
     u16 *codes = arena_new<u16>(c, (size_t)nblk * 256); u8 *trees = (u8 *)arena_alloc(c, (size_t)nblk * ZENC_TREE_SLOT);
-    u64 *offs = arena_new<u64>(c, (size_t)nblk + 2);
+    const bool with_list = direct && dloc && dloc->list && dloc->list_n && dloc->offs;
+    u64 *offs = with_list ? dloc->offs : arena_new<u64>(c, (size_t)nblk + 2);
     const u32 try_fse = level >= 2;
     const u32 sample_stride = nblk >= 16 * ZENC_CACHE_ENTRIES ? nblk / ZENC_CACHE_ENTRIES : 0;
     ZTreeCache *cache = sample_stride ? arena_new<ZTreeCache>(c, 1) : nullptr;
@@ -1413,16 +1542,22 @@
         done = (u8 *)arena_alloc(c, nblk); if (!done) return NAF_GPU_ENOMEM;
         bool dplans = false;
         if (direct) {
-            ZEncPlan pd; memset(&pd, 0, sizeof pd);
-            const u32 bn = 32768, perq = bn / 4;
-            pd.n = bn; pd.kind = ZK_RAW; pd.csize = 3 + bn;
-            for (u32 k = 0; k < 4; k++) pd.ssz[k] = (perq * 4 + 8) >> 3;
-            zenc_plan_finish(pd, bn, 4, zenc_flat16().tb, min_gain);
+            ZEncPlan pd = zenc_direct_plan(min_gain);
             if (pd.kind == ZK_HUF) {
-                pd.pad = 2; dplans = true;
+                dplans = true; J->pd = pd; J->dplans = true;
+                if (with_list && pd.csize != dloc->csize) return ctx_fail(c, NAF_GPU_EARG, "direct blocks: the list was made for blocks of %u bytes, the frame's are %u", dloc->csize, pd.csize);
+                if (with_list) {
+                    const char *eg = ctx_opt(c, "PLAN_LIST_GRID");
+                    u32 grid = nblk < ZENC_LIST_GRID ? nblk : ZENC_LIST_GRID;
+                    if (eg && atoi(eg) >= 1 && (u32)atoi(eg) < grid) grid = (u32)atoi(eg);
+                    J->list = dloc->list; J->list_n = dloc->list_n; J->list_grid = grid;
+                    HIP_TRY(c, hipMemsetAsync(done, 1, nblk, c->stream));
+                    LAUNCH(c, "zenc_flat_scan", k_zenc_flat_scan_list, grid, 256, 0, d_src, (u64)n, nblk, plan, codes, trees, offs, done, min_gain, prefer_flat, zenc_flat16(), J->list, J->list_n);
+                } else
                 LAUNCH(c, "zenc_direct_plans", k_zenc_direct_plans, cdiv(nblk, 256), 256, 0, direct, nblk, pd, zenc_flat16(), plan, trees, offs, done);
-            }
-        }
+            } else if (with_list) return ctx_fail(c, NAF_GPU_EARG, "direct blocks: a list, and the blocks are not Huffman blocks");
+        }
+        if (!J->list)
         LAUNCH(c, "zenc_flat_scan", k_zenc_flat_scan, (dplans && cdiv(nblk, ZENC_FLATSCAN_WAVES) > 16384u) ? 16384u : cdiv(nblk, ZENC_FLATSCAN_WAVES), 64 * ZENC_FLATSCAN_WAVES, 0, d_src, (u64)n, nblk, plan, codes, trees, offs, done, min_gain, prefer_flat, zenc_flat16(), dplans ? direct : (const u8 *)nullptr, direct);
     }
     const char *eft = ctx_opt(c, "FRAME_TREE");
@@ -1476,8 +1611,13 @@
     }
     const char *td = ctx_opt(c, "TREE_DEFER");
     u8 *wt_defer = (nblk >= 256 && !(td && td[0] == '0')) ? (u8 *)arena_alloc(c, (size_t)nblk * 256) : nullptr;
+    if (J->list) {
+        LAUNCH(c, "zenc_plan", k_zenc_plan_list, J->list_grid, 256, 0, d_src, (u64)n, nblk, plan, codes, trees, offs, cache, try_fse, min_gain, maxbits, prefer_flat, (const u8 *)done, wt_defer, long_last, J->list, J->list_n);
+        if (wt_defer) LAUNCH(c, "zenc_tree", k_zenc_tree_list, J->list_grid, 64, 64 * sizeof(ZTreeLane), plan, trees, offs, (const u8 *)wt_defer, min_gain, J->list, J->list_n);
+    } else {
     LAUNCH(c, "zenc_plan", k_zenc_plan, nblk, 256, 0, d_src, (u64)n, nblk, plan, codes, trees, offs, (const u32 *)nullptr, (u64)0, cache, 0u, try_fse, min_gain, maxbits, prefer_flat, (const u8 *)done, wt_defer, (u32 *)nullptr, (const ZEncPlan *)fplan, (const u16 *)fcodes, (const u32 *)(fhist ? fhist + 257 : nullptr), long_last);
     if (wt_defer) LAUNCH(c, "zenc_tree", k_zenc_tree, cdiv(nblk, 64), 64, 64 * sizeof(ZTreeLane), nblk, plan, trees, offs, (const u8 *)wt_defer, min_gain);
+    }
     if (frame_tree) {
         i32 *fv = arena_new<i32>(c, (size_t)nblk + 1); if (!fv) return NAF_GPU_ENOMEM;
         LAUNCH(c, "zenc_frame_class", k_zenc_frame_class, cdiv(nblk, 256), 256, 0, (const ZEncPlan *)plan, nblk, fv);
@@ -1520,7 +1660,8 @@
         L.mode = mode; L.plan1 = plan1; L.codes1 = codes1; L.trees1 = trees1; L.B = B;
     }
     int rc = scan_exclusive_u64(c, offs, nblk, offs + nblk + 1); if (rc) return rc;
-    J->direct = direct != nullptr;
+    J->direct = direct != nullptr; J->dflags = direct;
+    if (direct && c->split_ev[ZSPLIT_MAX - 2] && hipEventRecord(c->split_ev[ZSPLIT_MAX - 2], c->stream) == hipSuccess) J->planned_ev = c->split_ev[ZSPLIT_MAX - 2];
     if (direct && dloc) J->dloc = *dloc;
     J->block_bytes = (u32)bs; J->nblk = nblk; J->plan = plan; J->codes = codes; J->trees = trees; J->offs = offs; J->hdr = hdr; J->with_magic = with_magic; J->frame_wlog = frame_wlog;
     return 0;
@@ -1557,22 +1698,34 @@
     {
         J->L.wave_general = (!J->L.mode && J->block_bytes <= 32768u && (J->direct || nblk <= 2048u)) ? 1u : 0u;
     }
+    const u32 *list = J->list, *list_n = J->list_n;
+    const u32 g16 = cdiv(J->list_grid, ZENC_BLOCKS_PER_WG), gww = J->list_grid;
     if (J->L.frame_split) LAUNCH(c, "zenc_write", k_zenc_write<true>, cdiv(nblk, ZENC_BLOCKS_PER_WG), 64, 0, J->src, (u64)J->n, nblk, (const ZEncPlan *)J->plan, (const u16 *)J->codes, (const u8 *)J->trees,
            (const u64 *)J->offs, d_dst, hdr, J->L);
+    if (list) LAUNCH(c, "zenc_write", k_zenc_write_list, g16, 64, 0, J->src, (u64)J->n, nblk, (const ZEncPlan *)J->plan, (const u16 *)J->codes, (const u8 *)J->trees,
+           (const u64 *)J->offs, d_dst, hdr, J->L, list, list_n);
+    else
     LAUNCH(c, "zenc_write", k_zenc_write<false>, cdiv(nblk, ZENC_BLOCKS_PER_WG), 64, 0, J->src, (u64)J->n, nblk, (const ZEncPlan *)J->plan, (const u16 *)J->codes, (const u8 *)J->trees,
            (const u64 *)J->offs, d_dst, hdr, J->L);
-    naf_gpu_ctx *aux = (J->L.wave_general && J->direct && J->have_total && c->side3 && c->split_ev[ZSPLIT_MAX - 1]) ? c->side3 : nullptr;
-    if (aux && hipStreamWaitEvent(aux->stream, c->fork_ev, 0) != hipSuccess) aux = nullptr;
+    naf_gpu_ctx *aux = (J->L.wave_general && J->direct && J->have_total && J->planned_ev && c->side3 && c->split_ev[ZSPLIT_MAX - 1]) ? c->side3 : nullptr;
+    if (aux && hipStreamWaitEvent(aux->stream, J->planned_ev, 0) != hipSuccess) aux = nullptr;
+    const u32 ww_grid = list ? gww : cdiv(nblk, ZWW_BLOCKS);
     if (aux) {
-        hipLaunchKernelGGL(k_zenc_write_wave, dim3(cdiv(nblk, ZWW_BLOCKS)), dim3(256), 512u + 4u * ZWW_OBUF, aux->stream, J->src, (u64)J->n, nblk, (const ZEncPlan *)J->plan, (const u16 *)J->codes, (const u8 *)J->trees,
-                           (const u64 *)J->offs, d_dst, hdr, J->L.not_last);
-        if (hipGetLastError() != hipSuccess || hipEventRecord(c->split_ev[ZSPLIT_MAX - 1], aux->stream) != hipSuccess) return ctx_fail(c, NAF_GPU_EHIP, "zenc_write_wave beside the gather: launch failed");
+        hipLaunchKernelGGL(k_zenc_write_wave, dim3(ww_grid), dim3(256), 512u + 4u * ZWW_OBUF, aux->stream, J->src, (u64)J->n, nblk, (const ZEncPlan *)J->plan, (const u16 *)J->codes, (const u8 *)J->trees,
+                           (const u64 *)J->offs, d_dst, hdr, J->L.not_last, list, list_n);
+        if (hipGetLastError() != hipSuccess || hipEventRecord(c->split_ev[ZSPLIT_MAX - 1], aux->stream) != hipSuccess) {
+            hipStreamSynchronize(aux->stream);
+            return ctx_fail(c, NAF_GPU_EHIP, "zenc_write_wave beside the gather: launch failed");
+        }
     } else
-    if (J->L.wave_general) LAUNCH(c, "zenc_write_wave", k_zenc_write_wave, cdiv(nblk, ZWW_BLOCKS), 256, 512u + 4u * ZWW_OBUF, J->src, (u64)J->n, nblk, (const ZEncPlan *)J->plan, (const u16 *)J->codes, (const u8 *)J->trees,
-           (const u64 *)J->offs, d_dst, hdr, J->L.not_last);
-    if (J->direct && J->dloc.loc) LAUNCH(c, "zenc_write_direct", k_zenc_write_direct_loc, nblk, 256, 0, J->dloc, nblk, (const ZEncPlan *)J->plan, (const u8 *)J->trees, (const u64 *)J->offs, d_dst, hdr, J->L.not_last);
-    else if (J->direct) LAUNCH(c, "zenc_write_direct", k_zenc_write_direct, nblk, 256, 0, J->src, nblk, (const ZEncPlan *)J->plan, (const u8 *)J->trees, (const u64 *)J->offs, d_dst, hdr, J->L.not_last);
-    if (aux && hipStreamWaitEvent(c->stream, c->split_ev[ZSPLIT_MAX - 1], 0) != hipSuccess) return ctx_fail(c, NAF_GPU_EHIP, "zenc_write_wave beside the gather: join failed");
+    if (J->L.wave_general) LAUNCH(c, "zenc_write_wave", k_zenc_write_wave, ww_grid, 256, 512u + 4u * ZWW_OBUF, J->src, (u64)J->n, nblk, (const ZEncPlan *)J->plan, (const u16 *)J->codes, (const u8 *)J->trees,
+           (const u64 *)J->offs, d_dst, hdr, J->L.not_last, list, list_n);
+    if (J->direct && J->dplans && J->dloc.loc) LAUNCH(c, "zenc_write_direct", k_zenc_write_direct_loc, nblk, 256, 0, J->dloc, nblk, J->dflags, J->pd, zenc_flat16(), (const u64 *)J->offs, d_dst, hdr, J->L.not_last);
+    else if (J->direct && J->dplans) LAUNCH(c, "zenc_write_direct", k_zenc_write_direct, nblk, 256, 0, J->src, nblk, J->dflags, J->pd, zenc_flat16(), (const u64 *)J->offs, d_dst, hdr, J->L.not_last);
+    if (aux && hipStreamWaitEvent(c->stream, c->split_ev[ZSPLIT_MAX - 1], 0) != hipSuccess) {
+        hipStreamSynchronize(aux->stream);
+        return ctx_fail(c, NAF_GPU_EHIP, "zenc_write_wave beside the gather: join failed");
+    }
     if (!place) { if (J->have_total) total = J->known_total; else if ((rc = ctx_readback(c, &total, J->offs + nblk + 1, 8))) return rc; }
     *out_len = hdr + total;
     return 0;
```

Result: no change. 4259 GB/s, median of 2 (+0.2%).
